# lakehq/sail

Hardware: NVIDIA H100
Metric: TPC-H Q1 rows/s (scan+filter+hash-aggregate), lineitem resident in HBM (higher is better)
Workload: dtype i128 (Decimal128) / i64

## Files before the change

sail_b200/csrc/capi.cu:

```cuda
#include <cstdio>

#include "h2d.hpp"
#include "runner.hpp"

using namespace sg;

struct sailgpu_ctx {
  Ctx ctx;
};
struct sailgpu_op {
  std::unique_ptr<Op> op;
  sailgpu_ctx* owner = nullptr;
  std::string last_error;
  std::vector<bool> input_finished;
};

namespace sg { std::atomic<bool> g_exiting{false}; }

namespace {
thread_local std::string g_ctx_error;
void mark_exiting() { sg::g_exiting.store(true); }

template <typename F>
int32_t guard(std::string* err, F&& f) {
  try {
    f();
    return SAILGPU_OK;
  } catch (const Error& e) {
    if (err) *err = e.what();
    return e.code;
  } catch (const std::exception& e) {
    if (err) *err = std::string("internal error: ") + e.what();
    return SAILGPU_ERR_CUDA;
  }
}
void set_device(const Ctx& c) { SG_CUDA(cudaSetDevice(c.device)); }
using CtxLock = std::lock_guard<std::recursive_mutex>;
}

namespace sg { void set_ctx_error(const std::string& m) { g_ctx_error = m; } }
namespace sg { void resolve_exchange_timing(Ctx* ctx);
void pipeline_static_check(const Json& spec, const std::vector<Schema>& inputs);
size_t pipeline_precompile(const Json& spec, const std::vector<Schema>& inputs, uint64_t validity_mask, bool cold, bool compile, std::string* source); }

namespace sg {
struct ParquetColumnDesc { const uint8_t* chunk; uint64_t chunk_len; int32_t physical_type, type_length, max_def_level, codec; int64_t num_values; };
DevColumn decode_parquet_column(Ctx* ctx, const Field& f, const ParquetColumnDesc& c, int64_t n_rows);
std::string parquet_plan_summary(const Field& f, const ParquetColumnDesc& c, int64_t n_rows);
}

extern "C" {

SAILGPU_API void sailgpu_borrowed_release(struct ArrowArray* a) { if (a) a->release = nullptr; }

SAILGPU_API uint32_t sailgpu_version(void) { return (0u << 16) | 1u; }

SAILGPU_API int32_t sailgpu_ctx_create(int32_t device, sailgpu_ctx** out) {
  return guard(&g_ctx_error, [&] {
    SG_CHECK(out != nullptr, SAILGPU_ERR_INVALID, "out is null");
    int n = 0;
    cudaError_t e = cudaGetDeviceCount(&n);
    if (e != cudaSuccess || n == 0)
      fail(SAILGPU_ERR_NO_DEVICE, std::string("no usable CUDA device (") + cudaGetErrorString(e) + "); libsailgpu has no CPU fallback");
    SG_CHECK(device >= 0 && device < n, SAILGPU_ERR_INVALID, "device ordinal out of range");
    static const int hooked = std::atexit(mark_exiting);
    (void)hooked;
    auto c = std::make_unique<sailgpu_ctx>();
    c->ctx.device = device;
    SG_CUDA(cudaSetDevice(device));
    cudaDeviceProp prop;
    SG_CUDA(cudaGetDeviceProperties(&prop, device));
    SG_CHECK(prop.major == 9 && prop.minor == 0, SAILGPU_ERR_NO_DEVICE, std::string("device '") + prop.name + "' is not sm_90 (Hopper); this library only carries sm_90a code");
    c->ctx.sm_count = prop.multiProcessorCount;
    c->ctx.max_smem = prop.sharedMemPerBlockOptin;
    SG_CUDA(cudaStreamCreateWithFlags(&c->ctx.stream, cudaStreamNonBlocking));
    cudaMemPool_t pool;
    SG_CUDA(cudaDeviceGetDefaultMemPool(&pool, device));
    uint64_t threshold = UINT64_MAX;
    SG_CUDA(cudaMemPoolSetAttribute(pool, cudaMemPoolAttrReleaseThreshold, &threshold));
    *out = c.release();
  });
}

SAILGPU_API void sailgpu_ctx_destroy(sailgpu_ctx* c) {
  if (!c) return;
  if (sg::g_exiting.load()) return;
  CtxLock lk(c->ctx.mu);
  cudaSetDevice(c->ctx.device);
  c->ctx.shared_objects.clear();
  c->ctx.dead.store(true);
  if (c->ctx.stream) { cudaStreamSynchronize(c->ctx.stream); cudaStreamDestroy(c->ctx.stream); c->ctx.stream = nullptr; }
  destroy_pack_pool(&c->ctx);
}

SAILGPU_API const char* sailgpu_ctx_last_error(const sailgpu_ctx*) { return g_ctx_error.c_str(); }

SAILGPU_API void* sailgpu_ctx_stream(sailgpu_ctx* c) { return c ? (void*)c->ctx.stream : nullptr; }
SAILGPU_API int32_t sailgpu_ctx_synchronize(sailgpu_ctx* c) {
  return guard(&g_ctx_error, [&] {
    SG_CHECK(c != nullptr, SAILGPU_ERR_INVALID, "null context");
    CtxLock lk(c->ctx.mu);
    set_device(c->ctx);
    SG_CUDA(cudaStreamSynchronize(c->ctx.stream));
  });
}

SAILGPU_API int32_t sailgpu_op_create(sailgpu_ctx* c, const char* spec_json, size_t spec_len, const struct ArrowSchema* const* input_schemas,
                          int32_t n_inputs, int32_t partition, sailgpu_op** out, struct ArrowSchema* out_schema) {
  return guard(&g_ctx_error, [&] {
    SG_CHECK(c && spec_json && out && out_schema, SAILGPU_ERR_INVALID, "null argument");
    CtxLock lk(c->ctx.mu);
    set_device(c->ctx);
    Json spec = JsonParser(spec_json, spec_len).parse();
    std::vector<Schema> ins;
    for (int i = 0; i < n_inputs; ++i) ins.push_back(schema_from_arrow(input_schemas[i]));
    auto h = std::make_unique<sailgpu_op>();
    h->owner = c;
    h->op = make_op(&c->ctx, spec, ins, partition);
    h->input_finished.assign((size_t)n_inputs, false);
    schema_to_arrow(h->op->out_schema, out_schema);
    *out = h.release();
  });
}

SAILGPU_API int32_t sailgpu_spec_validate(const char* spec_json, size_t spec_len, const struct ArrowSchema* const* input_schemas,
                                          int32_t n_inputs, struct ArrowSchema* out_schema, char* err_buf, size_t err_cap) {
  std::string err;
  const int32_t rc = guard(&err, [&] {
    SG_CHECK(spec_json && out_schema, SAILGPU_ERR_INVALID, "null argument");
    Json spec = JsonParser(spec_json, spec_len).parse();
    std::vector<Schema> ins;
    for (int i = 0; i < n_inputs; ++i) ins.push_back(schema_from_arrow(input_schemas[i]));
    std::unique_ptr<Op> op = make_op(nullptr, spec, ins, 0);
    pipeline_static_check(spec, ins);
    schema_to_arrow(op->out_schema, out_schema);
  });
  if (rc != 0 && err_buf && err_cap) { const size_t k = std::min(err.size(), err_cap - 1); memcpy(err_buf, err.data(), k); err_buf[k] = 0; }
  return rc;
}

SAILGPU_API int64_t sailgpu_jit_precompile(const char* spec_json, size_t spec_len, const struct ArrowSchema* const* input_schemas, int32_t n_inputs,
                                           uint64_t validity_mask, int32_t flags, char* buf, size_t cap) {
  std::string err, source;
  size_t cubin = 0;
  const int32_t rc = guard(&err, [&] {
    SG_CHECK(spec_json && n_inputs >= 1, SAILGPU_ERR_INVALID, "null argument");
    Json spec = JsonParser(spec_json, spec_len).parse();
    std::vector<Schema> ins;
    for (int i = 0; i < n_inputs; ++i) ins.push_back(schema_from_arrow(input_schemas[i]));
    cubin = pipeline_precompile(spec, ins, validity_mask, (flags & SAILGPU_JIT_COLD_VARIANT) != 0, (flags & SAILGPU_JIT_COMPILE) != 0, &source);
  });
// ... 9 lines not shown
  const int32_t rc = guard(&err, [&] {
    SG_CHECK(schema_c && cols && column >= 0 && column < n_cols, SAILGPU_ERR_INVALID, "bad argument");
    Schema schema = schema_from_arrow(schema_c);
    SG_CHECK((int)schema.size() == n_cols, SAILGPU_ERR_INVALID, "parquet: column count mismatch");
    ParquetColumnDesc d{cols[column].chunk, cols[column].chunk_len, cols[column].physical_type, cols[column].type_length, cols[column].max_def_level, cols[column].codec, cols[column].num_values};
    out = parquet_plan_summary(schema[(size_t)column], d, n_rows);
  });
  const std::string& text = rc != 0 ? err : out;
  if (buf && cap) { const size_t k = std::min(text.size(), cap - 1); memcpy(buf, text.data(), k); buf[k] = 0; }
  return rc;
}
SAILGPU_API int32_t sailgpu_parquet_decode(sailgpu_ctx* c, const struct ArrowSchema* schema_c, const sailgpu_parquet_column* cols, int32_t n_cols, int64_t n_rows,
                                           struct ArrowDeviceArray* out) {
  return guard(&g_ctx_error, [&] {
    SG_CHECK(c && schema_c && cols && out && n_rows >= 0, SAILGPU_ERR_INVALID, "null argument");
    CtxLock lk(c->ctx.mu);
    set_device(c->ctx);
    Schema schema = schema_from_arrow(schema_c);
    SG_CHECK((int)schema.size() == n_cols, SAILGPU_ERR_INVALID, "parquet: " + std::to_string(n_cols) + " column chunks for a schema of " + std::to_string(schema.size()) + " fields");
    auto b = std::make_shared<DevBatch>();
    b->rows = n_rows;
    for (int i = 0; i < n_cols; ++i) {
      ParquetColumnDesc d{cols[i].chunk, cols[i].chunk_len, cols[i].physical_type, cols[i].type_length, cols[i].max_def_level, cols[i].codec, cols[i].num_values};
      b->cols.push_back(decode_parquet_column(&c->ctx, schema[(size_t)i], d, n_rows));
    }
    export_device_batch(&c->ctx, schema, b, out);
  });
}

SAILGPU_API int32_t sailgpu_op_push(sailgpu_op* h, int32_t input_idx, struct ArrowArray* batch) {
  if (!h) return SAILGPU_ERR_INVALID;
  return guard(&h->last_error, [&] {
    CtxLock lk(h->owner->ctx.mu);
    set_device(h->owner->ctx);
    SG_CHECK(input_idx >= 0 && input_idx < (int)h->op->in_schemas.size(), SAILGPU_ERR_INVALID, "input index out of range");
    SG_CHECK(!h->input_finished[(size_t)input_idx], SAILGPU_ERR_STATE, "push after finish_input");
    BatchPtr b = import_host_batch(&h->owner->ctx, h->op->in_schemas[(size_t)input_idx], batch);
    h->op->push(input_idx, b);
  });
}

SAILGPU_API int32_t sailgpu_op_push_device(sailgpu_op* h, int32_t input_idx, struct ArrowDeviceArray* batch) {
  if (!h) return SAILGPU_ERR_INVALID;
  return guard(&h->last_error, [&] {
    CtxLock lk(h->owner->ctx.mu);
    set_device(h->owner->ctx);
    SG_CHECK(input_idx >= 0 && input_idx < (int)h->op->in_schemas.size(), SAILGPU_ERR_INVALID, "input index out of range");
    SG_CHECK(!h->input_finished[(size_t)input_idx], SAILGPU_ERR_STATE, "push after finish_input");
    SG_CHECK(batch && batch->array.release, SAILGPU_ERR_INVALID, "batch is null or released");
    BatchPtr b = take_internal_batch(batch, &h->owner->ctx);
    if (!b) { SG_CHECK(batch->array.n_children == (int64_t)h->op->in_schemas[(size_t)input_idx].size(), SAILGPU_ERR_INVALID, "device batch has no column arrays (a handle of another library instance?)"); }
    if (!b) { Trace t(&h->owner->ctx, "import_device_batch"); b = import_device_batch(&h->owner->ctx, h->op->in_schemas[(size_t)input_idx], batch); }
    Trace t2(&h->owner->ctx, "op.push");
    h->op->push(input_idx, b);
  });
}

SAILGPU_API int32_t sailgpu_op_finish_input(sailgpu_op* h, int32_t input_idx) {
  if (!h) return SAILGPU_ERR_INVALID;
  return guard(&h->last_error, [&] {
    CtxLock lk(h->owner->ctx.mu);
    set_device(h->owner->ctx);
    SG_CHECK(input_idx >= 0 && input_idx < (int)h->op->in_schemas.size(), SAILGPU_ERR_INVALID, "input index out of range");
    if (h->input_finished[(size_t)input_idx]) return;
    h->input_finished[(size_t)input_idx] = true;
    Trace t(&h->owner->ctx, "op.finish");
    h->op->finish(input_idx);
  });
}

static int32_t pull_common(sailgpu_op* h, int part, struct ArrowArray* host_out, struct ArrowDeviceArray* dev_out, int32_t* has_more, bool handle_only = false) {
  if (!h) return SAILGPU_ERR_INVALID;
  return guard(&h->last_error, [&] {
    CtxLock lk(h->owner->ctx.mu);
    set_device(h->owner->ctx);
    SG_CHECK(has_more && (host_out || dev_out), SAILGPU_ERR_INVALID, "null argument");
    BatchPtr b;
    bool more;
    { Trace t(&h->owner->ctx, "op.pull"); more = part >= 0 ? h->op->pull_partition(part, &b) : h->op->pull(&b); }
    Trace t2(&h->owner->ctx, "export");
    *has_more = more ? 1 : 0;
    if (!b) b = empty_batch(&h->owner->ctx, h->op->out_schema);
    if (host_out) export_host_batch(&h->owner->ctx, h->op->out_schema, b, host_out);
    else export_device_batch(&h->owner->ctx, h->op->out_schema, b, dev_out, handle_only);
  });
}

SAILGPU_API int32_t sailgpu_op_pull(sailgpu_op* h, struct ArrowArray* out, int32_t* has_more) { return pull_common(h, -1, out, nullptr, has_more); }
SAILGPU_API int32_t sailgpu_op_pull_device(sailgpu_op* h, struct ArrowDeviceArray* out, int32_t* has_more) { return pull_common(h, -1, nullptr, out, has_more); }
SAILGPU_API int32_t sailgpu_op_pull_device_handle(sailgpu_op* h, struct ArrowDeviceArray* out, int32_t* has_more) { return pull_common(h, -1, nullptr, out, has_more, true); }
SAILGPU_API int32_t sailgpu_op_pull_partition(sailgpu_op* h, int32_t part, struct ArrowDeviceArray* out, int32_t* has_more) {
  if (part < 0) return SAILGPU_ERR_INVALID;
  return pull_common(h, part, nullptr, out, has_more);
}

SAILGPU_API int32_t sailgpu_op_pull_ipc(sailgpu_op* h, uint8_t** data, size_t* len, int64_t* rows, int32_t* has_more) {
  if (!h || !data || !len || !has_more) return SAILGPU_ERR_INVALID;
  struct ArrowArray batch;
  memset(&batch, 0, sizeof(batch));
  int32_t rc = pull_common(h, -1, &batch, nullptr, has_more);
  if (rc != SAILGPU_OK) return rc;
  struct ArrowSchema schema;
  memset(&schema, 0, sizeof(schema));
  rc = guard(&h->last_error, [&] { schema_to_arrow(h->op->out_schema, &schema); });
  if (rc == SAILGPU_OK) {
    rc = sailgpu_ipc_stream(&schema, &batch, data, len);
    if (rc != SAILGPU_OK) h->last_error = sailgpu_ipc_last_error();
    else if (rows) *rows = batch.length;
  }
  if (schema.release) schema.release(&schema);
  if (batch.release) batch.release(&batch);
  return rc;
}

SAILGPU_API int64_t sailgpu_op_metrics(sailgpu_op* h, char* json_buf, size_t cap) {
  if (!h) return -1;
  CtxLock lk(h->owner->ctx.mu);
  cudaSetDevice(h->owner->ctx.device);
  const Metrics& m = h->op->m;
  char tmp[2048];
  sg::resolve_exchange_timing(&h->owner->ctx);
  int n = snprintf(tmp, sizeof(tmp),
                   "{\"output_rows\":%llu,\"output_batches\":%llu,\"input_rows\":%llu,\"input_batches\":%llu,"
                   "\"elapsed_compute\":%llu,\"build_input_rows\":%llu,\"build_input_batches\":%llu,\"build_time\":%llu,"
                   "\"join_time\":%llu,\"gpu.kernel_launches\":%llu,\"gpu.h2d_bytes\":%llu,\"gpu.d2h_bytes\":%llu,"
                   "\"gpu.pipeline_launches\":%llu,\"gpu.jit_launches\":%llu,\"gpu.pipeline_kernel_ns\":%llu,"
                   "\"gpu.exchange_sent_bytes\":%llu,\"gpu.exchange_recv_bytes\":%llu,\"gpu.exchange_ns\":%llu,\"gpu.exchange_calls\":%llu}",
                   (unsigned long long)m.output_rows, (unsigned long long)m.output_batches, (unsigned long long)m.input_rows,
                   (unsigned long long)m.input_batches, (unsigned long long)m.elapsed_compute_ns, (unsigned long long)m.build_input_rows,
                   (unsigned long long)m.build_input_batches, (unsigned long long)m.build_time_ns, (unsigned long long)m.join_time_ns,
                   (unsigned long long)m.kernel_launches, (unsigned long long)h->owner->ctx.h2d_bytes.load(),
                   (unsigned long long)h->owner->ctx.d2h_bytes.load(), (unsigned long long)h->op->m.pipeline_launches, (unsigned long long)h->op->m.jit_launches,
                   (unsigned long long)h->op->pipeline_kernel_ns(), (unsigned long long)h->owner->ctx.exch_sent_bytes.load(),
                   (unsigned long long)h->owner->ctx.exch_recv_bytes.load(), (unsigned long long)h->owner->ctx.exch_ns.load(),
                   (unsigned long long)h->owner->ctx.exch_calls.load());
  if (json_buf && cap) { size_t k = std::min<size_t>((size_t)n, cap - 1); memcpy(json_buf, tmp, k); json_buf[k] = 0; }
  return n + 1;
}

SAILGPU_API const char* sailgpu_last_error(const sailgpu_op* h) { return h ? h->last_error.c_str() : "null handle"; }

SAILGPU_API void sailgpu_op_destroy(sailgpu_op* h) {
  if (!h) return;
  if (sg::g_exiting.load()) return;
  CtxLock lk(h->owner->ctx.mu);
  cudaSetDevice(h->owner->ctx.device);
  cudaStreamSynchronize(h->owner->ctx.stream);
  delete h;
}

SAILGPU_API int32_t sailgpu_host_alloc(sailgpu_ctx* c, size_t bytes, void** out) {
  return guard(&g_ctx_error, [&] {
    SG_CHECK(c && out, SAILGPU_ERR_INVALID, "null argument");
    CtxLock lk(c->ctx.mu);
    set_device(c->ctx);
    SG_CUDA(cudaHostAlloc(out, bytes ? bytes : 1, cudaHostAllocDefault));
  });
}
SAILGPU_API void sailgpu_host_free(sailgpu_ctx* c, void* p) {
  if (!c || !p) return;
  CtxLock lk(c->ctx.mu);
  cudaSetDevice(c->ctx.device);
  cudaFreeHost(p);
}

}
```

sail_b200/csrc/device.cu:

```cuda
#include <cstdlib>
#include <cstring>

#include "device.hpp"
#include "h2d.hpp"
#include "kernels.hpp"
#include "relational.hpp"

namespace sg {

Schema schema_from_arrow(const ArrowSchema* s) {
  SG_CHECK(s && s->format && std::string(s->format) == "+s", SAILGPU_ERR_INVALID, "input schema must be a struct (+s)");
  Schema out;
  for (int64_t i = 0; i < s->n_children; ++i) {
    const ArrowSchema* c = s->children[i];
    Field f;
    f.name = c->name ? c->name : "";
    f.type = type_from_arrow_format(c->format);
    f.nullable = (c->flags & ARROW_FLAG_NULLABLE) != 0;
    out.push_back(f);
  }
  return out;
}

namespace {
struct SchemaPriv {
  std::string format, name;
  std::vector<ArrowSchema> children;
  std::vector<ArrowSchema*> child_ptrs;
};
void release_schema(ArrowSchema* s) {
  if (!s || !s->release) return;
  for (int64_t i = 0; i < s->n_children; ++i)
// ... 82 lines not shown
  c.type = f.type;
  c.length = a->length;
  c.null_count = a->null_count;
  auto borrow = [&](const void* p, size_t bytes) {
    auto b = std::make_shared<DevBuf>();
    b->ptr = const_cast<void*>(p); b->bytes = bytes;
    b->on_release = [token] {};
    return b;
  };
  const uint8_t* vbits = a->n_buffers > 0 ? static_cast<const uint8_t*>(a->buffers[0]) : nullptr;
  if (vbits && a->null_count != 0 && a->length > 0) {
    c.validity = import_bitmap(J, vbits, a->offset, a->length);
    if (on_device && c.validity->on_release) c.validity->on_release = [token] {};
    if (c.null_count < 0) c.null_count = -1;
  } else {
    c.null_count = 0;
  }
  const int w = f.type.arrow_width();
  switch (f.type.id) {
    case TypeId::Bool: {
      const uint8_t* bits = static_cast<const uint8_t*>(a->buffers[1]);
      c.data = a->length ? import_bitmap(J, bits, a->offset, a->length) : dev_alloc(ctx, 0);
      if (on_device && c.data->on_release) c.data->on_release = [token] {};
      break;
    }
    case TypeId::Utf8: {
      const int32_t* offs = static_cast<const int32_t*>(a->buffers[1]) + a->offset;
      const uint8_t* bytes = static_cast<const uint8_t*>(a->buffers[2]);
      BufPtr doffs, dbytes;
      if (on_device) {
        doffs = borrow(offs, (size_t)(a->length + 1) * 4);
        int32_t last = 0;
        if (a->length) SG_CUDA(cudaMemcpyAsync(&last, offs + a->length, 4, cudaMemcpyDeviceToHost, stream));
        SG_CUDA(cudaStreamSynchronize(stream));
        dbytes = borrow(bytes, (size_t)last);
      } else {
        doffs = J.upload(offs, a->length + 1, 4);
        const int32_t last = a->length ? offs[a->length] : 0;
        dbytes = J.upload(bytes, last, 1);
      }
      c.data = dev_alloc(ctx, (size_t)a->length * 16);
      {
        BufPtr views = c.data;
        const int64_t n = a->length;
        J.after([=] { SG_CUDA(launch_utf8_to_views(static_cast<const int32_t*>(doffs->ptr), static_cast<const uint8_t*>(dbytes->ptr), views->ptr, n, stream)); });
      }
      c.heaps = {dbytes, doffs};
      c.arrow_is_utf8 = true;
      break;
    }
    case TypeId::Utf8View: {
      const uint8_t* views = static_cast<const uint8_t*>(a->buffers[1]) + a->offset * 16;
      const int64_t n_data = a->n_buffers - 3;
      if (on_device && n_data <= 0) c.data = borrow(views, (size_t)a->length * 16);
      else c.data = J.upload(views, a->length, 16, n_data <= 0 ? HostCol::View16 : HostCol::Raw);
      if (n_data > 0) {
        std::vector<int64_t> sizes((size_t)n_data);
        const int64_t* size_buf = static_cast<const int64_t*>(a->buffers[a->n_buffers - 1]);
        if (on_device) { SG_CUDA(cudaMemcpyAsync(sizes.data(), size_buf, (size_t)n_data * 8, cudaMemcpyDeviceToHost, stream)); SG_CUDA(cudaStreamSynchronize(stream)); }
        else std::memcpy(sizes.data(), size_buf, (size_t)n_data * 8);
        auto bases = std::make_shared<std::vector<uint64_t>>((size_t)n_data);
        for (int64_t k = 0; k < n_data; ++k) {
          BufPtr h = on_device ? borrow(a->buffers[2 + k], (size_t)sizes[k]) : J.upload(a->buffers[2 + k], sizes[k], 1);
          (*bases)[(size_t)k] = reinterpret_cast<uint64_t>(h->ptr);
          c.heaps.push_back(h);
        }
        BufPtr dbases = dev_alloc(ctx, (size_t)n_data * 8);
        BufPtr vdata = c.data;
        const int64_t n = a->length;
        J.after([=] {
          SG_CUDA(cudaMemcpyAsync(dbases->ptr, bases->data(), (size_t)n_data * 8, cudaMemcpyHostToDevice, stream));
          SG_CUDA(launch_resolve_views(vdata->ptr, n, static_cast<const uint64_t*>(dbases->ptr), stream));
          SG_CUDA(cudaStreamSynchronize(stream));
        });
        c.heaps.push_back(dbases);
      }
      break;
    }
    default: {
      SG_CHECK(w > 0, SAILGPU_ERR_UNSUPPORTED, "unsupported column type " + f.type.str());
      const uint8_t* p = static_cast<const uint8_t*>(a->buffers[1]) + a->offset * w;
      if (on_device) c.data = borrow(p, (size_t)a->length * w);
      else {
        const TypeId id = f.type.id;
        const HostCol kind = id == TypeId::Decimal128 ? HostCol::Dec128
                           : (id == TypeId::Int64 || id == TypeId::UInt64) ? HostCol::Int64
                           : (id == TypeId::Int32 || id == TypeId::UInt32 || id == TypeId::Date32) ? HostCol::Int32 : HostCol::Raw;
        c.data = J.upload(p, a->length, w, kind);
      }
    }
  }
  return c;
}

BatchPtr import_batch(Ctx* ctx, const Schema& schema, ArrowArray* arr, bool on_device, cudaStream_t stream) {
  SG_CHECK(arr && arr->release, SAILGPU_ERR_INVALID, "batch is null or already released");
  SG_CHECK(arr->n_children == (int64_t)schema.size(), SAILGPU_ERR_INVALID,
           "batch has " + std::to_string(arr->n_children) + " columns, schema has " + std::to_string(schema.size()));
  SG_CHECK(arr->offset == 0, SAILGPU_ERR_UNSUPPORTED, "struct-level offset is not supported");
  auto token = std::make_shared<ReleaseToken>();
  token->arr = *arr;
  arr->release = nullptr;
  auto b = std::make_shared<DevBatch>();
  b->rows = token->arr.length;
  ImportJob J(ctx, on_device, stream);
  for (size_t i = 0; i < schema.size(); ++i) {
// ... 20 lines not shown
  if (arr->sync_event) SG_CUDA(cudaStreamWaitEvent(ctx->stream, *static_cast<cudaEvent_t*>(arr->sync_event), 0));
  return import_batch(ctx, schema, &arr->array, true, ctx->stream);
}

namespace {

struct ArrayPriv {
  std::vector<void*> host_allocs;
  std::vector<const void*> buffers;
  std::vector<ArrowArray> children;
  std::vector<ArrowArray*> child_ptrs;
  std::vector<BufPtr> keep;
  BatchPtr batch;
  Ctx* ctx = nullptr;
  bool opaque = false;
};
void release_array(ArrowArray* a) {
  if (!a || !a->release) return;
  for (int64_t i = 0; i < a->n_children; ++i)
    if (a->children[i]->release) a->children[i]->release(a->children[i]);
  auto* p = static_cast<ArrayPriv*>(a->private_data);
  for (void* h : p->host_allocs) free(h);
  delete p;
  a->release = nullptr;
}
void init_array(ArrowArray* a, int64_t length, int64_t null_count, ArrayPriv* p) {
  a->length = length; a->null_count = null_count; a->offset = 0;
  a->n_buffers = (int64_t)p->buffers.size(); a->buffers = p->buffers.data();
  a->n_children = 0; a->children = nullptr; a->dictionary = nullptr;
  a->release = release_array; a->private_data = p;
}

struct StringExport { BufPtr views_or_offsets, heap; int64_t heap_bytes = 0; };
StringExport export_strings(Ctx* ctx, const DevColumn& c, bool as_utf8) {
  StringExport out;
  const int64_t n = c.length;
  if (n == 0) {
    out.views_or_offsets = dev_alloc_zero(ctx, as_utf8 ? 4 : 0);
    out.heap = dev_alloc(ctx, 0);
    return out;
  }
  if (!as_utf8) {
    BufPtr mx = dev_alloc_zero(ctx, 8);
    unsigned int max_len = 0;
    SG_CUDA(launch_max_view_len(c.data->ptr, n, static_cast<unsigned int*>(mx->ptr), ctx->stream));
    SG_CUDA(cudaMemcpyAsync(&max_len, mx->ptr, 4, cudaMemcpyDeviceToHost, ctx->stream));
    SG_CUDA(cudaStreamSynchronize(ctx->stream));
    if (max_len <= 12) {
      out.views_or_offsets = c.data;
      out.heap = dev_alloc(ctx, 0);
      return out;
    }
  }
  BufPtr lens = dev_alloc(ctx, (size_t)n * 4);
  BufPtr offs = dev_alloc(ctx, (size_t)n * 8);
  BufPtr scratch = dev_alloc(ctx, 1026 * 8);
  SG_CUDA(launch_view_lengths(c.data->ptr, n, static_cast<uint32_t*>(lens->ptr), as_utf8 ? 1 : 0, ctx->stream));
  SG_CUDA(launch_exclusive_scan_u32(static_cast<uint32_t*>(lens->ptr), n, static_cast<uint64_t*>(offs->ptr), static_cast<uint64_t*>(scratch->ptr), ctx->stream));
  const int64_t nblocks = std::min<int64_t>(1024, (n + 4095) / 4096);
  uint64_t total = 0;
  SG_CUDA(cudaMemcpyAsync(&total, static_cast<uint64_t*>(scratch->ptr) + nblocks, 8, cudaMemcpyDeviceToHost, ctx->stream));
  SG_CUDA(cudaStreamSynchronize(ctx->stream));
  out.heap_bytes = (int64_t)total;
  out.heap = dev_alloc(ctx, (size_t)total);
  if (as_utf8) {
    SG_CHECK(total < (1ull << 31), SAILGPU_ERR_UNSUPPORTED, "Utf8 output exceeds 2 GiB of string data; use Utf8View");
    out.views_or_offsets = dev_alloc(ctx, (size_t)(n + 1) * 4);
    SG_CUDA(launch_views_to_utf8(c.data->ptr, n, static_cast<uint64_t*>(offs->ptr), static_cast<int32_t*>(out.views_or_offsets->ptr),
                                 static_cast<uint8_t*>(out.heap->ptr), ctx->stream));
  } else {
    SG_CHECK(total < (1ull << 31), SAILGPU_ERR_UNSUPPORTED, "string heap of one output batch exceeds 2 GiB");
    out.views_or_offsets = dev_alloc(ctx, (size_t)n * 16);
    SG_CUDA(cudaMemcpyAsync(out.views_or_offsets->ptr, c.data->ptr, (size_t)n * 16, cudaMemcpyDeviceToDevice, ctx->stream));
    SG_CUDA(launch_views_to_arrow(out.views_or_offsets->ptr, n, static_cast<uint64_t*>(offs->ptr), static_cast<uint8_t*>(out.heap->ptr), ctx->stream));
  }
  return out;
}

void* to_host(Ctx* ctx, const void* dptr, size_t bytes, ArrayPriv* p) {
  void* h = malloc(bytes ? bytes : 1);
  SG_CHECK(h != nullptr, SAILGPU_ERR_CUDA, "host allocation failed");
  p->host_allocs.push_back(h);
  ctx->d2h_bytes += bytes;
  if (!bytes) return h;
  if (bytes <= Ctx::D2H_SMALL) {
    if (!ctx->d2h_stage && cudaHostAlloc(&ctx->d2h_stage, Ctx::D2H_STAGE_BYTES, cudaHostAllocDefault) != cudaSuccess) { cudaGetLastError(); ctx->d2h_stage = nullptr; }
    const size_t off = (ctx->d2h_used + 15) & ~(size_t)15;
    if (ctx->d2h_stage && off + bytes <= Ctx::D2H_STAGE_BYTES) {
      SG_CUDA(cudaMemcpyAsync(static_cast<uint8_t*>(ctx->d2h_stage) + off, dptr, bytes, cudaMemcpyDeviceToHost, ctx->stream));
      ctx->d2h_pending.push_back({h, off, bytes});
      ctx->d2h_used = off + bytes;
      return h;
    }
  }
  SG_CUDA(cudaMemcpyAsync(h, dptr, bytes, cudaMemcpyDeviceToHost, ctx->stream));
  return h;
}

void finish_small_d2h(Ctx* ctx) {
  for (auto& it : ctx->d2h_pending) memcpy(it.host, static_cast<const uint8_t*>(ctx->d2h_stage) + it.off, it.bytes);
  ctx->d2h_pending.clear();
  ctx->d2h_used = 0;
}

void export_column(Ctx* ctx, const Field& f, const DevColumn& c, ArrowArray* out, bool to_device) {
  auto* p = new ArrayPriv();
  const int64_t n = c.length;
  auto emit = [&](const BufPtr& b, size_t bytes) -> const void* {
    if (!b) return nullptr;
    if (to_device) { p->keep.push_back(b); return b->ptr; }
    return to_host(ctx, b->ptr, bytes, p);
  };
  int64_t null_count = c.validity ? c.null_count : 0;
  p->buffers.push_back(c.validity ? emit(c.validity, (size_t)((n + 7) / 8)) : nullptr);
  if (f.type.is_string()) {
    const bool as_utf8 = f.type.id == TypeId::Utf8;
    StringExport s = export_strings(ctx, c, as_utf8);
    if (as_utf8) {
      p->buffers.push_back(emit(s.views_or_offsets, (size_t)(n + 1) * 4));
      p->buffers.push_back(emit(s.heap, (size_t)s.heap_bytes));
    } else {
      p->buffers.push_back(emit(s.views_or_offsets, (size_t)n * 16));
      const bool has_heap = s.heap_bytes > 0;
      if (has_heap) p->buffers.push_back(emit(s.heap, (size_t)s.heap_bytes));
      int64_t* sizes = static_cast<int64_t*>(malloc(8));
      sizes[0] = s.heap_bytes;
      p->host_allocs.push_back(sizes);
      if (to_device) {
        BufPtr dsz = dev_alloc(ctx, 8);
        SG_CUDA(cudaMemcpyAsync(dsz->ptr, sizes, 8, cudaMemcpyHostToDevice, ctx->stream));
        p->keep.push_back(dsz);
        p->buffers.push_back(dsz->ptr);
      } else {
        p->buffers.push_back(sizes);
      }
    }
  } else if (f.type.id == TypeId::Bool) {
    p->buffers.push_back(emit(c.data, (size_t)((n + 7) / 8)));
  } else {
    p->buffers.push_back(emit(c.data, (size_t)n * f.type.arrow_width()));
  }
  init_array(out, n, null_count, p);
}

}

void export_host_batch(Ctx* ctx, const Schema& schema, const BatchPtr& b, ArrowArray* out) {
  ctx->d2h_pending.clear(); ctx->d2h_used = 0;
  auto* p = new ArrayPriv();
  p->buffers.push_back(nullptr);
  p->children.resize(schema.size());
  p->child_ptrs.resize(schema.size());
  for (size_t i = 0; i < schema.size(); ++i) {
    p->children[i].release = nullptr;
    export_column(ctx, schema[i], b->cols[i], &p->children[i], false);
    p->child_ptrs[i] = &p->children[i];
  }
  SG_CUDA(cudaStreamSynchronize(ctx->stream));
  finish_small_d2h(ctx);
  init_array(out, b->rows, 0, p);
  out->n_children = (int64_t)schema.size();
  out->children = p->child_ptrs.data();
}

void export_device_batch(Ctx* ctx, const Schema& schema, const BatchPtr& b, ArrowDeviceArray* out, bool handle_only) {
  auto* p = new ArrayPriv();
  p->buffers.push_back(nullptr);
  p->batch = b;
  p->ctx = ctx;
  if (handle_only) {
    p->opaque = true;
    init_array(&out->array, b->rows, 0, p);
    out->array.n_children = 0;
    out->array.children = nullptr;
  } else {
    p->children.resize(schema.size());
    p->child_ptrs.resize(schema.size());
    for (size_t i = 0; i < schema.size(); ++i) {
      p->children[i].release = nullptr;
      export_column(ctx, schema[i], b->cols[i], &p->children[i], true);
      p->child_ptrs[i] = &p->children[i];
    }
    SG_CUDA(cudaStreamSynchronize(ctx->stream));
    init_array(&out->array, b->rows, 0, p);
    out->array.n_children = (int64_t)schema.size();
    out->array.children = p->child_ptrs.data();
  }
  out->device_id = ctx->device;
  out->device_type = ARROW_DEVICE_CUDA;
  out->sync_event = nullptr;
  out->reserved[0] = out->reserved[1] = out->reserved[2] = 0;
}

BatchPtr take_internal_batch(ArrowDeviceArray* arr, Ctx* consumer) {
  if (arr->array.release != release_array) return nullptr;
  auto* p = static_cast<ArrayPriv*>(arr->array.private_data);
  BatchPtr b = p->batch;
  if (b) {
    if (p->opaque && p->ctx && p->ctx != consumer) cudaStreamSynchronize(p->ctx->stream);
    arr->array.release(&arr->array);
  }
  return b;
}

BatchPtr empty_batch(Ctx* ctx, const Schema& schema) {
  auto b = std::make_shared<DevBatch>();
  for (auto& f : schema) {
    DevColumn c; c.type = f.type; c.length = 0; c.data = dev_alloc(ctx, 0);
    c.arrow_is_utf8 = f.type.id == TypeId::Utf8;
    b->cols.push_back(c);
  }
  return b;
}

BatchPtr concat_batches(Ctx* ctx, const Schema& schema, const std::vector<BatchPtr>& parts) {
  if (parts.empty()) return empty_batch(ctx, schema);
// ... 49 lines not shown
```

sail_b200/csrc/device.hpp:

```cpp
#pragma once
#include <cuda_runtime.h>

#include <atomic>
#include <functional>
#include <mutex>
#include <unordered_map>
#include <vector>

#include "common.hpp"

namespace sg {

#define SG_CUDA(call)                                                                                  \
  do {                                                                                                 \
    cudaError_t _e = (call);                                                                           \
    if (_e != cudaSuccess)                                                                             \
      ::sg::fail(SAILGPU_ERR_CUDA, std::string("CUDA error: ") + cudaGetErrorString(_e) + " at " #call); \
  } while (0)

struct PackPool;

struct Ctx {
  int device = 0;
  int sm_count = 132;
  size_t max_smem = 227 * 1024;
  cudaStream_t stream = nullptr;
  std::map<std::string, std::shared_ptr<void>> shared_objects;
  PackPool* pack_pool = nullptr;
  std::string last_error;
  std::recursive_mutex mu;
  void* nccl_comm = nullptr;
  int rank = 0, world = 1;
  std::atomic<bool> dead{false};
  std::atomic<uint64_t> h2d_bytes{0}, d2h_bytes{0};
  std::atomic<uint64_t> exch_sent_bytes{0}, exch_recv_bytes{0}, exch_ns{0}, exch_calls{0};
  std::vector<std::pair<cudaEvent_t, cudaEvent_t>> exch_events;
  struct D2HItem { void* host; size_t off, bytes; };
  void* d2h_stage = nullptr;
  size_t d2h_used = 0;
  std::vector<D2HItem> d2h_pending;
  static constexpr size_t D2H_STAGE_BYTES = 1 << 20, D2H_SMALL = 64 << 10;
  std::mutex cache_mu;
  std::unordered_map<size_t, std::vector<void*>> cache;
  size_t cached_bytes = 0;
  static constexpr size_t CACHE_LIMIT = 64ull << 30;
  static size_t size_class(size_t padded) { return padded <= (1u << 20) ? (padded + 511) & ~(size_t)511 : (padded + (1u << 20) - 1) & ~(size_t)((1u << 20) - 1); }
};

extern std::atomic<bool> g_exiting;

struct DevBuf {
  void* ptr = nullptr;
  size_t bytes = 0;
  size_t cls = 0;
  Ctx* ctx = nullptr;
  std::function<void()> on_release;
  ~DevBuf() {
    if (g_exiting.load()) return;
    if (on_release) { on_release(); return; }
    if (!ptr || !ctx) return;
    if (ctx->dead.load()) { cudaFree(ptr); return; }
    if (cls) {
      std::lock_guard<std::mutex> g(ctx->cache_mu);
      if (ctx->cached_bytes + cls <= Ctx::CACHE_LIMIT) { ctx->cache[cls].push_back(ptr); ctx->cached_bytes += cls; return; }
    }
    cudaFreeAsync(ptr, ctx->stream);
  }
};
using BufPtr = std::shared_ptr<DevBuf>;

inline BufPtr dev_alloc(Ctx* ctx, size_t bytes) {
  auto b = std::make_shared<DevBuf>();
  b->ctx = ctx;
  b->bytes = bytes;
  const size_t padded = ((bytes + 255) & ~(size_t)255) + 256;
  static const bool no_cache = getenv("SAILGPU_NO_ALLOC_CACHE") != nullptr;
  const size_t cls = no_cache ? 0 : Ctx::size_class(padded);
  if (cls) {
    std::lock_guard<std::mutex> g(ctx->cache_mu);
    auto it = ctx->cache.find(cls);
// ... 55 lines not shown
```

sail_b200/csrc/engine.cu:

```cuda
#include "runner.hpp"

namespace sg {


StageSpec parse_stage(const Json& j, const Schema& in, Schema* out) {
  StageSpec st;
  const std::string op = j.at("op").as_str();
  if (op == "filter") {
    st.kind = StageSpec::Filter;
    st.predicate = parse_expr(j.at("predicate"), in);
    SG_CHECK(st.predicate->type.id == TypeId::Bool, SAILGPU_ERR_INVALID, "filter predicate must be boolean");
    const Json* p = j.find("projection");
    if (p && !p->is_null()) {
      st.has_projection = true;
      for (auto& x : p->a) {
        int i = (int)x.as_int();
        SG_CHECK(i >= 0 && i < (int)in.size(), SAILGPU_ERR_INVALID, "filter projection index out of range");
        st.projection.push_back(i);
        out->push_back(in[(size_t)i]);
      }
    } else *out = in;
  } else if (op == "projection") {
    st.kind = StageSpec::Projection;
    for (auto& x : j.at("exprs").a) {
      ExprPtr e = parse_expr(x.at("expr"), in);
      st.exprs.push_back(e);
      st.names.push_back(x.at("name").as_str());
      out->push_back({st.names.back(), e->type, e->nullable});
    }
  } else if (op == "aggregate") {
    st.kind = StageSpec::Aggregate;
    const Json* md = j.find("mode");
    st.mode = md ? md->as_str() : "single";
    SG_CHECK(st.mode == "single" || st.mode == "partial" || st.mode == "final" || st.mode == "final_partitioned", SAILGPU_ERR_INVALID,
             "aggregate mode '" + st.mode + "'");
// ... 9 lines not shown
      StageSpec::Agg ag;
      ag.fn = a.at("fn").as_str();
      ag.name = a.at("name").as_str();
      const Json* it = a.find("input_type");
      if (it && !it->is_null()) ag.input_type = parse_type(it->as_str());
      const Json* args = a.find("args");
      if (!merging && args && args->kind == Json::Arr && !args->a.empty()) { ag.arg = parse_expr(args->a[0], in); ag.has_arg = true; ag.input_type = ag.arg->type; }
      SG_CHECK(ag.fn == "count" || ag.has_arg || merging, SAILGPU_ERR_INVALID, "aggregate '" + ag.fn + "' needs an argument");
      SG_CHECK(ag.fn == "count" || ag.input_type.id != TypeId::Null, SAILGPU_ERR_INVALID, "aggregate '" + ag.name + "' needs input_type in final mode");
      AggTypes at = agg_types(ag.fn, ag.fn == "count" ? T(TypeId::Int64) : ag.input_type);
      if (merging) {
        for (size_t k = 0; k < at.state.size(); ++k) {
          SG_CHECK(state_col + k < in.size(), SAILGPU_ERR_INVALID, "final aggregate: input has too few state columns");
          const DataType& have = in[state_col + k].type;
          SG_CHECK(have == at.state[k] || (have.id == TypeId::Int64 && at.state[k].id == TypeId::UInt64) || (have.id == TypeId::UInt64 && at.state[k].id == TypeId::Int64),
                   SAILGPU_ERR_INVALID, "final aggregate: state column " + std::to_string(state_col + k) + " is " + have.str() + ", expected " + at.state[k].str());
        }
      }
      state_col += at.state.size();
      if (st.mode == "partial") {
        if (ag.fn == "avg") { out->push_back({ag.name + "[count]", at.state[0], false}); out->push_back({ag.name + "[sum]", at.state[1], true}); }
        else out->push_back({ag.name + "[" + ag.fn + "]", at.state[0], ag.fn != "count"});
      } else {
        out->push_back({ag.name, at.final_type, ag.fn != "count"});
      }
      st.aggs.push_back(ag);
    }
  } else {
    fail(SAILGPU_ERR_UNSUPPORTED, "operator '" + op + "' cannot be part of a fused pipeline");
  }
  return st;
}

void check_device_error(Ctx* ctx, uint32_t* dev_flag) {
  uint32_t f = 0;
  SG_CUDA(cudaMemcpyAsync(&f, dev_flag, 4, cudaMemcpyDeviceToHost, ctx->stream));
  SG_CUDA(cudaStreamSynchronize(ctx->stream));
  if (!f) return;
  SG_CUDA(cudaMemsetAsync(dev_flag, 0, 4, ctx->stream));
  if (f & ERR_DIV_ZERO) fail(SAILGPU_ERR_ARITHMETIC, "Divide by zero");
  if (f & ERR_OVERFLOW) fail(SAILGPU_ERR_ARITHMETIC, "Arithmetic overflow");
  if (f & ERR_TABLE_FULL) fail(SAILGPU_ERR_CUDA, "hash table overflow");
  fail(SAILGPU_ERR_UNSUPPORTED, "unsupported value encountered on device");
}

struct AggTable {
  BufPtr table, state, occ;
  uint64_t capacity = 0;
  bool direct = false;
};

struct PipelineOp : Op {
  PipelineRunner run;
  bool has_agg = false;
  StageSpec* agg_stage = nullptr;
  AggTable tab;
  std::shared_ptr<CompiledPipeline> agg_cp;
  std::deque<BatchPtr> ready;
  std::vector<BufPtr> kept_heaps;
  bool input_done = false, emitted = false;

  void collect_heaps(const DevBatch& b) {
    for (auto& c : b.cols)
      if (c.type.is_string()) for (auto& h : c.heaps) kept_heaps.push_back(h);
  }

  void push(int input, const BatchPtr& b) override {
    SG_CHECK(input == 0, SAILGPU_ERR_INVALID, "operator has one input");
    SG_CHECK(!input_done, SAILGPU_ERR_STATE, "push after finish_input");
    const uint64_t t0 = now_ns();
    m.input_rows += (uint64_t)b->rows; m.input_batches++;
    if (has_agg) { collect_heaps(*b); push_agg(b); }
    else if (const std::vector<int>* cols = rename_only()) {
      auto out = std::make_shared<DevBatch>();
      out->rows = b->rows;
      for (int c : *cols) out->cols.push_back(b->cols[(size_t)c]);
// ... 59 lines not shown
    mask_run.stages.push_back(f);
    mask_run.custom_sink = [](PipelineCompiler& pc, CompiledPipeline& cp) { pc.finish_mask_store(cp); };
    Schema in2 = in;
    Field mf; mf.name = "__mask"; mf.type.id = TypeId::Bool; mf.nullable = false;
    in2.push_back(mf);
    sel_run.init(ctx, in2);
    if (!share_key.empty()) sel_run.share(share_key + "#select");
    sel_run.stages = run.stages;
    StageSpec& s0 = sel_run.stages[0];
    auto me = std::make_shared<Expr>(); me->kind = Expr::Col; me->col = (int)in.size(); me->type.id = TypeId::Bool; me->nullable = false;
    s0.predicate = me;
    if (!s0.has_projection) { s0.has_projection = true; s0.projection.clear(); for (size_t i = 0; i < in.size(); ++i) s0.projection.push_back((int)i); }
    two_pass_ready = true;
  }
  bool two_pass_applies(const BatchPtr& b) const {
    const char* mn = getenv("SAILGPU_TWO_PASS_MIN");
    if (mn && !strcmp(mn, "off")) return false;
    const int64_t min_rows = mn && *mn ? atoll(mn) : TWO_PASS_MIN_ROWS;
    return !has_agg && !run.stages.empty() && run.stages[0].kind == StageSpec::Filter && b->rows >= min_rows;
  }
  BatchPtr run_two_pass(const BatchPtr& b) {
    if (!two_pass_ready) setup_two_pass();
    BatchPtr mb = run_streaming(mask_run, ctx, b, m, nullptr, {});
    auto b2 = std::make_shared<DevBatch>(*b);
    b2->cols.push_back(mb->cols[0]);
    auto cp2 = sel_run.compiled_for(*b2);
    const int tile_rows = cp2->rpt * NT;
    const int64_t n = b->rows, n_tiles = (n + tile_rows - 1) / tile_rows;
    BufPtr counts = dev_alloc_zero(ctx, (size_t)(n_tiles + 1) * 4), offs = dev_alloc(ctx, (size_t)(n_tiles + 1) * 8), scratch = dev_alloc(ctx, 1026 * 8);
    SG_CUDA(launch_tile_popcount(static_cast<const uint32_t*>(mb->cols[0].data->ptr), n, tile_rows, n_tiles, static_cast<uint32_t*>(counts->ptr), ctx->stream));
    SG_CUDA(launch_exclusive_scan_u32(static_cast<const uint32_t*>(counts->ptr), n_tiles + 1, static_cast<uint64_t*>(offs->ptr), static_cast<uint64_t*>(scratch->ptr), ctx->stream));
    unsigned long long total = 0;
    SG_CUDA(cudaMemcpyAsync(&total, static_cast<const uint64_t*>(offs->ptr) + n_tiles, 8, cudaMemcpyDeviceToHost, ctx->stream));
    SG_CUDA(cudaStreamSynchronize(ctx->stream));
    m.kernel_launches += 4;
    return run_streaming(sel_run, ctx, b2, m, nullptr, {}, static_cast<const unsigned long long*>(offs->ptr), (int64_t)total);
  }

  BatchPtr run_stream(const BatchPtr& b) {
    if (two_pass_applies(b)) return run_two_pass(b);
    return run_streaming(run, ctx, b, m, nullptr, {});
  }

  static constexpr uint64_t MIN_CAPACITY = 1ull << 22, MAX_CAPACITY = 1ull << 28;
  static constexpr uint64_t CARD_MANY_GROUPS = 256, HOT_GROUP_LIMIT = 1 << 16;
  static uint64_t min_capacity() { const char* v = getenv("SAILGPU_AGG_MIN_CAPACITY"); return v && *v ? next_pow2((uint64_t)atoll(v)) : MIN_CAPACITY; }
  bool use_cold = false;
  int64_t rows_in_table = 0;
  int64_t known_groups = -1;
  struct Pending { BatchPtr batch; std::shared_ptr<CompiledPipeline> cp; BufPtr deferred; int64_t n_tiles = 0; bool active = false; } pend;

  unsigned long long* n_deferred_ptr() { return reinterpret_cast<unsigned long long*>(static_cast<uint8_t*>(run.scal.buf->ptr) + 40); }

  uint64_t read_n_groups() {
    run.ensure_scratch();
    unsigned long long g = 0;
    SG_CUDA(cudaMemcpyAsync(&g, run.scal.n_groups(), 8, cudaMemcpyDeviceToHost, ctx->stream));
    SG_CUDA(cudaStreamSynchronize(ctx->stream));
    return g;
  }

  void fill_table(AggParams& A) {
    A.table = static_cast<uint8_t*>(tab.table->ptr);
    A.state = static_cast<uint32_t*>(tab.state->ptr);
    A.occ = static_cast<uint32_t*>(tab.occ->ptr);
    A.capacity_mask = tab.capacity - 1;
    A.n_groups = run.scal.n_groups();
    A.direct_key = tab.direct ? 1 : 0;
  }
  static bool direct_eligible(const AggParams& A) {
    const char* e = getenv("SAILGPU_DIRECT_KEY");
    return A.n_keys == 1 && A.key_words == 1 && !A.has_null_word && e && *e && atoi(e) != 0;
  }
  void build_occ(const AggTable& t, const AggParams& layout) {
    if (!t.direct) return;
    AggParams A = layout;
    A.table = static_cast<uint8_t*>(t.table->ptr); A.occ = static_cast<uint32_t*>(t.occ->ptr); A.capacity_mask = t.capacity - 1;
    BufPtr counter = dev_alloc_zero(ctx, 8);
    SG_CUDA(launch_agg_build_occ(A, static_cast<unsigned long long*>(counter->ptr), ctx->stream));
    m.kernel_launches++;
  }

  void alloc_table(const AggParams& A0, uint64_t cap, uint64_t groups) {
    SG_CHECK(cap <= MAX_CAPACITY, SAILGPU_ERR_UNSUPPORTED, "aggregate needs more than 2^28 group slots");
    AggTable old = tab;
    tab.capacity = cap;
    tab.direct = direct_eligible(A0);
    tab.table = dev_alloc(ctx, (size_t)(cap + 1) * A0.entry_words * 8);
    tab.state = tab.direct ? dev_alloc(ctx, 4) : dev_alloc_zero(ctx, (size_t)cap * 4);
    tab.occ = dev_alloc(ctx, (size_t)(cap + 1) * 4);
    if (tab.direct) { run.ensure_scratch(); AggParams A = A0; fill_table(A); SG_CUDA(launch_agg_init_direct(A, ctx->stream)); m.kernel_launches++; }
    if (old.capacity && groups) {
      build_occ(old, A0);
      AggParams A = A0;
      fill_table(A);
      SG_CUDA(cudaMemsetAsync(run.scal.n_groups(), 0, 8, ctx->stream));
      SG_CUDA(launch_agg_rehash(A, static_cast<const uint8_t*>(old.table->ptr), static_cast<const uint32_t*>(old.occ->ptr), groups, run.scal.error(), ctx->stream));
      m.kernel_launches++;
    }
  }

  void launch_agg(const std::shared_ptr<CompiledPipeline>& cp, const DevBatch& b, const BufPtr& list, int64_t n_list, const BufPtr& deferred_out) {
    PipelineParams P;
    run.prepare(P, *cp, b, 0, b.rows);
    if (list) { P.tile_list = static_cast<const uint32_t*>(list->ptr); P.n_list = n_list; }
    PipelineAux aux;
    memset(&aux, 0, sizeof(aux));
    aux.agg = cp->agg;
    fill_table(aux.agg);
    if (deferred_out) {
      SG_CUDA(cudaMemsetAsync(n_deferred_ptr(), 0, 8, ctx->stream));
      aux.agg.deferred = static_cast<uint32_t*>(deferred_out->ptr);
      aux.agg.n_deferred = n_deferred_ptr();
      const char* fl = getenv("SAILGPU_AGG_FIRST_LIMIT");
      aux.agg.group_limit = (!list && fl && *fl) ? (unsigned long long)atoll(fl) : ~0ull;
      run.group_limit_cap = (cp->cold_variant || list) ? ~0ull : HOT_GROUP_LIMIT;
    }
    run.launch(P, cp, &aux, m);
  }

  std::vector<bool> sticky_sig;
  BufPtr ones; size_t ones_bytes = 0;

  BatchPtr with_union_signature(const BatchPtr& b, bool* widened) {
    *widened = false;
    if (sticky_sig.empty()) sticky_sig.assign(b->cols.size(), false);
    bool same = true;
    for (size_t i = 0; i < b->cols.size(); ++i) {
      const bool has = (bool)b->cols[i].validity;
      if (has && !sticky_sig[i]) { sticky_sig[i] = true; *widened = true; }
      same &= has == sticky_sig[i];
    }
    if (same) return b;
    const size_t need = (size_t)((b->rows + 31) / 32 * 4);
    if (!ones || ones_bytes < need) {
      ones_bytes = std::max<size_t>(need, 1 << 16);
      ones = dev_alloc(ctx, ones_bytes);
      SG_CUDA(cudaMemsetAsync(ones->ptr, 0xFF, ones_bytes, ctx->stream));
    }
    auto bb = std::make_shared<DevBatch>(*b);
    for (size_t i = 0; i < bb->cols.size(); ++i)
      if (sticky_sig[i] && !bb->cols[i].validity) { bb->cols[i].validity = ones; bb->cols[i].null_count = 0; }
    return bb;
  }

  static bool same_layout(const CompiledPipeline& a, const CompiledPipeline& b) {
    const AggParams &x = a.agg, &y = b.agg;
    if (x.entry_words != y.entry_words || x.key_words != y.key_words || x.has_null_word != y.has_null_word || x.n_accs != y.n_accs) return false;
    for (int j = 0; j < x.n_accs; ++j)
      if (x.accs[j].op != y.accs[j].op || x.accs[j].word != y.accs[j].word || x.accs[j].track_seen != y.accs[j].track_seen) return false;
    return a.acc_ident == b.acc_ident;
  }

  void migrate_layout(const std::shared_ptr<CompiledPipeline>& from, const std::shared_ptr<CompiledPipeline>& to) {
    Trace tr(ctx, "agg.migrate");
    const AggParams &O = from->agg, &N = to->agg;
    AggMigrateMap M;
    memset(&M, 0, sizeof(M));
    M.old_entry_words = (int32_t)O.entry_words; M.old_key_words = O.key_words;
    M.key_shift = (N.has_null_word && !O.has_null_word) ? 1 : 0;
    SG_CHECK(N.key_words == O.key_words + M.key_shift && N.has_null_word >= O.has_null_word, SAILGPU_ERR_UNSUPPORTED, "aggregate layouts of two batches cannot be reconciled (group keys)");
    std::vector<int> src((size_t)N.n_accs, -1);
    for (auto& kv : to->acc_ident) {
      auto it = from->acc_ident.find(kv.first);
      SG_CHECK(it != from->acc_ident.end(), SAILGPU_ERR_UNSUPPORTED, "aggregate layouts of two batches cannot be reconciled (" + kv.first + ")");
      src[(size_t)kv.second] = it->second;
    }
    for (int j = 0; j < N.n_accs; ++j) {
      SG_CHECK(src[(size_t)j] >= 0 && O.accs[src[(size_t)j]].op == N.accs[j].op, SAILGPU_ERR_UNSUPPORTED, "aggregate layouts of two batches cannot be reconciled (accumulator kinds)");
      M.acc_src_word[j] = (int16_t)O.accs[src[(size_t)j]].word;
      M.seen_src[j] = N.accs[j].track_seen ? (O.accs[src[(size_t)j]].track_seen ? (int8_t)src[(size_t)j] : (int8_t)-1) : (int8_t)-2;
    }
    check_device_error(ctx, run.scal.error());
    const uint64_t groups = read_n_groups();
    AggTable old = tab;
    build_occ(old, O);
    tab.direct = direct_eligible(N);
    tab.table = dev_alloc(ctx, (size_t)(tab.capacity + 1) * N.entry_words * 8);
    tab.state = tab.direct ? dev_alloc(ctx, 4) : dev_alloc_zero(ctx, (size_t)tab.capacity * 4);
    tab.occ = dev_alloc(ctx, (size_t)(tab.capacity + 1) * 4);
    run.ensure_scratch();
    AggParams A = N;
    fill_table(A);
    if (tab.direct) { SG_CUDA(launch_agg_init_direct(A, ctx->stream)); m.kernel_launches++; }
    SG_CUDA(cudaMemsetAsync(run.scal.n_groups(), 0, 8, ctx->stream));
    SG_CUDA(launch_agg_migrate(A, M, static_cast<const uint8_t*>(old.table->ptr), static_cast<const uint32_t*>(old.occ->ptr), groups, run.scal.error(), ctx->stream));
    m.kernel_launches++;
    known_groups = -1;
  }

  void push_agg(const BatchPtr& b0) {
    Trace tr(ctx, "agg.push");
    resolve_pending();
    if (b0->rows == 0) return;
    bool widened = false;
    const BatchPtr b = with_union_signature(b0, &widened);
    auto cp = run.compiled_for(*b, use_cold);
    if (agg_cp && tab.capacity && !same_layout(*agg_cp, *cp)) {
      SG_CHECK(widened, SAILGPU_ERR_STATE, "aggregate layout changed without a new validity buffer");
      migrate_layout(agg_cp, cp);
    }
    agg_cp = cp;
    const bool grouped = cp->agg.n_keys > 0;
    if (!tab.capacity) alloc_table(cp->agg, grouped ? std::min<uint64_t>(min_capacity(), next_pow2(8 * (uint64_t)b->rows + 2048)) : 1024, 0);
    const int64_t tile_rows = (int64_t)cp->rpt * NT;
    const int64_t n_tiles = (b->rows + tile_rows - 1) / tile_rows;
    BufPtr deferred = grouped ? dev_alloc(ctx, (size_t)n_tiles * 4) : nullptr;
    launch_agg(cp, *b, nullptr, 0, deferred);
    rows_in_table += b->rows;
    known_groups = -1;
    if (grouped) { pend.batch = b; pend.cp = cp; pend.deferred = deferred; pend.n_tiles = n_tiles; pend.active = true; }
  }

  void resolve_pending() {
    if (!pend.active) return;
    Trace tr(ctx, "agg.resolve");
    uint64_t prev_def = 0;
    for (;;) {
      unsigned long long gd[3] = {0, 0, 0};
      SG_CUDA(cudaMemcpyAsync(gd, run.scal.n_groups(), 24, cudaMemcpyDeviceToHost, ctx->stream));
      check_device_error(ctx, run.scal.error());
      const uint64_t groups = gd[0], n_def = gd[2];
      if (n_def == 0) { known_groups = (int64_t)groups; break; }
      const int64_t tile_rows = (int64_t)pend.cp->rpt * NT;
      const double rows_def = (double)std::min<int64_t>((int64_t)n_def * tile_rows, pend.batch->rows);
      const double rows_done = std::max(1.0, (double)rows_in_table - rows_def);
      const double ratio = groups ? std::min(1.0, (double)groups / rows_done) : 1.0;
      const double est = ratio * rows_def * 1.25 + 1024.0;
      uint64_t cap = next_pow2((uint64_t)(2.0 * ((double)groups + est)) + 2 * MIN_CAPACITY / 2);
      const bool stuck = prev_def != 0 && n_def >= prev_def;
      if (cap <= tab.capacity && stuck) cap = tab.capacity * 2;
      prev_def = n_def;
      if (cap > tab.capacity) alloc_table(pend.cp->agg, cap, groups);
      std::shared_ptr<CompiledPipeline> cp = pend.cp;
      if (!use_cold && groups > CARD_MANY_GROUPS && getenv("SAILGPU_NO_COLD") == nullptr) {
        auto cold = run.compiled_for(*pend.batch, true);
        if (cold->agg.entry_words == cp->agg.entry_words) {
          use_cold = true;
          if (cold->rpt == cp->rpt) cp = cold;
        }
      }
      BufPtr next_deferred = dev_alloc(ctx, (size_t)n_def * 4);
      launch_agg(cp, *pend.batch, pend.deferred, (int64_t)n_def, next_deferred);
      pend.cp = cp; pend.deferred = next_deferred;
    }
    pend = Pending();
  }

  BatchPtr extract_agg() {
    resolve_pending();
    Trace tr(ctx, "agg.extract");
    std::shared_ptr<CompiledPipeline> cp = agg_cp;
    if (!cp) {
      DevBatch dummy;
      for (auto& f : run.in_schema) { DevColumn c; c.type = f.type; dummy.cols.push_back(c); }
      cp = run.compiled_for(dummy);
    }
    const AggParams& A0 = cp->agg;
    run.ensure_scratch();
    uint64_t groups = 0;
    if (tab.capacity) {
      if (known_groups >= 0) groups = (uint64_t)known_groups;
      else { check_device_error(ctx, run.scal.error()); groups = read_n_groups(); }
    }
    const bool synth = A0.n_keys == 0 && groups == 0;
    const int64_t rows = synth ? 1 : (int64_t)groups;
    auto out = std::make_shared<DevBatch>();
    out->rows = rows;
    AggExtractParams X;
    memset(&X, 0, sizeof(X));
    X.n_cols = (int)cp->agg_outs.size();
    std::vector<BufPtr> vbytes((size_t)X.n_cols);
    for (int i = 0; i < X.n_cols; ++i) {
      const AggOutSpec& s = cp->agg_outs[(size_t)i];
      AggOutCol& o = X.cols[i];
      o.kind = s.kind; o.a = s.a; o.b = s.b; o.nullable = s.nullable ? 1 : 0;
      o.width = s.type.is_string() ? 16 : s.type.arrow_width();
      SG_CHECK(s.type.id != TypeId::Bool, SAILGPU_ERR_UNSUPPORTED, "boolean group keys are not supported yet");
      if (s.kind == 0) { o.key_word = s.b; o.src_words = A0.keys[s.a].width == 16 ? 2 : 1; }
      else if (s.kind == 1) { const int op = A0.accs[s.a].op; o.src_words = (op == ACC_SUM_I128 || op == ACC_MIN_I128 || op == ACC_MAX_I128) ? 2 : 1; }
      else {
        o.is_float = s.type.is_float() ? 1 : 0;
        if (!o.is_float) { i128 mul = pow10_i128(s.type.scale - s.in_type.scale); o.scale_mul_lo = (uint64_t)(u128)mul; o.scale_mul_hi = (uint64_t)((u128)mul >> 64); }
      }
      DevColumn c; c.type = s.type; c.length = rows; c.arrow_is_utf8 = s.type.id == TypeId::Utf8;
      c.data = dev_alloc_zero(ctx, (size_t)rows * o.width);
      o.data = static_cast<uint8_t*>(c.data->ptr);
      if (s.nullable) { vbytes[(size_t)i] = dev_alloc_zero(ctx, (size_t)rows + 4); o.valid_bytes = static_cast<uint8_t*>(vbytes[(size_t)i]->ptr); }
      if (c.type.is_string()) c.heaps = kept_heaps;
      out->cols.push_back(c);
    }
    if (!synth && rows > 0) {
      build_occ(tab, A0);
      AggParams A = A0;
      fill_table(A);
      SG_CUDA(launch_agg_extract(A, X, groups, run.scal.error(), ctx->stream));
      m.kernel_launches++;
    } else if (synth) {
      for (int i = 0; i < X.n_cols; ++i) {
        const AggOutSpec& s = cp->agg_outs[(size_t)i];
        const bool is_count = s.kind == 1 && (A0.accs[s.a].op == ACC_COUNT || (A0.accs[s.a].op == ACC_SUM_I64 && !A0.accs[s.a].track_seen));
        if (vbytes[(size_t)i] && is_count) SG_CUDA(cudaMemsetAsync(vbytes[(size_t)i]->ptr, 1, 1, ctx->stream));
      }
    }
    SG_CUDA(cudaMemsetAsync(run.scal.nulls(0), 0, 8 * 20, ctx->stream));
    std::vector<unsigned long long> nulls((size_t)X.n_cols, 0);
    BufPtr nullctr = dev_alloc_zero(ctx, (size_t)X.n_cols * 8 + 8);
    for (int i = 0; i < X.n_cols; ++i) {
      if (!vbytes[(size_t)i] || rows == 0) continue;
      DevColumn& c = out->cols[(size_t)i];
      c.validity = dev_alloc_zero(ctx, (size_t)((rows + 31) / 32 * 4));
      SG_CUDA(launch_pack_bytes(static_cast<const uint8_t*>(vbytes[(size_t)i]->ptr), static_cast<uint32_t*>(c.validity->ptr), rows,
                                static_cast<unsigned long long*>(nullctr->ptr) + i, ctx->stream));
    }
    SG_CUDA(cudaMemcpyAsync(nulls.data(), nullctr->ptr, (size_t)X.n_cols * 8, cudaMemcpyDeviceToHost, ctx->stream));
    SG_CUDA(cudaStreamSynchronize(ctx->stream));
    for (int i = 0; i < X.n_cols; ++i) {
      DevColumn& c = out->cols[(size_t)i];
      if (c.validity) { c.null_count = (int64_t)nulls[(size_t)i]; if (c.null_count == 0) c.validity = nullptr; }
    }
    return out;
  }
};

size_t pipeline_precompile(const Json& spec, const std::vector<Schema>& inputs, uint64_t validity_mask, bool cold, bool compile, std::string* source) {
  static Ctx plan_ctx;
  std::unique_ptr<Op> op = make_op(&plan_ctx, spec, inputs, 0);
  PipelineOp* p = dynamic_cast<PipelineOp*>(op.get());
  SG_CHECK(p != nullptr, SAILGPU_ERR_UNSUPPORTED, "only filter / projection / aggregate pipelines are specialised");
  DevBatch shape;
  for (size_t i = 0; i < inputs[0].size(); ++i) {
    DevColumn c; c.type = inputs[0][i].type;
    if (i < 64 && ((validity_mask >> i) & 1)) c.validity = std::make_shared<DevBuf>();
    shape.cols.push_back(c);
  }
  auto cp = p->run.compiled_for(shape, cold);
  std::string why;
  SG_CHECK(jit_supported(*cp, &why), SAILGPU_ERR_UNSUPPORTED, "kernel specialiser: " + why);
  JitPlan plan;
  SG_CHECK(jit_plan(*cp, plan_ctx.max_smem, &plan), SAILGPU_ERR_UNSUPPORTED, "kernel specialiser: pipeline does not fit in shared memory");
  const std::string src = jit_generate(*cp, plan);
  if (source) *source = src;
  return compile ? jit_precompile_to_cache(src) : 0;
}

static thread_local bool g_in_static_check = false;
std::unique_ptr<Op> make_wide_agg_op(Ctx* ctx, const Json& spec, const std::vector<Schema>& inputs, const Schema& out_schema);
void pipeline_static_check(const Json& spec, const std::vector<Schema>& inputs) {
  static Ctx plan_ctx;
// ... 19 lines not shown
  if (kind == "hash_join") return make_join_op(ctx, spec, inputs);
  if (kind == "nested_loop_join") return make_nlj_op(ctx, spec, inputs);
  if (kind == "sort") return make_sort_op(ctx, spec, inputs);
  if (kind == "sort_preserving_merge") return make_merge_op(ctx, spec, inputs);
  if (kind == "repartition") return make_repartition_op(ctx, spec, inputs);
  if (kind == "chain") return make_chain_op(ctx, spec, inputs);
  if (kind == "exchange") return make_exchange_op(ctx, spec, inputs);
  SG_CHECK(inputs.size() == 1, SAILGPU_ERR_INVALID, "operator '" + kind + "' takes exactly one input");
  auto op = std::make_unique<PipelineOp>();
  op->ctx = ctx; op->kind = kind; op->in_schemas = inputs;
  op->run.init(ctx, inputs[0]);
  std::vector<const Json*> stage_specs;
  if (kind == "pipeline") for (auto& s : spec.at("stages").a) stage_specs.push_back(&s);
  else stage_specs.push_back(&spec);
  SG_CHECK(!stage_specs.empty(), SAILGPU_ERR_INVALID, "empty pipeline");
  Schema cur = inputs[0];
  for (const Json* s : stage_specs) {
    Schema next;
    op->run.stages.push_back(parse_stage(*s, cur, &next));
    cur = next;
  }
  {
    std::string key = "pipeline|";
    json_dump(spec, &key);
    for (auto& f : inputs[0]) { key += '|'; key += f.type.str(); key += f.nullable ? '?' : '!'; }
    op->share_key = key;
    op->run.share(key);
  }
  op->has_agg = op->run.stages.back().kind == StageSpec::Aggregate;
  for (size_t i = 0; i + 1 < op->run.stages.size(); ++i)
    SG_CHECK(op->run.stages[i].kind != StageSpec::Aggregate, SAILGPU_ERR_INVALID, "aggregate must be the last stage of a pipeline");
  op->out_schema = cur;
  if (kind == "aggregate" && !g_in_static_check) {
    bool wide = false;
    g_in_static_check = true;
    try { pipeline_static_check(spec, inputs); }
    catch (const Error& e) { wide = e.code == SAILGPU_ERR_UNSUPPORTED && std::string(e.what()).find("group key") != std::string::npos; }
    g_in_static_check = false;
    if (wide) return make_wide_agg_op(ctx, spec, inputs, cur);
  }
  return op;
}

}
```

sail_b200/csrc/engine.hpp:

```cpp
#pragma once
#include <chrono>
#include <deque>

#include "compiler.hpp"
#include "device.hpp"
#include "kernels.hpp"

namespace sg {

BatchPtr take_internal_batch(ArrowDeviceArray* arr, Ctx* consumer);

struct Metrics {
  uint64_t input_rows = 0, input_batches = 0, output_rows = 0, output_batches = 0;
  uint64_t elapsed_compute_ns = 0, kernel_launches = 0;
  uint64_t build_input_rows = 0, build_input_batches = 0, build_time_ns = 0, join_time_ns = 0;
  uint64_t pipeline_launches = 0, pipeline_kernel_ns = 0, jit_launches = 0;
  std::vector<std::pair<cudaEvent_t, cudaEvent_t>> pending;
};

struct Op {
  Ctx* ctx = nullptr;
  std::vector<Schema> in_schemas;
  Schema out_schema;
  std::string last_error;
  std::string kind;
  Metrics m;
  virtual ~Op() { if (!g_exiting.load()) for (auto& p : m.pending) { cudaEventDestroy(p.first); cudaEventDestroy(p.second); } }
  uint64_t pipeline_kernel_ns() {
    for (auto& p : m.pending) {
      float ms = 0.f;
      if (cudaEventSynchronize(p.second) == cudaSuccess && cudaEventElapsedTime(&ms, p.first, p.second) == cudaSuccess)
        m.pipeline_kernel_ns += (uint64_t)((double)ms * 1e6);
      cudaEventDestroy(p.first); cudaEventDestroy(p.second);
    }
    m.pending.clear();
    return m.pipeline_kernel_ns;
  }
  virtual void push(int input, const BatchPtr& b) = 0;
  virtual void finish(int input) = 0;
  virtual bool pull(BatchPtr* out) = 0;
  virtual bool pull_partition(int, BatchPtr*) { fail(SAILGPU_ERR_STATE, "operator has no partitioned output"); }
};

std::unique_ptr<Op> make_op(Ctx* ctx, const Json& spec, const std::vector<Schema>& inputs, int partition);

StageSpec parse_stage(const Json& j, const Schema& in, Schema* out);
void check_device_error(Ctx* ctx, uint32_t* dev_flag);

struct DevScalars {
// ... 11 lines not shown
```

sail_b200/csrc/ops_more.cu:

```cuda
#include <dlfcn.h>

#include "relational.hpp"
#include "runner.hpp"

namespace sg {

struct JoinOp : Op {
  std::string jt;
  std::vector<int> lkeys, rkeys;
  Json filter_json; bool has_filter = false;
  std::vector<int> projection; bool has_proj = false;
  Schema bs, ps, joined;
  std::vector<BatchPtr> bparts;
  BatchPtr build;
  bool build_done = false, probe_done = false, tail_done = false;
  BufPtr table, dupflag, visited, next;
  uint64_t capacity = 0;
  bool dup = false;
  std::vector<BufPtr> build_valid_bytes, build_bool_bytes;
  std::vector<BufPtr> build_heaps;
  PipelineRunner brun, prun, frun, trun;
  ProbeParams pp{};
  std::map<const CompiledPipeline*, ProbeParams> pps;
  std::deque<BatchPtr> pending, ready;
// ... 313 lines not shown
    }
    return c;
  }

  void mark_all_matches(const BatchPtr& b) {
    JoinMultiParams J; memset(&J, 0, sizeof(J));
    J.n_probe = b->rows; J.n_keys = (int)lkeys.size();
    fill_raw(J.build_keys, *build, lkeys, bs);
    fill_raw(J.probe_keys, *b, rkeys, ps);
    J.table = static_cast<const uint8_t*>(table->ptr); J.capacity_mask = capacity - 1;
    J.visited = static_cast<uint8_t*>(visited->ptr);
    J.next = static_cast<const int64_t*>(next->ptr);
    J.pass = 2;
    SG_CUDA(launch_join_multi(J, ctx->stream));
    m.kernel_launches++;
  }

  void probe_general(const BatchPtr& b) {
    const int64_t n = b->rows;
    JoinMultiParams J; memset(&J, 0, sizeof(J));
    J.n_probe = n; J.n_keys = (int)lkeys.size();
    fill_raw(J.build_keys, *build, lkeys, bs);
    fill_raw(J.probe_keys, *b, rkeys, ps);
    J.table = static_cast<const uint8_t*>(table->ptr); J.capacity_mask = capacity - 1;
    J.emit_unmatched_probe = jt == "right" ? 1 : 0;
    J.next = static_cast<const int64_t*>(next->ptr);
    BufPtr counts = dev_alloc(ctx, (size_t)n * 4), offs = dev_alloc(ctx, (size_t)n * 8), scratch = dev_alloc(ctx, 1026 * 8);
    J.counts = static_cast<uint32_t*>(counts->ptr); J.pass = 0;
    SG_CUDA(launch_join_multi(J, ctx->stream));
    SG_CUDA(launch_exclusive_scan_u32(J.counts, n, static_cast<uint64_t*>(offs->ptr), static_cast<uint64_t*>(scratch->ptr), ctx->stream));
    const int64_t nblocks = std::min<int64_t>(1024, (n + 4095) / 4096);
    uint64_t total = 0;
    SG_CUDA(cudaMemcpyAsync(&total, static_cast<uint64_t*>(scratch->ptr) + nblocks, 8, cudaMemcpyDeviceToHost, ctx->stream));
    SG_CUDA(cudaStreamSynchronize(ctx->stream));
    if (total == 0) return;
    BufPtr ob = dev_alloc(ctx, (size_t)total * 8), op = dev_alloc(ctx, (size_t)total * 8);
    J.offsets = static_cast<const uint64_t*>(offs->ptr); J.out_build = static_cast<int64_t*>(ob->ptr); J.out_probe = static_cast<int64_t*>(op->ptr);
    J.visited = visited ? static_cast<uint8_t*>(visited->ptr) : nullptr;
    J.pass = 1;
    SG_CUDA(launch_join_multi(J, ctx->stream));
    m.kernel_launches += 2;
    auto out = std::make_shared<DevBatch>();
    out->rows = (int64_t)total;
    for (size_t i = 0; i < bs.size(); ++i) out->cols.push_back(gather_column(build->cols[i], bs[i], J.out_build, (int64_t)total, jt == "right"));
    for (size_t i = 0; i < ps.size(); ++i) out->cols.push_back(gather_column(b->cols[i], ps[i], J.out_probe, (int64_t)total, false));
    SG_CUDA(cudaStreamSynchronize(ctx->stream));
    ready.push_back(post_filter(out));
  }

  BatchPtr post_filter(const BatchPtr& joined_batch) {
    if (!has_filter && !has_proj) return joined_batch;
    if (frun.stages.empty()) {
      if (has_filter) {
        StageSpec st; st.kind = StageSpec::Filter; st.predicate = parse_expr(filter_json, joined); st.has_projection = has_proj; st.projection = projection;
        frun.stages.push_back(st);
      } else {
        return project_plain(joined_batch, 0);
      }
    }
    return run_streaming(frun, ctx, joined_batch, m, nullptr, {});
  }

  void emit_tail() {
    if (tail_done) return;
    tail_done = true;
    if (!needs_visited() || build->rows == 0) return;
    const int64_t n = build->rows;
    auto ext = std::make_shared<DevBatch>(*build);
    DevColumn vis; vis.type = T(TypeId::Bool); vis.length = n;
    vis.data = dev_alloc_zero(ctx, (size_t)((n + 31) / 32 * 4));
    SG_CUDA(launch_pack_bytes(static_cast<const uint8_t*>(visited->ptr), static_cast<uint32_t*>(vis.data->ptr), n, nullptr, ctx->stream));
    ext->cols.push_back(vis);
    Schema es = bs; es.push_back({"__visited", T(TypeId::Bool), false});
    trun.init(ctx, es);
    auto vcol = std::make_shared<Expr>(); vcol->kind = Expr::Col; vcol->col = (int)bs.size(); vcol->type = T(TypeId::Bool);
    ExprPtr pred = vcol;
    if (jt != "left_semi") { auto nt = std::make_shared<Expr>(); nt->kind = Expr::Not; nt->args = {vcol}; nt->type = T(TypeId::Bool); pred = nt; }
    StageSpec f; f.kind = StageSpec::Filter; f.predicate = pred; f.has_projection = true;
    for (size_t i = 0; i < bs.size(); ++i) f.projection.push_back((int)i);
// ... 219 lines not shown
  Json a; a.kind = Json::Obj;
  a.o = {{"op", FilteredSemiJoinOp::jstr("hash_join")}, {"join_type", FilteredSemiJoinOp::jstr("inner")}, {"on", spec.at("on")}, {"filter", fmap},
         {"projection", FilteredSemiJoinOp::jarr({FilteredSemiJoinOp::jnum(nb)})}};
  op->pairs = make_plain_join_op(ctx, a, {bs_id, inputs[1]});
  std::vector<Json> proj;
  const Json* pj = spec.find("projection");
  if (pj && !pj->is_null()) for (auto& x : pj->a) proj.push_back(x);
  else for (int i = 0; i < nb; ++i) proj.push_back(FilteredSemiJoinOp::jnum(i));
  Json b; b.kind = Json::Obj;
  b.o = {{"op", FilteredSemiJoinOp::jstr("hash_join")}, {"join_type", FilteredSemiJoinOp::jstr(jt)},
         {"on", FilteredSemiJoinOp::jarr({FilteredSemiJoinOp::jarr({FilteredSemiJoinOp::jnum(nb), FilteredSemiJoinOp::jnum(0)})})},
         {"projection", FilteredSemiJoinOp::jarr(proj)}};
  Schema ids = {{"__row", T(TypeId::Int64), true}};
  op->pick = make_plain_join_op(ctx, b, {bs_id, ids});
  return op;
}

struct NestedLoopJoinOp : Op {
  static constexpr int64_t MAX_BUILD_ROWS = 64;
  Schema ls, rs, joined;
  ExprPtr filter;
  std::vector<int> projection;
  std::vector<BatchPtr> lparts;
  std::vector<std::unique_ptr<PipelineRunner>> runs;
  std::deque<BatchPtr> pending, ready;
  bool left_done = false, right_done = false;

  static ExprPtr literal_of(Ctx* ctx, const DevColumn& c, const DataType& t, int64_t row) {
    auto e = std::make_shared<Expr>();
    e->kind = Expr::Lit; e->type = t;
    if (c.validity) {
      uint8_t byte = 0;
      SG_CUDA(cudaMemcpyAsync(&byte, static_cast<const uint8_t*>(c.validity->ptr) + (row >> 3), 1, cudaMemcpyDeviceToHost, ctx->stream));
      SG_CUDA(cudaStreamSynchronize(ctx->stream));
      if (!((byte >> (row & 7)) & 1)) { e->lit_null = true; e->nullable = true; return e; }
    }
    if (t.id == TypeId::Bool) {
      uint8_t byte = 0;
      SG_CUDA(cudaMemcpyAsync(&byte, static_cast<const uint8_t*>(c.data->ptr) + (row >> 3), 1, cudaMemcpyDeviceToHost, ctx->stream));
      SG_CUDA(cudaStreamSynchronize(ctx->stream));
      e->lit_i = (byte >> (row & 7)) & 1;
      return e;
    }
    const int w = t.is_string() ? 16 : t.arrow_width();
    uint8_t raw[16] = {0};
    SG_CUDA(cudaMemcpyAsync(raw, static_cast<const uint8_t*>(c.data->ptr) + row * w, (size_t)w, cudaMemcpyDeviceToHost, ctx->stream));
    SG_CUDA(cudaStreamSynchronize(ctx->stream));
    if (t.is_string()) {
      uint32_t len; memcpy(&len, raw, 4);
      e->lit_s.resize(len);
      if (len <= 12) memcpy(&e->lit_s[0], raw + 4, len);
      else {
        uint64_t ptr; memcpy(&ptr, raw + 8, 8);
        SG_CUDA(cudaMemcpyAsync(&e->lit_s[0], reinterpret_cast<const void*>(ptr), len, cudaMemcpyDeviceToHost, ctx->stream));
        SG_CUDA(cudaStreamSynchronize(ctx->stream));
      }
    } else if (t.id == TypeId::Float64) { memcpy(&e->lit_f, raw, 8); }
    else if (t.id == TypeId::Float32) { float f; memcpy(&f, raw, 4); e->lit_f = f; }
    else if (w == 16) { u128 v; memcpy(&v, raw, 16); e->lit_i = (i128)v; }
    else if (w == 8) { int64_t v; memcpy(&v, raw, 8); e->lit_i = t.is_unsigned_int() ? (i128)(uint64_t)v : (i128)v; }
    else if (w == 4) { int32_t v; memcpy(&v, raw, 4); e->lit_i = t.is_unsigned_int() ? (i128)(uint32_t)v : (i128)v; }
    else if (w == 2) { int16_t v; memcpy(&v, raw, 2); e->lit_i = t.is_unsigned_int() ? (i128)(uint16_t)v : (i128)v; }
    else { int8_t v; memcpy(&v, raw, 1); e->lit_i = t.is_unsigned_int() ? (i128)(uint8_t)v : (i128)v; }
    return e;
  }
  ExprPtr bind_row(const ExprPtr& e, const std::vector<ExprPtr>& lits) const {
    if (e->kind == Expr::Col) {
      if (e->col < (int)ls.size()) return lits[(size_t)e->col];
      auto c = std::make_shared<Expr>(*e);
      c->col = e->col - (int)ls.size();
      return c;
    }
    if (e->kind == Expr::Lit) return e;
    auto c = std::make_shared<Expr>(*e);
    for (auto& a : c->args) a = bind_row(a, lits);
    return c;
  }

  void build_runners() {
    BatchPtr left = lparts.empty() ? empty_batch(ctx, ls) : concat_batches(ctx, ls, lparts);
    lparts.clear();
    SG_CHECK(left->rows <= MAX_BUILD_ROWS, SAILGPU_ERR_UNSUPPORTED,
             "nested loop join with " + std::to_string(left->rows) + " build rows (the GPU path covers the scalar-subquery shapes: at most " + std::to_string(MAX_BUILD_ROWS) + ")");
    for (int64_t r = 0; r < left->rows; ++r) {
      std::vector<ExprPtr> lits;
      for (size_t c = 0; c < ls.size(); ++c) lits.push_back(literal_of(ctx, left->cols[c], ls[c].type, r));
      auto run = std::make_unique<PipelineRunner>();
      run->init(ctx, rs);
// ... 61 lines not shown
  for (int i : op->projection) op->out_schema.push_back(op->joined[(size_t)i]);
  SG_CHECK((int)op->out_schema.size() <= MAX_OUTPUTS, SAILGPU_ERR_UNSUPPORTED, "nested_loop_join: more than " + std::to_string(MAX_OUTPUTS) + " output columns");
  return op;
}

struct SortOp : Op {
  struct Key { ExprPtr e; bool asc, nulls_first; };
  std::vector<Key> keys;
  int64_t fetch = -1;
  std::vector<BatchPtr> parts;
  bool input_done = false, emitted = false;
  PipelineRunner krun;

  void push(int input, const BatchPtr& b) override {
    SG_CHECK(input == 0, SAILGPU_ERR_INVALID, "sort has one input");
    m.input_rows += (uint64_t)b->rows; m.input_batches++;
    parts.push_back(b);
  }
  void finish(int) override { input_done = true; }
  bool pull(BatchPtr* out) override {
    *out = nullptr;
    if (!input_done) return true;
    if (emitted) return false;
    const uint64_t t0 = now_ns();
    *out = run();
    emitted = true;
    m.elapsed_compute_ns += now_ns() - t0;
    m.output_rows += (uint64_t)(*out)->rows; m.output_batches++;
    return false;
  }

  struct Encoded { BufPtr keys, bits; int key_bytes = 0; };

  Encoded encode_keys(const BatchPtr& all, const Schema& sch, const std::vector<Key>& ks) {
    const int64_t n = all->rows;
    SortEncodeParams E; memset(&E, 0, sizeof(E));
    E.n = n; E.n_keys = (int)ks.size();
    int off = 0;
    BufPtr maxlen = dev_alloc_zero(ctx, 8 * 8);
    std::vector<int> str_keys;
    for (size_t k = 0; k < ks.size(); ++k) {
      SG_CHECK(ks[k].e->kind == Expr::Col, SAILGPU_ERR_UNSUPPORTED, "sort keys must be column references");
      const DevColumn& c = all->cols[(size_t)ks[k].e->col];
      const DataType& t = sch[(size_t)ks[k].e->col].type;
      SortKeyCol& s = E.cols[k];
      s.data = static_cast<const uint8_t*>(c.data->ptr);
      s.validity_bits = c.validity ? static_cast<const uint8_t*>(c.validity->ptr) : nullptr;
      s.asc = ks[k].asc; s.nulls_first = ks[k].nulls_first;
      if (t.is_string()) { s.kind = SORT_VIEW; s.width = 16; SG_CUDA(launch_max_view_len(c.data->ptr, n, static_cast<unsigned int*>(maxlen->ptr) + k, ctx->stream)); str_keys.push_back((int)k); }
      else if (t.id == TypeId::Bool) { s.kind = SORT_BOOL; s.width = 1; s.enc_bytes = 1; }
      else if (t.is_float()) { SG_CHECK(t.id == TypeId::Float64, SAILGPU_ERR_UNSUPPORTED, "Float32 sort keys"); s.kind = SORT_F64; s.width = 8; s.enc_bytes = 8; }
      else if (t.is_unsigned_int()) { s.kind = SORT_UINT; s.width = t.arrow_width(); s.enc_bytes = s.width; }
      else { s.kind = SORT_INT; s.width = t.arrow_width(); s.enc_bytes = s.width; }
    }
    if (!str_keys.empty()) {
      unsigned int lens[8] = {0};
      SG_CUDA(cudaMemcpyAsync(lens, maxlen->ptr, sizeof(lens), cudaMemcpyDeviceToHost, ctx->stream));
      SG_CUDA(cudaStreamSynchronize(ctx->stream));
      for (int k : str_keys) {
        SG_CHECK(lens[k] <= 256, SAILGPU_ERR_UNSUPPORTED, "sort key strings longer than 256 bytes are not supported yet");
        E.cols[k].str_len = (int)lens[k]; E.cols[k].enc_bytes = (int)lens[k] + 4;
      }
    }
    for (size_t k = 0; k < ks.size(); ++k) { E.cols[k].out_off = off; off += 1 + E.cols[k].enc_bytes; }
    E.key_bytes = off;
    Encoded out;
    out.key_bytes = off;
    out.keys = dev_alloc(ctx, (size_t)n * off);
    out.bits = dev_alloc_zero(ctx, (size_t)off * 8);
    E.keys = static_cast<uint8_t*>(out.keys->ptr);
    E.bits = static_cast<uint32_t*>(out.bits->ptr);
    SG_CUDA(launch_sort_encode(E, ctx->stream));
    m.kernel_launches += 1;
    return out;
  }

  BatchPtr take_rows(const BatchPtr& all, const Schema& sch, const int64_t* idx, int64_t take) {
    auto out = std::make_shared<DevBatch>();
    out->rows = take;
    JoinOp helper; helper.ctx = ctx;
    for (size_t i = 0; i < sch.size(); ++i) out->cols.push_back(helper.gather_column(all->cols[i], sch[i], idx, take, false));
    m.kernel_launches += sch.size();
    return out;
  }

  BatchPtr sort_rows(const BatchPtr& all, const Schema& sch, const std::vector<Key>& ks, int64_t limit) {
    const int64_t n = all->rows;
    if (n == 0) return all;
    SG_CHECK(n < (1ll << 32), SAILGPU_ERR_UNSUPPORTED, "sort of more than 2^32 rows in one partition");
    Encoded enc = encode_keys(all, sch, ks);
    const int64_t n_chunks = (n + 2047) / 2048;
    BufPtr ia = dev_alloc(ctx, (size_t)n * 4), ib = dev_alloc(ctx, (size_t)n * 4), ka = dev_alloc(ctx, (size_t)n * 8), kbuf = dev_alloc(ctx, (size_t)n * 8),
           hist = dev_alloc(ctx, (size_t)n_chunks * 256 * 4), offs = dev_alloc(ctx, (size_t)n_chunks * 256 * 8), scr = dev_alloc(ctx, 1026 * 8);
    RadixScratch S;
    S.idx_a = static_cast<uint32_t*>(ia->ptr); S.idx_b = static_cast<uint32_t*>(ib->ptr);
    S.kw_a = static_cast<uint64_t*>(ka->ptr); S.kw_b = static_cast<uint64_t*>(kbuf->ptr);
    S.hist = static_cast<uint32_t*>(hist->ptr); S.offs = static_cast<uint64_t*>(offs->ptr); S.scan_scratch = static_cast<uint64_t*>(scr->ptr);
    int sort_launches = 0;
    SG_CUDA(radix_sort_indices(static_cast<const uint8_t*>(enc.keys->ptr), enc.key_bytes, n, S, static_cast<const uint32_t*>(enc.bits->ptr), ctx->stream, &sort_launches));
    m.kernel_launches += (uint64_t)(sort_launches + 1);
    const int64_t take = limit >= 0 ? std::min<int64_t>(limit, n) : n;
    BufPtr idx = dev_alloc(ctx, (size_t)take * 8);
    SG_CUDA(launch_widen_u32(static_cast<const uint32_t*>(ia->ptr), static_cast<int64_t*>(idx->ptr), take, ctx->stream));
    BatchPtr out = take_rows(all, sch, static_cast<const int64_t*>(idx->ptr), take);
    SG_CUDA(cudaStreamSynchronize(ctx->stream));
    return out;
  }

  static constexpr int64_t TOPK_MIN_ROWS = 1 << 18, TOPK_MAX_K = 1 << 16;
  BatchPtr topk_rows(const BatchPtr& all, const Schema& sch, const std::vector<Key>& ks, int64_t k) {
    const int64_t n = all->rows;
    Encoded enc = encode_keys(all, sch, ks);
    const uint8_t* kp = static_cast<const uint8_t*>(enc.keys->ptr);
    const int total_bits = std::min(64, enc.key_bytes * 8);
    const int64_t want_at_most = std::max<int64_t>(4 * k, 1 << 16);
    BufPtr hist = dev_alloc(ctx, 2048 * 4);
    std::vector<uint32_t> h(2048);
    int used = 0;
    uint64_t prefix = 0;
    int64_t below = 0, cand = n;
    while (used < total_bits && below + cand > want_at_most) {
      const int db = std::min(11, total_bits - used);
      SG_CUDA(cudaMemsetAsync(hist->ptr, 0, 2048 * 4, ctx->stream));
      SG_CUDA(launch_topk_hist(kp, enc.key_bytes, n, used, prefix, db, static_cast<uint32_t*>(hist->ptr), ctx->stream));
      SG_CUDA(cudaMemcpyAsync(h.data(), hist->ptr, 2048 * 4, cudaMemcpyDeviceToHost, ctx->stream));
      SG_CUDA(cudaStreamSynchronize(ctx->stream));
      m.kernel_launches += 1;
      int64_t run = below;
      int bin = 0;
      for (; bin < (1 << db); ++bin) { if (run + h[(size_t)bin] >= k) break; run += h[(size_t)bin]; }
      if (bin == (1 << db)) bin = (1 << db) - 1;
      below = run; cand = h[(size_t)bin];
      prefix = (prefix << db) | (uint64_t)bin;
      used += db;
    }
    if (below + cand > std::max<int64_t>(want_at_most, n / 4)) return nullptr;
    BufPtr idx = dev_alloc(ctx, (size_t)(below + cand) * 8), ctr = dev_alloc_zero(ctx, 8);
    SG_CUDA(launch_topk_compact(kp, enc.key_bytes, n, used, prefix, static_cast<int64_t*>(idx->ptr), static_cast<unsigned long long*>(ctr->ptr), ctx->stream));
    m.kernel_launches += 1;
    const int64_t nc = below + cand;
    BatchPtr sub = take_rows(all, sch, static_cast<const int64_t*>(idx->ptr), nc);
    DevColumn rowno; rowno.type = T(TypeId::Int64); rowno.length = nc; rowno.data = idx;
    sub->cols.push_back(rowno);
    Schema sch2 = sch;
    sch2.push_back({"__row", T(TypeId::Int64), false});
    std::vector<Key> ks2 = ks;
    auto re = std::make_shared<Expr>(); re->kind = Expr::Col; re->col = (int)sch.size(); re->type = T(TypeId::Int64); re->nullable = false;
    ks2.push_back({re, true, true});
    BatchPtr sorted = sort_rows(sub, sch2, ks2, k);
    sorted->cols.pop_back();
    return sorted;
  }

  BatchPtr run() {
    const Schema& sch = in_schemas[0];
    BatchPtr all = concat_batches(ctx, sch, parts);
    parts.clear();
    const int64_t n = all->rows;
    if (n == 0) return all;
// ... 22 lines not shown
    SG_CHECK(input >= 0 && input < (int)done_in.size(), SAILGPU_ERR_INVALID, "merge input index out of range");
    done_in[(size_t)input] = true;
    input_done = true;
    for (bool d : done_in) input_done = input_done && d;
  }
  bool pull(BatchPtr* out) override {
    *out = nullptr;
    if (!input_done) return true;
    if (emitted) return false;
    const uint64_t t0 = now_ns();
    *out = merge();
    emitted = true;
    m.elapsed_compute_ns += now_ns() - t0;
    m.output_rows += (uint64_t)(*out)->rows; m.output_batches++;
    return false;
  }

  BatchPtr merge() {
    const Schema& sch = in_schemas[0];
    std::vector<BatchPtr> runs;
    for (auto& in : per_input) {
      if (in.empty()) continue;
      if (runs_are_batches) for (auto& b : in) runs.push_back(b);
      else runs.push_back(in.size() == 1 ? in[0] : concat_batches(ctx, sch, in));
    }
    per_input.clear();
    if (runs.empty()) return empty_batch(ctx, sch);
    if (fetch >= 0)
      for (auto& r : runs)
        if (r->rows > fetch) {
          BufPtr idx = dev_alloc(ctx, (size_t)fetch * 8);
          SG_CUDA(launch_iota(static_cast<int64_t*>(idx->ptr), fetch, ctx->stream));
          r = take_rows(r, sch, static_cast<const int64_t*>(idx->ptr), fetch);
          SG_CUDA(cudaStreamSynchronize(ctx->stream));
        }
    if (runs.size() == 1) return runs[0];
    std::vector<int64_t> off(runs.size() + 1, 0);
    for (size_t i = 0; i < runs.size(); ++i) off[i + 1] = off[i] + runs[i]->rows;
    BatchPtr all = concat_batches(ctx, sch, runs);
    const int64_t n = all->rows;
    Encoded enc = encode_keys(all, sch, keys);
    BufPtr doff = dev_alloc(ctx, off.size() * 8), perm = dev_alloc(ctx, (size_t)n * 8);
    SG_CUDA(cudaMemcpyAsync(doff->ptr, off.data(), off.size() * 8, cudaMemcpyHostToDevice, ctx->stream));
    SG_CUDA(launch_merge_rank(static_cast<const uint8_t*>(enc.keys->ptr), enc.key_bytes, static_cast<const int64_t*>(doff->ptr), (int)runs.size(), n,
                              static_cast<int64_t*>(perm->ptr), ctx->stream));
    m.kernel_launches += 1;
    const int64_t take = fetch >= 0 ? std::min<int64_t>(fetch, n) : n;
    BatchPtr out = take_rows(all, sch, static_cast<const int64_t*>(perm->ptr), take);
    SG_CUDA(cudaStreamSynchronize(ctx->stream));
    return out;
  }
};

static void parse_sort_keys(SortOp* op, const Json& spec, const Schema& in) {
  for (auto& k : spec.at("keys").a) {
    SortOp::Key key;
    key.e = parse_expr(k.at("expr"), in);
    const Json* asc = k.find("asc"); key.asc = !asc || asc->kind != Json::Bool || asc->b;
    const Json* nf = k.find("nulls_first"); key.nulls_first = nf && nf->kind == Json::Bool ? nf->b : key.asc;
    op->keys.push_back(key);
  }
  SG_CHECK(!op->keys.empty() && op->keys.size() <= 7, SAILGPU_ERR_INVALID, "sort needs 1..7 keys");
  for (auto& k : op->keys) {
    SG_CHECK(k.e->kind == Expr::Col, SAILGPU_ERR_UNSUPPORTED, "sort keys must be column references");
    SG_CHECK(k.e->type.id != TypeId::Float32, SAILGPU_ERR_UNSUPPORTED, "Float32 sort keys");
  }
  const Json* f = spec.find("fetch");
  if (f && !f->is_null()) op->fetch = f->as_int();
}

std::unique_ptr<Op> make_merge_op(Ctx* ctx, const Json& spec, const std::vector<Schema>& inputs) {
  SG_CHECK(!inputs.empty(), SAILGPU_ERR_INVALID, "sort_preserving_merge takes one input per sorted partition");
  for (auto& s : inputs) {
    SG_CHECK(s.size() == inputs[0].size(), SAILGPU_ERR_INVALID, "sort_preserving_merge inputs differ in schema");
    for (size_t i = 0; i < s.size(); ++i) SG_CHECK(s[i].type == inputs[0][i].type, SAILGPU_ERR_INVALID, "sort_preserving_merge inputs differ in schema");
  }
  auto op = std::make_unique<MergeOp>();
  op->ctx = ctx; op->kind = "sort_preserving_merge"; op->in_schemas = inputs; op->out_schema = inputs[0];
  parse_sort_keys(op.get(), spec, inputs[0]);
  const Json* r = spec.find("runs");
  op->runs_are_batches = r && !r->is_null() && r->as_str() == "batches";
  op->per_input.resize(inputs.size());
// ... 56 lines not shown
  BatchPtr run() {
    const Schema& in = in_schemas[0];
    if (parts.empty()) return empty_batch(ctx, out_schema);
    BatchPtr all = parts.size() == 1 ? parts[0] : concat_batches(ctx, in, parts);
    parts.clear();
    const int64_t n = all->rows;
    SG_CHECK(n < (1ll << 32), SAILGPU_ERR_UNSUPPORTED, "sort-based grouping of more than 2^32 rows in one partition");
    const Json& gb = spec.at("group_by");
    std::vector<Json> kex;
    for (size_t i = 0; i < gb.a.size(); ++i) kex.push_back(jobj({{"expr", gb.a[i].at("expr")}, {"name", jstr("__k" + std::to_string(i))}}));
    Schema ks;
    BatchPtr kb = through(jobj({{"op", jstr("projection")}, {"exprs", jarr(kex)}}), in, all, &ks);
    SortOp so; so.ctx = ctx;
    std::vector<SortOp::Key> keys;
    for (int i = 0; i < n_keys; ++i) keys.push_back({parse_expr(jcol(i), ks), true, true});
    SortOp::Encoded enc = so.encode_keys(kb, ks, keys);
    const int64_t n_chunks = (n + 2047) / 2048;
    BufPtr ia = dev_alloc(ctx, (size_t)n * 4), ib = dev_alloc(ctx, (size_t)n * 4), ka = dev_alloc(ctx, (size_t)n * 8), kbuf = dev_alloc(ctx, (size_t)n * 8),
           hist = dev_alloc(ctx, (size_t)n_chunks * 256 * 4), offs = dev_alloc(ctx, (size_t)n_chunks * 256 * 8), scr = dev_alloc(ctx, 1026 * 8);
    RadixScratch S;
    S.idx_a = static_cast<uint32_t*>(ia->ptr); S.idx_b = static_cast<uint32_t*>(ib->ptr);
    S.kw_a = static_cast<uint64_t*>(ka->ptr); S.kw_b = static_cast<uint64_t*>(kbuf->ptr);
    S.hist = static_cast<uint32_t*>(hist->ptr); S.offs = static_cast<uint64_t*>(offs->ptr); S.scan_scratch = static_cast<uint64_t*>(scr->ptr);
    int sort_launches = 0;
    BufPtr hk = dev_alloc(ctx, (size_t)n * 8), all_bits = dev_alloc(ctx, 16 * 4), coll = dev_alloc_zero(ctx, 8);
    SG_CUDA(cudaMemsetAsync(all_bits->ptr, 0xFF, 16 * 4, ctx->stream));
    SG_CUDA(launch_key_hash(static_cast<const uint8_t*>(enc.keys->ptr), enc.key_bytes, n, static_cast<uint8_t*>(hk->ptr), ctx->stream));
    SG_CUDA(radix_sort_indices(static_cast<const uint8_t*>(hk->ptr), 8, n, S, static_cast<const uint32_t*>(all_bits->ptr), ctx->stream, &sort_launches));
    BufPtr heads = dev_alloc(ctx, (size_t)n * 4), before = dev_alloc(ctx, (size_t)n * 8), scr2 = dev_alloc(ctx, 1026 * 8);
    SG_CUDA(launch_group_heads(static_cast<const uint8_t*>(enc.keys->ptr), enc.key_bytes, S.idx_a, n, static_cast<uint32_t*>(heads->ptr),
                               static_cast<const uint8_t*>(hk->ptr), static_cast<unsigned long long*>(coll->ptr), ctx->stream));
    unsigned long long n_coll = 0;
    SG_CUDA(cudaMemcpyAsync(&n_coll, coll->ptr, 8, cudaMemcpyDeviceToHost, ctx->stream));
    SG_CUDA(cudaStreamSynchronize(ctx->stream));
    if (n_coll != 0 || getenv("SAILGPU_WIDEAGG_FULL_SORT") != nullptr) {
      int more = 0;
      SG_CUDA(radix_sort_indices(static_cast<const uint8_t*>(enc.keys->ptr), enc.key_bytes, n, S, static_cast<const uint32_t*>(enc.bits->ptr), ctx->stream, &more));
      SG_CUDA(launch_group_heads(static_cast<const uint8_t*>(enc.keys->ptr), enc.key_bytes, S.idx_a, n, static_cast<uint32_t*>(heads->ptr), nullptr, nullptr, ctx->stream));
      sort_launches += more + 1;
    }
    SG_CUDA(launch_exclusive_scan_u32(static_cast<const uint32_t*>(heads->ptr), n, static_cast<uint64_t*>(before->ptr), static_cast<uint64_t*>(scr2->ptr), ctx->stream));
    uint64_t n_groups = 0;
    SG_CUDA(cudaMemcpyAsync(&n_groups, static_cast<uint64_t*>(scr2->ptr) + std::min<int64_t>(1024, (n + 4095) / 4096), 8, cudaMemcpyDeviceToHost, ctx->stream));
    SG_CUDA(cudaStreamSynchronize(ctx->stream));
    DevColumn gid; gid.type = T(TypeId::Int64); gid.length = n; gid.data = dev_alloc(ctx, (size_t)n * 8);
    BufPtr rep = dev_alloc(ctx, (size_t)n_groups * 8);
    SG_CUDA(launch_assign_groups(S.idx_a, static_cast<const uint32_t*>(heads->ptr), static_cast<const uint64_t*>(before->ptr), n,
                                 static_cast<int64_t*>(gid.data->ptr), static_cast<int64_t*>(rep->ptr), ctx->stream));
    m.kernel_launches += (uint64_t)sort_launches + 4;
    auto agg_in = std::make_shared<DevBatch>();
    agg_in->rows = n;
    Schema ain;
    Field gf; gf.name = "__gid"; gf.type = T(TypeId::Int64); gf.nullable = false;
    int gid_col = 0;
    if (merging) {
      ain.push_back(gf); agg_in->cols.push_back(gid);
      for (size_t i = (size_t)n_keys; i < in.size(); ++i) { ain.push_back(in[i]); agg_in->cols.push_back(all->cols[i]); }
    } else {
      ain = in; agg_in->cols = all->cols;
      gid_col = (int)in.size();
      ain.push_back(gf); agg_in->cols.push_back(gid);
    }
    std::vector<std::pair<std::string, Json>> so2;
    for (auto& kv : spec.o) {
      if (kv.first == "group_by") so2.push_back({"group_by", jarr({jobj({{"expr", jcol(gid_col)}, {"name", jstr("__gid")}})})});
      else so2.push_back(kv);
    }
    Schema aos;
    BatchPtr agg = through(jobj(so2), ain, agg_in, &aos);
    SG_CHECK((uint64_t)agg->rows == n_groups, SAILGPU_ERR_STATE, "sort-based grouping: group count mismatch");
    JoinOp helper; helper.ctx = ctx;
    DevColumn repc; repc.type = T(TypeId::Int64); repc.length = (int64_t)n_groups; repc.data = rep;
    DevColumn pick = helper.gather_column(repc, gf, static_cast<const int64_t*>(agg->cols[0].data->ptr), agg->rows, false);
    auto out = std::make_shared<DevBatch>();
    out->rows = agg->rows;
    for (int i = 0; i < n_keys; ++i) {
      DevColumn c = helper.gather_column(kb->cols[(size_t)i], ks[(size_t)i], static_cast<const int64_t*>(pick.data->ptr), agg->rows, false);
      out->cols.push_back(c);
    }
    for (size_t i = 1; i < agg->cols.size(); ++i) out->cols.push_back(agg->cols[i]);
    m.kernel_launches += (uint64_t)n_keys + 1;
    SG_CUDA(cudaStreamSynchronize(ctx->stream));
    return out;
  }
};

std::unique_ptr<Op> make_wide_agg_op(Ctx* ctx, const Json& spec, const std::vector<Schema>& inputs, const Schema& out_schema) {
  auto op = std::make_unique<WideAggOp>();
  op->ctx = ctx; op->kind = "aggregate"; op->in_schemas = inputs; op->out_schema = out_schema; op->spec = spec;
  op->n_keys = (int)spec.at("group_by").a.size();
  const std::string mode = spec.at("mode").as_str();
  op->merging = mode == "final" || mode == "final_partitioned";
  SG_CHECK(op->n_keys >= 1 && op->n_keys <= 7, SAILGPU_ERR_UNSUPPORTED, "sort-based grouping takes 1 to 7 group keys");
  for (int i = 0; i < op->n_keys; ++i) {
    const DataType& t = out_schema[(size_t)i].type;
    SG_CHECK(t.id != TypeId::Float32, SAILGPU_ERR_UNSUPPORTED, "Float32 group keys");
  }
  return op;
}

struct RepartitionOp : Op {
  int n_parts = 1;
  std::vector<ExprPtr> exprs;
  PipelineRunner run;
  std::vector<std::deque<BatchPtr>> ready;
  bool input_done = false;
  int rr = 0;
  bool row_round_robin = false;
  int64_t next_idx = 0;

  void partition_round_robin(const BatchPtr& b) {
    const int64_t n = b->rows;
    JoinOp helper; helper.ctx = ctx;
    for (int p = 0; p < n_parts; ++p) {
      const int64_t first = ((int64_t)p - next_idx % n_parts + n_parts) % n_parts;
      if (first >= n) continue;
      const int64_t k = (n - first + n_parts - 1) / n_parts;
      BufPtr idx = dev_alloc(ctx, (size_t)k * 8);
      SG_CUDA(launch_iota_stride(static_cast<int64_t*>(idx->ptr), first, n_parts, k, ctx->stream));
      auto pb = std::make_shared<DevBatch>();
      pb->rows = k;
      for (size_t c = 0; c < b->cols.size(); ++c) pb->cols.push_back(helper.gather_column(b->cols[c], in_schemas[0][c], static_cast<const int64_t*>(idx->ptr), k, false));
      m.kernel_launches += 1 + b->cols.size();
      ready[(size_t)p].push_back(pb);
    }
    next_idx = (next_idx + n) % n_parts;
    SG_CUDA(cudaStreamSynchronize(ctx->stream));
  }

  void push(int input, const BatchPtr& b) override {
    SG_CHECK(input == 0, SAILGPU_ERR_INVALID, "repartition has one input");
    const uint64_t t0 = now_ns();
    m.input_rows += (uint64_t)b->rows; m.input_batches++;
    if (b->rows && row_round_robin) partition_round_robin(b);
    else if (b->rows) partition(b);
    m.elapsed_compute_ns += now_ns() - t0;
  }
  void finish(int) override { input_done = true; }
  bool pull(BatchPtr* out) override {
    *out = nullptr;
    for (int t = 0; t < n_parts; ++t) {
      const int p = (rr + t) % n_parts;
      if (!ready[(size_t)p].empty()) { *out = ready[(size_t)p].front(); ready[(size_t)p].pop_front(); rr = p + 1; break; }
    }
    bool any = false; for (auto& q : ready) any |= !q.empty();
    if (*out) { m.output_rows += (uint64_t)(*out)->rows; m.output_batches++; }
    return any || !input_done;
  }
  bool pull_partition(int p, BatchPtr* out) override {
    SG_CHECK(p >= 0 && p < n_parts, SAILGPU_ERR_INVALID, "partition index out of range");
    *out = nullptr;
    if (!ready[(size_t)p].empty()) { *out = ready[(size_t)p].front(); ready[(size_t)p].pop_front(); m.output_rows += (uint64_t)(*out)->rows; m.output_batches++; }
    return !ready[(size_t)p].empty() || !input_done;
  }

  void partition(const BatchPtr& b) {
    auto cp = run.compiled_for(*b);
    const int64_t n = b->rows;
    BufPtr counts = dev_alloc_zero(ctx, (size_t)n_parts * 8), offsets = dev_alloc(ctx, (size_t)n_parts * 8);
    PipelineAux aux; memset(&aux, 0, sizeof(aux));
    aux.part.n_parts = n_parts;
    aux.part.n_keys = (int)cp->keys.size();
    for (size_t i = 0; i < cp->keys.size(); ++i) aux.part.keys[i] = cp->keys[i];
    aux.part.part_counts = static_cast<unsigned long long*>(counts->ptr);
    aux.part.part_offsets = static_cast<const int64_t*>(offsets->ptr);
    aux.part.pid_slot = NO_SLOT;
    aux.part.smem_off = cp->scratch_off;
    PipelineParams P;
    run.prepare(P, *cp, *b, 0, n);
    P.n_out = 0;
    aux.part.pass = 0;
    run.launch(P, cp, &aux, m);
    std::vector<int64_t> cnt((size_t)n_parts), off((size_t)n_parts);
    SG_CUDA(cudaMemcpyAsync(cnt.data(), counts->ptr, (size_t)n_parts * 8, cudaMemcpyDeviceToHost, ctx->stream));
    SG_CUDA(cudaStreamSynchronize(ctx->stream));
    int64_t run_off = 0;
    for (int p = 0; p < n_parts; ++p) { off[(size_t)p] = run_off; run_off += cnt[(size_t)p]; }
    SG_CUDA(cudaMemcpyAsync(offsets->ptr, off.data(), (size_t)n_parts * 8, cudaMemcpyHostToDevice, ctx->stream));
    SG_CUDA(cudaMemsetAsync(counts->ptr, 0, (size_t)n_parts * 8, ctx->stream));
    run.prepare(P, *cp, *b, 0, n);
    P.n_out = (int)cp->outs.size();
    std::vector<DevColumn> cols;
    std::vector<BufPtr> vbytes((size_t)P.n_out), bbytes((size_t)P.n_out);
    std::vector<BufPtr> heaps;
    for (auto& c : b->cols) if (c.type.is_string()) for (auto& h : c.heaps) heaps.push_back(h);
    for (int j = 0; j < P.n_out; ++j) {
      OutputCol o = cp->outs[(size_t)j];
      DevColumn c; c.type = cp->out_types[(size_t)j]; c.arrow_is_utf8 = c.type.id == TypeId::Utf8;
      if (o.width) { c.data = dev_alloc(ctx, (size_t)n * o.width); o.data = static_cast<uint8_t*>(c.data->ptr); }
      else { bbytes[(size_t)j] = dev_alloc(ctx, (size_t)n + 4); o.data = static_cast<uint8_t*>(bbytes[(size_t)j]->ptr); }
      if (o.valid_slot != NO_SLOT) { vbytes[(size_t)j] = dev_alloc(ctx, (size_t)n + 4); o.valid_bytes = static_cast<uint8_t*>(vbytes[(size_t)j]->ptr); }
      if (c.type.is_string()) c.heaps = heaps;
      P.out[j] = o;
      cols.push_back(c);
    }
    aux.part.pass = 1;
    run.launch(P, cp, &aux, m);
    check_device_error(ctx, run.scal.error());
    for (int p = 0; p < n_parts; ++p) {
      const int64_t o = off[(size_t)p], k = cnt[(size_t)p];
      if (k == 0) continue;
      auto pb = std::make_shared<DevBatch>();
      pb->rows = k;
      for (int j = 0; j < P.n_out; ++j) {
        DevColumn c = cols[(size_t)j];
        c.length = k;
        if (bbytes[(size_t)j]) {
          c.data = dev_alloc_zero(ctx, (size_t)((k + 31) / 32 * 4));
          SG_CUDA(launch_pack_bytes(static_cast<const uint8_t*>(bbytes[(size_t)j]->ptr) + o, static_cast<uint32_t*>(c.data->ptr), k, nullptr, ctx->stream));
        } else {
          auto view = std::make_shared<DevBuf>();
          const int w = c.type.is_string() ? 16 : c.type.arrow_width();
          view->ptr = static_cast<uint8_t*>(cols[(size_t)j].data->ptr) + o * w; view->bytes = (size_t)k * w;
          BufPtr keep = cols[(size_t)j].data;
          view->on_release = [keep] {};
          c.data = view;
        }
        if (vbytes[(size_t)j]) {
          c.validity = dev_alloc_zero(ctx, (size_t)((k + 31) / 32 * 4));
          SG_CUDA(launch_pack_bytes(static_cast<const uint8_t*>(vbytes[(size_t)j]->ptr) + o, static_cast<uint32_t*>(c.validity->ptr), k, nullptr, ctx->stream));
          c.null_count = -1;
        }
        pb->cols.push_back(c);
      }
      ready[(size_t)p].push_back(pb);
    }
    SG_CUDA(cudaStreamSynchronize(ctx->stream));
  }
};

std::unique_ptr<Op> make_repartition_op(Ctx* ctx, const Json& spec, const std::vector<Schema>& inputs) {
  SG_CHECK(inputs.size() == 1, SAILGPU_ERR_INVALID, "repartition takes one input");
  auto op = std::make_unique<RepartitionOp>();
  op->ctx = ctx; op->kind = "repartition"; op->in_schemas = inputs; op->out_schema = inputs[0];
  const Json* sch = spec.find("scheme");
  const std::string scheme = sch ? sch->as_str() : "hash";
  SG_CHECK(scheme == "hash" || scheme == "round_robin_row", SAILGPU_ERR_UNSUPPORTED,
           "repartition scheme '" + scheme + "': Partitioning::Hash and the row round-robin of ExplicitRepartitionExec run on the GPU; "
           "RoundRobinBatch only re-labels whole batches and stays with the reference's stream plumbing (SURVEY.md 8b)");
  op->n_parts = (int)spec.at("n").as_int();
  SG_CHECK(op->n_parts >= 1 && op->n_parts <= 4096, SAILGPU_ERR_INVALID, "partition count out of range");
  if (scheme == "round_robin_row") {
    const Json* ip = spec.find("input_partition"); const Json* np = spec.find("num_input_partitions");
    const int64_t in_part = ip && !ip->is_null() ? ip->as_int() : 0, n_in = np && !np->is_null() ? np->as_int() : 1;
    SG_CHECK(n_in >= 1 && in_part >= 0 && in_part < n_in, SAILGPU_ERR_INVALID, "input_partition / num_input_partitions out of range");
    op->row_round_robin = true;
    op->next_idx = (in_part * op->n_parts) / n_in;
    op->ready.resize((size_t)op->n_parts);
    return op;
  }
  for (auto& e : spec.at("exprs").a) op->exprs.push_back(parse_expr(e, inputs[0]));
  SG_CHECK(!op->exprs.empty() && (int)op->exprs.size() <= MAX_KEYS, SAILGPU_ERR_INVALID, "hash repartition needs 1.." + std::to_string(MAX_KEYS) + " key expressions");
  op->ready.resize((size_t)op->n_parts);
  op->run.init(ctx, inputs[0]);
  auto* raw = op.get();
  op->run.custom_sink = [raw](PipelineCompiler& pc, CompiledPipeline& cp) {
    pc.finish_partition(cp, raw->exprs);
    cp.extra_scratch = (uint32_t)(raw->n_parts * 16 + 16);
  };
  return op;
}


BatchPtr exchange_batches(Ctx* ctx, const Schema& schema, const std::vector<BatchPtr>& parts, std::vector<int64_t>* source_offsets = nullptr, int64_t abort_above_rows = -1);
std::unique_ptr<Op> make_repartition_op(Ctx* ctx, const Json& spec, const std::vector<Schema>& inputs);

struct ExchangeOp : Op {
  std::string mode = "gather";
  int root = 0;
  int64_t small_rows = 1 << 14;
  Json exprs_json;
  std::vector<BatchPtr> parts_in;
  BatchPtr result;
  bool done = false, pulled = false;
  bool* on_root_hint = nullptr;
  bool keep_runs = false;
  std::deque<BatchPtr> run_batches;

  void split_runs(const std::vector<int64_t>& off) {
    JoinOp helper; helper.ctx = ctx;
    const Schema& sch = in_schemas[0];
    for (size_t s = 0; s + 1 < off.size(); ++s) {
      const int64_t k = off[s + 1] - off[s];
      if (k == 0) continue;
      if (k == result->rows) { run_batches.push_back(result); continue; }
      BufPtr idx = dev_alloc(ctx, (size_t)k * 8);
      SG_CUDA(launch_iota_stride(static_cast<int64_t*>(idx->ptr), off[s], 1, k, ctx->stream));
      auto b = std::make_shared<DevBatch>();
      b->rows = k;
      for (size_t c = 0; c < sch.size(); ++c) b->cols.push_back(helper.gather_column(result->cols[c], sch[c], static_cast<const int64_t*>(idx->ptr), k, false));
      SG_CUDA(cudaStreamSynchronize(ctx->stream));
      run_batches.push_back(b);
    }
    if (run_batches.empty()) run_batches.push_back(result);
  }

  void push(int input, const BatchPtr& b) override {
    SG_CHECK(input == 0, SAILGPU_ERR_INVALID, "exchange has one input");
    m.input_rows += (uint64_t)b->rows; m.input_batches++;
    if (b->rows) parts_in.push_back(b);
  }
  void finish(int) override {
    const uint64_t t0 = now_ns();
    const Schema& sch = in_schemas[0];
    BatchPtr all = parts_in.empty() ? empty_batch(ctx, sch) : concat_batches(ctx, sch, parts_in);
    parts_in.clear();
    const int W = ctx->world;
    if (W == 1) { result = all; done = true; if (keep_runs) run_batches.push_back(result); return; }
    std::vector<int64_t> src_off;
    if (mode == "gather" && on_root_hint && *on_root_hint) {
      result = all; done = true; if (keep_runs) run_batches.push_back(result); return;
    }
    std::vector<BatchPtr> parts((size_t)W);
    bool sent = false;
    if (mode == "gather" || mode == "auto") {
      for (int p = 0; p < W; ++p) parts[(size_t)p] = p == root ? all : empty_batch(ctx, sch);
      result = exchange_batches(ctx, sch, parts, keep_runs ? &src_off : nullptr, mode == "auto" ? small_rows : -1);
      sent = result != nullptr;
      if (on_root_hint) *on_root_hint = sent && mode == "auto";
    }
    if (!sent) {
      if (on_root_hint) *on_root_hint = false;
      Json spec; spec.kind = Json::Obj;
      Json opk; opk.kind = Json::Str; opk.s = "repartition";
// ... 153 lines not shown
BatchPtr exchange_batches(Ctx* ctx, const Schema& schema, const std::vector<BatchPtr>& parts, std::vector<int64_t>* source_offsets, int64_t abort_above_rows) {
  const int n = (int)parts.size();
  SG_CHECK(n == ctx->world, SAILGPU_ERR_INVALID, "exchange needs one batch per rank");
  if (n == 1) { if (source_offsets) *source_offsets = {0, parts[0]->rows}; return parts[0]; }
  SG_CHECK(ctx->nccl_comm != nullptr, SAILGPU_ERR_STATE, "sailgpu_ctx_comm_init has not been called");
  const int W = n, me = ctx->rank;
  const size_t ncols = schema.size();
  const size_t rec = 1 + 2 * ncols;
  std::vector<int64_t> mine((size_t)W * rec, 0);
  struct Pending { int p; size_t ci; BufPtr offs, scratch; int64_t nblocks; };
  std::vector<Pending> pend;
  for (int p = 0; p < W; ++p) {
    mine[(size_t)p * rec] = parts[(size_t)p]->rows;
    for (size_t ci = 0; ci < ncols; ++ci) {
      const DevColumn& col = parts[(size_t)p]->cols[ci];
      const int64_t k = col.length;
      mine[(size_t)p * rec + 1 + ncols + ci] = (k > 0 && col.validity) ? 1 : 0;
      if (schema[ci].type.is_string() && k > 0) {
        BufPtr lens = dev_alloc(ctx, (size_t)k * 4), offs = dev_alloc(ctx, (size_t)k * 8), scratch = dev_alloc(ctx, 1026 * 8);
        SG_CUDA(launch_view_lengths(col.data->ptr, k, static_cast<uint32_t*>(lens->ptr), 0, ctx->stream));
        SG_CUDA(launch_exclusive_scan_u32(static_cast<uint32_t*>(lens->ptr), k, static_cast<uint64_t*>(offs->ptr), static_cast<uint64_t*>(scratch->ptr), ctx->stream));
        pend.push_back({p, ci, offs, scratch, std::min<int64_t>(1024, (k + 4095) / 4096)});
      }
    }
  }
  BufPtr dmine = dev_alloc(ctx, mine.size() * 8), dall = dev_alloc(ctx, mine.size() * 8 * (size_t)W);
  SG_CUDA(cudaMemcpyAsync(dmine->ptr, mine.data(), mine.size() * 8, cudaMemcpyHostToDevice, ctx->stream));
  for (auto& q : pend)
    SG_CUDA(cudaMemcpyAsync(static_cast<int64_t*>(dmine->ptr) + (size_t)q.p * rec + 1 + q.ci, static_cast<uint64_t*>(q.scratch->ptr) + q.nblocks, 8,
                            cudaMemcpyDeviceToDevice, ctx->stream));
  NCCL_CALL(g_nccl.AllGather(dmine->ptr, dall->ptr, mine.size(), NCCL_INT64, ctx->nccl_comm, ctx->stream));
  std::vector<int64_t> all(mine.size() * (size_t)W);
  SG_CUDA(cudaMemcpyAsync(all.data(), dall->ptr, all.size() * 8, cudaMemcpyDeviceToHost, ctx->stream));
  SG_CUDA(cudaStreamSynchronize(ctx->stream));
  auto cnt = [&](int src, int dst, size_t field) { return all[((size_t)src * W + dst) * rec + field]; };
  if (abort_above_rows >= 0) {
    int64_t mx = 0;
    for (int s = 0; s < W; ++s) { int64_t r = 0; for (int d = 0; d < W; ++d) r += cnt(s, d, 0); mx = std::max(mx, r); }
    if (mx > abort_above_rows) return nullptr;
  }
  auto vneed = [&](int dst, size_t ci) { for (int s = 0; s < W; ++s) if (cnt(s, dst, 1 + ncols + ci)) return true; return false; };
  struct SendCol { BufPtr data, validity_bytes, heap; int64_t heap_bytes = 0; };
  std::vector<std::vector<SendCol>> sc((size_t)W, std::vector<SendCol>(ncols));
  for (int p = 0; p < W; ++p)
    for (size_t ci = 0; ci < ncols; ++ci) {
      const DevColumn& col = parts[(size_t)p]->cols[ci];
      SendCol& sd = sc[(size_t)p][ci];
      const int64_t k = col.length;
      if (k == 0) continue;
      if (schema[ci].type.id == TypeId::Bool) {
        sd.data = dev_alloc(ctx, (size_t)k);
        SG_CUDA(launch_unpack_bits(static_cast<const uint8_t*>(col.data->ptr), static_cast<uint8_t*>(sd.data->ptr), k, 0, ctx->stream));
      } else if (!schema[ci].type.is_string()) sd.data = col.data;
      if (vneed(p, ci)) {
        sd.validity_bytes = dev_alloc(ctx, (size_t)k);
        if (col.validity) SG_CUDA(launch_unpack_bits(static_cast<const uint8_t*>(col.validity->ptr), static_cast<uint8_t*>(sd.validity_bytes->ptr), k, 0, ctx->stream));
        else SG_CUDA(cudaMemsetAsync(sd.validity_bytes->ptr, 1, (size_t)k, ctx->stream));
      }
    }
  for (auto& q : pend) {
    const DevColumn& col = parts[(size_t)q.p]->cols[q.ci];
    SendCol& sd = sc[(size_t)q.p][q.ci];
    const int64_t k = col.length;
    sd.heap_bytes = cnt(me, q.p, 1 + q.ci);
    sd.heap = dev_alloc(ctx, (size_t)sd.heap_bytes);
    sd.data = dev_alloc(ctx, (size_t)k * 16);
    SG_CUDA(cudaMemcpyAsync(sd.data->ptr, col.data->ptr, (size_t)k * 16, cudaMemcpyDeviceToDevice, ctx->stream));
// ... 183 lines not shown
```

sail_b200/csrc/parquet.cu:

```cuda
#include <cstring>

#include "device.hpp"
#include "h2d.hpp"
#include "kernels.hpp"

namespace sg {

namespace {

struct TReader {
  const uint8_t* p; const uint8_t* end;
  int16_t last = 0;
  uint64_t varint() {
    uint64_t v = 0; int sh = 0;
    for (;;) {
      SG_CHECK(p < end && sh < 64, SAILGPU_ERR_INVALID, "parquet: truncated page header");
      const uint8_t b = *p++;
      v |= (uint64_t)(b & 0x7F) << sh;
      if (!(b & 0x80)) return v;
      sh += 7;
    }
  }
  int64_t zigzag() { const uint64_t v = varint(); return (int64_t)(v >> 1) ^ -(int64_t)(v & 1); }
  bool field(int* id, int* type) {
// ... 320 lines not shown
  return P;
}

DevColumn decode_parquet_column(Ctx* ctx, const Field& f, const ParquetColumnDesc& c, int64_t n_rows) {
  ColumnPlan P = plan_parquet_column(f, c, n_rows);
  const uint8_t* base = c.chunk;
  const int pt = c.physical_type;
  const bool is_str = P.is_str;
  const int out_width = P.out_width;
  std::vector<Run>& level_runs = P.level_runs; std::vector<Run>& index_runs = P.index_runs;
  std::vector<Segment>& segs = P.segs;
  std::vector<uint64_t>& str_off = P.str_off;
  const int64_t dense_done = P.dense, dict_count = P.dict_count, dict_len = P.dict_len;
  const uint8_t* dict_bytes = P.dict_bytes;
  const bool any_dict_page = P.any_dict_page, any_plain_page = P.any_plain_page;
  DevColumn col; col.type = f.type; col.length = n_rows;
  BufPtr dchunk = dev_alloc(ctx, (size_t)c.chunk_len + 64);
  {
    HostStager st(ctx);
    st.add_raw(dchunk->ptr, c.chunk, (size_t)c.chunk_len);
    st.flush();
  }
  const uint8_t* dbase = static_cast<const uint8_t*>(dchunk->ptr);
  BufPtr err = dev_alloc_zero(ctx, 8);
  auto expand = [&](const std::vector<Run>& runs, int64_t n) -> BufPtr {
    BufPtr out = dev_alloc(ctx, (size_t)n * 4 + 16);
    if (n == 0) return out;
    std::vector<int64_t> starts(runs.size());
    for (size_t i = 0; i < runs.size(); ++i) starts[i] = runs[i].out_start;
    BufPtr druns = upload_vec(ctx, runs.data(), runs.size() * sizeof(Run)), dstarts = upload_vec(ctx, starts.data(), starts.size() * 8);
    expand_runs_kernel<<<(int)std::min<int64_t>((n + 255) / 256, grid_cap(8)), 256, 0, ctx->stream>>>(dbase, static_cast<const Run*>(druns->ptr), static_cast<const int64_t*>(dstarts->ptr),
                                                                                                (int)runs.size(), n, static_cast<uint32_t*>(out->ptr));
    SG_CUDA(cudaGetLastError());
    SG_CUDA(cudaStreamSynchronize(ctx->stream));
    return out;
  };
  DecodeParams D; memset(&D, 0, sizeof(D));
  D.chunk = dbase; D.n_rows = n_rows; D.physical = pt; D.type_length = c.type_length; D.out_width = out_width; D.is_view = is_str ? 1 : 0;
  D.error = static_cast<uint32_t*>(err->ptr);
  BufPtr valid, vpos, scratch, didx, ddict, dsegs, dstr;
  if (c.max_def_level > 0) {
    valid = expand(level_runs, n_rows);
    vpos = dev_alloc(ctx, (size_t)(n_rows + 1) * 8);
    scratch = dev_alloc(ctx, 1026 * 8);
    SG_CUDA(launch_exclusive_scan_u32(static_cast<const uint32_t*>(valid->ptr), n_rows, static_cast<uint64_t*>(vpos->ptr), static_cast<uint64_t*>(scratch->ptr), ctx->stream));
    D.valid = static_cast<const uint32_t*>(valid->ptr); D.vpos = static_cast<const uint64_t*>(vpos->ptr);
  }
  if (any_dict_page) {
    DecodeParams Q; memset(&Q, 0, sizeof(Q));
    Q.chunk = dbase; Q.n_rows = dict_count; Q.physical = pt; Q.type_length = c.type_length; Q.out_width = out_width; Q.is_view = D.is_view; Q.error = D.error;
    std::vector<Segment> ds{Segment{0, (int64_t)(dict_bytes - base), 0}};
    std::vector<uint64_t> doff;
    BufPtr qsegs, qoff;
    if (is_str) {
      const uint8_t* q = dict_bytes;
      for (int64_t i = 0; i < dict_count; ++i) {
        SG_CHECK(q + 4 <= dict_bytes + dict_len, SAILGPU_ERR_INVALID, "parquet: dictionary value overruns its page");
        uint32_t len; memcpy(&len, q, 4);
        doff.push_back((uint64_t)(q - base));
        q += 4 + (size_t)len;
      }
      qoff = upload_vec(ctx, doff.data(), doff.size() * 8);
      Q.str_off = static_cast<const uint64_t*>(qoff->ptr);
    }
    qsegs = upload_vec(ctx, ds.data(), sizeof(Segment));
    Q.segs = static_cast<const Segment*>(qsegs->ptr); Q.n_segs = 1;
    ddict = dev_alloc(ctx, (size_t)std::max<int64_t>(dict_count, 1) * out_width);
    if (dict_count) decode_values_kernel<<<(int)std::min<int64_t>((dict_count + 255) / 256, grid_cap(4)), 256, 0, ctx->stream>>>(Q, static_cast<uint8_t*>(ddict->ptr));
    SG_CUDA(cudaGetLastError());
    SG_CUDA(cudaStreamSynchronize(ctx->stream));
    didx = expand(index_runs, dense_done);
    D.dict_idx = static_cast<const uint32_t*>(didx->ptr); D.dict_vals = static_cast<const uint8_t*>(ddict->ptr); D.dict_size = (uint32_t)dict_count;
  }
  if (is_str && any_plain_page) {
    str_off.resize((size_t)dense_done, 0);
    dstr = upload_vec(ctx, str_off.data(), str_off.size() * 8);
    D.str_off = static_cast<const uint64_t*>(dstr->ptr);
  }
  if (segs.empty()) segs.push_back(Segment{0, 0, 0});
  dsegs = upload_vec(ctx, segs.data(), segs.size() * sizeof(Segment));
  D.segs = static_cast<const Segment*>(dsegs->ptr); D.n_segs = (int)segs.size();
  col.data = dev_alloc(ctx, (size_t)n_rows * out_width);
  if (n_rows) decode_values_kernel<<<(int)std::min<int64_t>((n_rows + 255) / 256, grid_cap(8)), 256, 0, ctx->stream>>>(D, static_cast<uint8_t*>(col.data->ptr));
  SG_CUDA(cudaGetLastError());
  if (is_str) col.heaps = {dchunk};
  col.null_count = 0;
  if (c.max_def_level > 0 && dense_done < n_rows) {
    BufPtr bytes = dev_alloc(ctx, (size_t)n_rows + 4);
    SG_CUDA(launch_u32_to_bytes(static_cast<const uint32_t*>(valid->ptr), static_cast<uint8_t*>(bytes->ptr), n_rows, ctx->stream));
    col.validity = dev_alloc_zero(ctx, (size_t)((n_rows + 31) / 32 * 4));
    SG_CUDA(launch_pack_bytes(static_cast<const uint8_t*>(bytes->ptr), static_cast<uint32_t*>(col.validity->ptr), n_rows, nullptr, ctx->stream));
    col.null_count = n_rows - dense_done;
  }
  uint32_t e = 0;
  SG_CUDA(cudaMemcpyAsync(&e, err->ptr, 4, cudaMemcpyDeviceToHost, ctx->stream));
  SG_CUDA(cudaStreamSynchronize(ctx->stream));
  SG_CHECK(e == 0, SAILGPU_ERR_INVALID, "parquet: dictionary index out of range in column '" + f.name + "'");
  return col;
}

std::string parquet_plan_summary(const Field& f, const ParquetColumnDesc& c, int64_t n_rows) {
  ColumnPlan P = plan_parquet_column(f, c, n_rows);
  int64_t level_vals = 0, index_vals = 0;
  for (auto& r : P.level_runs) level_vals += r.count;
  for (auto& r : P.index_runs) index_vals += r.count;
  char b[512];
  snprintf(b, sizeof b, "{\"pages\":%lld,\"dense\":%lld,\"dict_count\":%lld,\"level_values\":%lld,\"index_values\":%lld,\"level_runs\":%zu,\"index_runs\":%zu,"
                        "\"plain_strings\":%zu,\"dict_pages\":%d,\"plain_pages\":%d}",
           (long long)P.n_pages, (long long)P.dense, (long long)P.dict_count, (long long)level_vals, (long long)index_vals, P.level_runs.size(), P.index_runs.size(),
           P.str_off.size(), P.any_dict_page ? 1 : 0, P.any_plain_page ? 1 : 0);
  return b;
}

}
```

sail_b200/csrc/relational.cu:

```cuda
#include <cuda_runtime.h>
#include <stdint.h>

#include <algorithm>
#include <vector>

#include "dev_util.cuh"
#include "kernels.hpp"
#include "relational.hpp"

namespace sg {

__device__ __forceinline__ bool col_is_null(const RawKeyCol& k, int64_t row) {
  return k.validity_bits && !((k.validity_bits[row >> 3] >> (row & 7)) & 1);
}
__device__ __forceinline__ uint64_t raw_key_hash(const RawKeyCol* keys, int n_keys, int64_t row, bool* has_null) {
  uint64_t h = 0x243F6A8885A308D3ull;
  *has_null = false;
  for (int i = 0; i < n_keys; ++i) {
    const RawKeyCol& k = keys[i];
    if (col_is_null(k, row)) { *has_null = true; return 0; }
    const uint8_t* p = k.data + row * k.stride;
    if (k.width == 16) {
      ulonglong2 v = *reinterpret_cast<const ulonglong2*>(p);
      h = mix64(h ^ (k.is_view ? view_hash(v) : mix64(v.x ^ mix64(v.y))));
// ... 210 lines not shown
    const bool in = i < b1;
    const uint64_t w = in ? kw_in[i] : 0;
    const uint32_t row = in ? (idx_in ? idx_in[i] : (uint32_t)i) : 0;
    const uint32_t d = in ? (uint32_t)((w >> shift) & 255u) : 0x100u + lane;
    const unsigned peers = __match_any_sync(0xFFFFFFFFu, d);
    const int rank = __popc(peers & ((1u << lane) - 1));
    uint64_t pos = 0;
    if (in) pos = base[d] + rank;
    __syncwarp();
    if (in && rank == __popc(peers) - 1) base[d] += __popc(peers);
    __syncwarp();
    if (in) { kw_out[pos] = w; idx_out[pos] = row; }
  }
}

__global__ void iota_u32_kernel(uint32_t* out, int64_t n) {
  for (int64_t i = blockIdx.x * (int64_t)blockDim.x + threadIdx.x; i < n; i += (int64_t)gridDim.x * blockDim.x) out[i] = (uint32_t)i;
}

__global__ void small_sort_kernel(const uint8_t* __restrict__ keys, int key_bytes, int n, uint32_t* __restrict__ idx_out) {
  const int i = threadIdx.x;
  if (i >= n) return;
  const uint8_t* ki = keys + (int64_t)i * key_bytes;
  int rank = 0;
  for (int j = 0; j < n; ++j) {
    const uint8_t* kj = keys + (int64_t)j * key_bytes;
    int c = 0;
    for (int b = 0; b < key_bytes && c == 0; ++b) c = (int)kj[b] - (int)ki[b];
    rank += (c < 0 || (c == 0 && j < i)) ? 1 : 0;
  }
  idx_out[rank] = (uint32_t)i;
}

cudaError_t radix_sort_indices(const uint8_t* keys, int key_bytes, int64_t n, const RadixScratch& S, const uint32_t* bits, cudaStream_t s, int* launches) {
  int nl = 0;
  if (launches) *launches = 0;
  if (n == 0) return cudaSuccess;
  if (n <= 1024) { small_sort_kernel<<<1, 1024, 0, s>>>(keys, key_bytes, (int)n, S.idx_a); if (launches) *launches = 1; return cudaGetLastError(); }
  std::vector<uint32_t> hb((size_t)key_bytes * 2);
  cudaError_t e = cudaMemcpyAsync(hb.data(), bits, hb.size() * 4, cudaMemcpyDeviceToHost, s);
  if (e != cudaSuccess) return e;
  e = cudaStreamSynchronize(s);
  if (e != cudaSuccess) return e;
  auto trivial = [&](int d) { return (hb[(size_t)d] & hb[(size_t)key_bytes + d] & 0xFFu) == 0; };
  const int64_t n_chunks = (n + RADIX_CHUNK - 1) / RADIX_CHUNK;
  const int blocks = (int)((n_chunks + 7) / 8);
  const int flat = (int)std::min<int64_t>((n + 255) / 256, grid_cap(8));
  const uint32_t* in_idx = nullptr;
  uint32_t* out_idx = S.idx_a;
  uint64_t* kw_in = S.kw_a; uint64_t* kw_out = S.kw_b;
  for (int hi = key_bytes; hi > 0;) {
    const int lo = std::max(0, hi - 8);
    bool any = false;
    for (int d = lo; d < hi; ++d) any |= !trivial(d);
    if (any) {
      radix_gather_word_kernel<<<flat, 256, 0, s>>>(keys, key_bytes, lo, hi - lo, in_idx, n, kw_in); ++nl;
      for (int d = hi - 1; d >= lo; --d) {
        if (trivial(d)) continue;
        const int shift = 8 * (hi - 1 - d);
        radix_hist_kernel<<<blocks, 256, 0, s>>>(kw_in, shift, n, S.hist, n_chunks);
        e = launch_exclusive_scan_u32(S.hist, 256 * n_chunks, S.offs, S.scan_scratch, s);
        if (e != cudaSuccess) return e;
        radix_scatter_kernel<<<blocks, 256, 0, s>>>(kw_in, in_idx, kw_out, out_idx, shift, n, S.offs, n_chunks);
        nl += 5;
        std::swap(kw_in, kw_out);
        in_idx = out_idx;
// ... 172 lines not shown
```

sail_b200/csrc/relational.hpp:

```cpp
#pragma once
#include <cuda_runtime.h>
#include <stdint.h>

#include "vm.h"

namespace sg {

struct RawKeyCol {
  const uint8_t* data;
  const uint8_t* validity_bits;
  int32_t width;
  int32_t is_view;
  int32_t stride;
  int32_t pad;
};

struct JoinMultiParams {
  int64_t n_probe;
  int32_t n_keys;
  int32_t pass;
  int32_t emit_unmatched_probe;
  int32_t pad;
  RawKeyCol probe_keys[MAX_KEYS];
  RawKeyCol build_keys[MAX_KEYS];
// ... 7 lines not shown
  const int64_t* next;
};

enum SortKind : int32_t { SORT_INT = 0, SORT_UINT = 1, SORT_F64 = 2, SORT_BOOL = 3, SORT_VIEW = 4 };
struct SortKeyCol {
  const uint8_t* data;
  const uint8_t* validity_bits;
  int32_t kind, width;
  int32_t asc, nulls_first;
  int32_t out_off;
  int32_t enc_bytes;
  int32_t str_len;
  int32_t pad;
};
struct SortEncodeParams {
  int64_t n;
  int32_t n_keys, key_bytes;
  uint8_t* keys;
  uint32_t* bits;
  SortKeyCol cols[8];
};
struct RadixScratch {
  uint32_t *idx_a, *idx_b;
  uint64_t *kw_a, *kw_b;
  uint32_t* hist;
  uint64_t* offs;
  uint64_t* scan_scratch;
};

cudaError_t launch_join_multi(const JoinMultiParams& P, cudaStream_t s);
cudaError_t launch_gather_bits(const uint8_t* bits, uint8_t* out, const int64_t* idx, int64_t n, int dflt, cudaStream_t s);
cudaError_t launch_max_view_len(const void* views, int64_t n, unsigned int* out, cudaStream_t s);
cudaError_t launch_sort_encode(const SortEncodeParams& P, cudaStream_t s);
cudaError_t radix_sort_indices(const uint8_t* keys, int key_bytes, int64_t n, const RadixScratch& S, const uint32_t* bits, cudaStream_t s, int* launches);
cudaError_t launch_topk_hist(const uint8_t* keys, int key_bytes, int64_t n, int used, uint64_t prefix, int digit_bits, uint32_t* hist , cudaStream_t s);
cudaError_t launch_topk_compact(const uint8_t* keys, int key_bytes, int64_t n, int used, uint64_t threshold, int64_t* out, unsigned long long* counter, cudaStream_t s);
cudaError_t launch_merge_rank(const uint8_t* keys, int key_bytes, const int64_t* run_off, int n_runs, int64_t n, int64_t* perm, cudaStream_t s);
cudaError_t launch_key_hash(const uint8_t* keys, int key_bytes, int64_t n, uint8_t* out8, cudaStream_t s);
cudaError_t launch_group_heads(const uint8_t* keys, int key_bytes, const uint32_t* idx, int64_t n, uint32_t* heads, const uint8_t* hashes,
                               unsigned long long* collisions, cudaStream_t s);
cudaError_t launch_assign_groups(const uint32_t* idx, const uint32_t* heads, const uint64_t* before, int64_t n, int64_t* gid_of_row, int64_t* rep, cudaStream_t s);
cudaError_t launch_iota(int64_t* out, int64_t n, cudaStream_t s);
cudaError_t launch_iota_stride(int64_t* out, int64_t first, int64_t stride, int64_t n, cudaStream_t s);
cudaError_t launch_widen_u32(const uint32_t* in, int64_t* out, int64_t n, cudaStream_t s);
struct CopySeg { const uint8_t* src; uint8_t* dst; unsigned long long bytes; };
cudaError_t launch_multi_copy_raw(const CopySeg* dev_segs, int n, cudaStream_t s);
cudaError_t launch_rebase_views(void* views, int64_t n, uint64_t heap_base, cudaStream_t s);

}
```

sail_b200/csrc/runner.hpp:

```cpp
#pragma once
#include <algorithm>

#include "engine.hpp"
#include "jit.hpp"

namespace sg {

inline uint64_t now_ns() {
  return (uint64_t)std::chrono::duration_cast<std::chrono::nanoseconds>(std::chrono::steady_clock::now().time_since_epoch()).count();
}
struct Trace {
  Ctx* ctx; const char* what; uint64_t t0; bool on;
  Trace(Ctx* c, const char* w) : ctx(c), what(w), on(getenv("SAILGPU_TRACE") != nullptr) { if (on) { cudaStreamSynchronize(ctx->stream); t0 = now_ns(); } }
  ~Trace() { if (on) { cudaStreamSynchronize(ctx->stream); fprintf(stderr, "[sailgpu trace] %-28s %8.3f ms\n", what, (now_ns() - t0) / 1e6); } }
};

inline uint64_t next_pow2(uint64_t v) { uint64_t p = 1; while (p < v) p <<= 1; return p; }

struct DevProgram {
  BufPtr literals;
  std::vector<uint64_t> literal_ptrs;
};

inline bool timing_enabled() { static const bool on = getenv("SAILGPU_TIMING") != nullptr; return on; }
// ... 64 lines not shown
      } else if (st.kind == StageSpec::Projection) {
        pc.set_exprs(st.exprs);
      } else {
        pc.finish_aggregate(*cp, st);
        agg = true;
      }
    }
    if (!agg) { if (custom_sink) custom_sink(pc, *cp); else pc.finish_store_or_compact(*cp); }
    int hot = 0;
    if (agg) hot = cp->agg.n_keys == 0 ? 1 : hot_wanted;
    pc.finalize(*cp, ctx, hot);
    cache[cache_key] = cp;
    if (getenv("SAILGPU_DUMP")) dump_pipeline(*cp);
    return cp;
  }

  DevProgram& program_for(const std::shared_ptr<CompiledPipeline>& cp) {
    auto& programs = shared_state->programs;
    auto it = programs.find(cp.get());
    if (it == programs.end()) {
      DevProgram dp;
      size_t lit_bytes = 0;
      for (auto& s : cp->literals) lit_bytes += (s.size() + 15) & ~(size_t)15;
      dp.literals = dev_alloc(ctx, lit_bytes + 16);
      std::vector<uint8_t> blob(lit_bytes + 16, 0);
      size_t off = 0;
      for (auto& s : cp->literals) {
        memcpy(blob.data() + off, s.data(), s.size());
        dp.literal_ptrs.push_back(reinterpret_cast<uint64_t>(dp.literals->ptr) + off);
        off += (s.size() + 15) & ~(size_t)15;
      }
      if (!cp->literals.empty()) {
        SG_CUDA(cudaMemcpyAsync(dp.literals->ptr, blob.data(), blob.size(), cudaMemcpyHostToDevice, ctx->stream));
        SG_CUDA(cudaStreamSynchronize(ctx->stream));
      }
      for (auto& fx : cp->literal_fixups) cp->prog[(size_t)fx.first].imm1 = dp.literal_ptrs[(size_t)fx.second];
      it = programs.emplace(cp.get(), std::move(dp)).first;
    }
    return it->second;
  }

  void prepare(PipelineParams& P, const CompiledPipeline& cp, const DevBatch& b, int64_t row0, int64_t nrows) {
    ensure_scratch();
    memset(&P, 0, sizeof(P));
    P.n_rows = nrows;
    P.tile_rows = cp.rpt * NT;
    P.n_inputs = (int)cp.inputs.size();
    P.n_inst = (int)cp.prog.size();
    P.sink = cp.sink;
    P.arena_bytes = cp.arena_bytes;
    P.mask_slot = cp.mask_slot;
    P.error_flag = scal.error();
    P.n_probes = cp.n_probes;
    bool tma = getenv("SAILGPU_NO_TMA") == nullptr;
    SG_CHECK(row0 % 1024 == 0, SAILGPU_ERR_INVALID, "chunk offset must be a multiple of 1024 rows");
    for (size_t i = 0; i < cp.inputs.size(); ++i) {
      const InputReg& r = cp.inputs[i];
      const DevColumn& c = b.cols[(size_t)r.col];
      const uint8_t* base = static_cast<const uint8_t*>(r.validity ? c.validity->ptr : c.data->ptr);
      base += r.width ? row0 * r.width : row0 / 8;
      P.in[i].data = base;
      P.in[i].slot = (uint32_t)r.slot;
      P.in[i].width = r.width;
      P.in[i].tma_ok = (reinterpret_cast<uint64_t>(base) & 15) == 0 ? 1 : 0;
      tma &= P.in[i].tma_ok != 0;
    }
    P.use_tma = tma ? 1 : 0;
// ... 111 lines not shown
    P.out[j] = o;
    out->cols.push_back(c);
  }
  BufPtr status;
  if (compact && tile_offsets) {
    P.tile_offsets = tile_offsets;
  } else if (compact) {
    const int64_t n_tiles = (n + P.tile_rows - 1) / P.tile_rows;
    status = dev_alloc_zero(ctx, (size_t)(n_tiles + 1) * 8);
    P.tile_status = static_cast<unsigned long long*>(status->ptr);
    P.ticket = run.scal.ticket();
    P.out_count = run.scal.out_count();
    SG_CUDA(cudaMemsetAsync(static_cast<uint8_t*>(run.scal.buf->ptr) + 8, 0, 16, ctx->stream));
  }
  run.launch(P, cp, aux_host, m);
  int64_t out_rows = n;
  if (compact) {
    unsigned long long cnt = (unsigned long long)known_out_rows;
    if (!tile_offsets) SG_CUDA(cudaMemcpyAsync(&cnt, run.scal.out_count(), 8, cudaMemcpyDeviceToHost, ctx->stream));
    check_device_error(ctx, run.scal.error());
    out_rows = (int64_t)cnt;
    for (int j = 0; j < P.n_out; ++j) {
      DevColumn& c = out->cols[(size_t)j];
      if (bool_tmp[(size_t)j]) {
        c.data = dev_alloc_zero(ctx, (size_t)((out_rows + 31) / 32 * 4));
        SG_CUDA(launch_pack_bytes(static_cast<const uint8_t*>(bool_tmp[(size_t)j]->ptr), static_cast<uint32_t*>(c.data->ptr), out_rows, nullptr, ctx->stream));
      }
      if (valid_tmp[(size_t)j]) {
        c.validity = dev_alloc_zero(ctx, (size_t)((out_rows + 31) / 32 * 4));
        SG_CUDA(launch_pack_bytes(static_cast<const uint8_t*>(valid_tmp[(size_t)j]->ptr), static_cast<uint32_t*>(c.validity->ptr), out_rows, nullptr, ctx->stream));
        c.null_count = -1;
      }
    }
    if (!bool_tmp.empty() || !valid_tmp.empty()) SG_CUDA(cudaStreamSynchronize(ctx->stream));
  } else {
    check_device_error(ctx, run.scal.error());
  }
  out->rows = out_rows;
  for (auto& c : out->cols) c.length = out_rows;
  return out;
}


}
```

Before: 25.02 billion.

## Cut host syncs in aggregation with pinned counters, batched view export, small sort

Replaces the per-batch host read of the aggregation group and deferred-row counters with an asynchronous copy into mapped pinned memory, using double-buffered slots, events and an in-flight queue. Host-to-device stalls between batches should shrink. The change also batches the string-view max-length checks during export, adds a single-block small multi-column sort kernel, and counts host syncs as a new metric. The added complexity risks ordering bugs between the counter slots and the deferred reset.

```diff
diff --git a/sail_b200/csrc/capi.cu b/sail_b200/csrc/capi.cu
--- a/sail_b200/csrc/capi.cu
+++ b/sail_b200/csrc/capi.cu
@@ -35,6 +35,11 @@
   }
 }
 void set_device(const Ctx& c) { SG_CUDA(cudaSetDevice(c.device)); }
+struct SyncCharge {
+  sailgpu_op* h; uint64_t s0;
+  explicit SyncCharge(sailgpu_op* op) : h(op), s0(op->owner->ctx.host_syncs.load()) {}
+  ~SyncCharge() { if (h->op) h->op->m.host_syncs += h->owner->ctx.host_syncs.load() - s0; }
+};
 using CtxLock = std::lock_guard<std::recursive_mutex>;
 }
 
@@ -90,6 +95,7 @@
   c->ctx.shared_objects.clear();
   c->ctx.dead.store(true);
   if (c->ctx.stream) { cudaStreamSynchronize(c->ctx.stream); cudaStreamDestroy(c->ctx.stream); c->ctx.stream = nullptr; }
+  if (c->ctx.pinned_block) { cudaFreeHost(c->ctx.pinned_block); c->ctx.pinned_block = nullptr; }
   destroy_pack_pool(&c->ctx);
 }
 
@@ -116,7 +122,9 @@
     for (int i = 0; i < n_inputs; ++i) ins.push_back(schema_from_arrow(input_schemas[i]));
     auto h = std::make_unique<sailgpu_op>();
     h->owner = c;
+    const uint64_t s0 = c->ctx.host_syncs.load();
     h->op = make_op(&c->ctx, spec, ins, partition);
+    h->op->m.host_syncs += c->ctx.host_syncs.load() - s0;
     h->input_finished.assign((size_t)n_inputs, false);
     schema_to_arrow(h->op->out_schema, out_schema);
     *out = h.release();
@@ -192,6 +200,7 @@
   if (!h) return SAILGPU_ERR_INVALID;
   return guard(&h->last_error, [&] {
     CtxLock lk(h->owner->ctx.mu);
+    SyncCharge charge(h);
     set_device(h->owner->ctx);
     SG_CHECK(input_idx >= 0 && input_idx < (int)h->op->in_schemas.size(), SAILGPU_ERR_INVALID, "input index out of range");
     SG_CHECK(!h->input_finished[(size_t)input_idx], SAILGPU_ERR_STATE, "push after finish_input");
@@ -204,6 +213,7 @@
   if (!h) return SAILGPU_ERR_INVALID;
   return guard(&h->last_error, [&] {
     CtxLock lk(h->owner->ctx.mu);
+    SyncCharge charge(h);
     set_device(h->owner->ctx);
     SG_CHECK(input_idx >= 0 && input_idx < (int)h->op->in_schemas.size(), SAILGPU_ERR_INVALID, "input index out of range");
     SG_CHECK(!h->input_finished[(size_t)input_idx], SAILGPU_ERR_STATE, "push after finish_input");
@@ -220,6 +230,7 @@
   if (!h) return SAILGPU_ERR_INVALID;
   return guard(&h->last_error, [&] {
     CtxLock lk(h->owner->ctx.mu);
+    SyncCharge charge(h);
     set_device(h->owner->ctx);
     SG_CHECK(input_idx >= 0 && input_idx < (int)h->op->in_schemas.size(), SAILGPU_ERR_INVALID, "input index out of range");
     if (h->input_finished[(size_t)input_idx]) return;
@@ -233,6 +244,7 @@
   if (!h) return SAILGPU_ERR_INVALID;
   return guard(&h->last_error, [&] {
     CtxLock lk(h->owner->ctx.mu);
+    SyncCharge charge(h);
     set_device(h->owner->ctx);
     SG_CHECK(has_more && (host_out || dev_out), SAILGPU_ERR_INVALID, "null argument");
     BatchPtr b;
@@ -285,7 +297,8 @@
                    "\"elapsed_compute\":%llu,\"build_input_rows\":%llu,\"build_input_batches\":%llu,\"build_time\":%llu,"
                    "\"join_time\":%llu,\"gpu.kernel_launches\":%llu,\"gpu.h2d_bytes\":%llu,\"gpu.d2h_bytes\":%llu,"
                    "\"gpu.pipeline_launches\":%llu,\"gpu.jit_launches\":%llu,\"gpu.pipeline_kernel_ns\":%llu,"
-                   "\"gpu.exchange_sent_bytes\":%llu,\"gpu.exchange_recv_bytes\":%llu,\"gpu.exchange_ns\":%llu,\"gpu.exchange_calls\":%llu}",
+                   "\"gpu.exchange_sent_bytes\":%llu,\"gpu.exchange_recv_bytes\":%llu,\"gpu.exchange_ns\":%llu,\"gpu.exchange_calls\":%llu,"
+                   "\"gpu.host_syncs\":%llu}",
                    (unsigned long long)m.output_rows, (unsigned long long)m.output_batches, (unsigned long long)m.input_rows,
                    (unsigned long long)m.input_batches, (unsigned long long)m.elapsed_compute_ns, (unsigned long long)m.build_input_rows,
                    (unsigned long long)m.build_input_batches, (unsigned long long)m.build_time_ns, (unsigned long long)m.join_time_ns,
@@ -293,7 +306,7 @@
                    (unsigned long long)h->owner->ctx.d2h_bytes.load(), (unsigned long long)h->op->m.pipeline_launches, (unsigned long long)h->op->m.jit_launches,
                    (unsigned long long)h->op->pipeline_kernel_ns(), (unsigned long long)h->owner->ctx.exch_sent_bytes.load(),
                    (unsigned long long)h->owner->ctx.exch_recv_bytes.load(), (unsigned long long)h->owner->ctx.exch_ns.load(),
-                   (unsigned long long)h->owner->ctx.exch_calls.load());
+                   (unsigned long long)h->owner->ctx.exch_calls.load(), (unsigned long long)m.host_syncs);
   if (json_buf && cap) { size_t k = std::min<size_t>((size_t)n, cap - 1); memcpy(json_buf, tmp, k); json_buf[k] = 0; }
   return n + 1;
 }
diff --git a/sail_b200/csrc/device.cu b/sail_b200/csrc/device.cu
--- a/sail_b200/csrc/device.cu
+++ b/sail_b200/csrc/device.cu
@@ -1,3 +1,4 @@
+#include <algorithm>
 #include <cstdlib>
 #include <cstring>
 
@@ -146,7 +147,7 @@
         doffs = borrow(offs, (size_t)(a->length + 1) * 4);
         int32_t last = 0;
         if (a->length) SG_CUDA(cudaMemcpyAsync(&last, offs + a->length, 4, cudaMemcpyDeviceToHost, stream));
-        SG_CUDA(cudaStreamSynchronize(stream));
+        stream_sync(ctx);
         dbytes = borrow(bytes, (size_t)last);
       } else {
         doffs = J.upload(offs, a->length + 1, 4);
@@ -171,7 +172,7 @@
       if (n_data > 0) {
         std::vector<int64_t> sizes((size_t)n_data);
         const int64_t* size_buf = static_cast<const int64_t*>(a->buffers[a->n_buffers - 1]);
-        if (on_device) { SG_CUDA(cudaMemcpyAsync(sizes.data(), size_buf, (size_t)n_data * 8, cudaMemcpyDeviceToHost, stream)); SG_CUDA(cudaStreamSynchronize(stream)); }
+        if (on_device) { SG_CUDA(cudaMemcpyAsync(sizes.data(), size_buf, (size_t)n_data * 8, cudaMemcpyDeviceToHost, stream)); stream_sync(ctx); }
         else std::memcpy(sizes.data(), size_buf, (size_t)n_data * 8);
         auto bases = std::make_shared<std::vector<uint64_t>>((size_t)n_data);
         for (int64_t k = 0; k < n_data; ++k) {
@@ -185,7 +186,7 @@
         J.after([=] {
           SG_CUDA(cudaMemcpyAsync(dbases->ptr, bases->data(), (size_t)n_data * 8, cudaMemcpyHostToDevice, stream));
           SG_CUDA(launch_resolve_views(vdata->ptr, n, static_cast<const uint64_t*>(dbases->ptr), stream));
-          SG_CUDA(cudaStreamSynchronize(stream));
+          stream_sync(ctx);
         });
         c.heaps.push_back(dbases);
       }
@@ -272,7 +273,7 @@
 }
 
 struct StringExport { BufPtr views_or_offsets, heap; int64_t heap_bytes = 0; };
-StringExport export_strings(Ctx* ctx, const DevColumn& c, bool as_utf8) {
+StringExport export_strings(Ctx* ctx, const DevColumn& c, bool as_utf8, bool inline_known) {
   StringExport out;
   const int64_t n = c.length;
   if (n == 0) {
@@ -280,12 +281,17 @@
     out.heap = dev_alloc(ctx, 0);
     return out;
   }
+  if (inline_known) {
+    out.views_or_offsets = c.data;
+    out.heap = dev_alloc(ctx, 0);
+    return out;
+  }
   if (!as_utf8) {
     BufPtr mx = dev_alloc_zero(ctx, 8);
     unsigned int max_len = 0;
     SG_CUDA(launch_max_view_len(c.data->ptr, n, static_cast<unsigned int*>(mx->ptr), ctx->stream));
     SG_CUDA(cudaMemcpyAsync(&max_len, mx->ptr, 4, cudaMemcpyDeviceToHost, ctx->stream));
-    SG_CUDA(cudaStreamSynchronize(ctx->stream));
+    stream_sync(ctx);
     if (max_len <= 12) {
       out.views_or_offsets = c.data;
       out.heap = dev_alloc(ctx, 0);
@@ -300,7 +306,7 @@
   const int64_t nblocks = std::min<int64_t>(1024, (n + 4095) / 4096);
   uint64_t total = 0;
   SG_CUDA(cudaMemcpyAsync(&total, static_cast<uint64_t*>(scratch->ptr) + nblocks, 8, cudaMemcpyDeviceToHost, ctx->stream));
-  SG_CUDA(cudaStreamSynchronize(ctx->stream));
+  stream_sync(ctx);
   out.heap_bytes = (int64_t)total;
   out.heap = dev_alloc(ctx, (size_t)total);
   if (as_utf8) {
@@ -343,7 +349,7 @@
   ctx->d2h_used = 0;
 }
 
-void export_column(Ctx* ctx, const Field& f, const DevColumn& c, ArrowArray* out, bool to_device) {
+void export_column(Ctx* ctx, const Field& f, const DevColumn& c, ArrowArray* out, bool to_device, bool inline_known = false) {
   auto* p = new ArrayPriv();
   const int64_t n = c.length;
   auto emit = [&](const BufPtr& b, size_t bytes) -> const void* {
@@ -355,7 +361,7 @@
   p->buffers.push_back(c.validity ? emit(c.validity, (size_t)((n + 7) / 8)) : nullptr);
   if (f.type.is_string()) {
     const bool as_utf8 = f.type.id == TypeId::Utf8;
-    StringExport s = export_strings(ctx, c, as_utf8);
+    StringExport s = export_strings(ctx, c, as_utf8, inline_known);
     if (as_utf8) {
       p->buffers.push_back(emit(s.views_or_offsets, (size_t)(n + 1) * 4));
       p->buffers.push_back(emit(s.heap, (size_t)s.heap_bytes));
@@ -391,13 +397,36 @@
   p->buffers.push_back(nullptr);
   p->children.resize(schema.size());
   p->child_ptrs.resize(schema.size());
+  std::vector<size_t> view_cols;
+  for (size_t i = 0; i < schema.size(); ++i)
+    if (schema[i].type.id == TypeId::Utf8View && b->cols[i].length > 0) view_cols.push_back(i);
+  const unsigned int* max_len = nullptr;
+  if (!view_cols.empty()) {
+    BufPtr mx = dev_alloc_zero(ctx, view_cols.size() * 4);
+    for (size_t k = 0; k < view_cols.size(); ++k)
+      SG_CUDA(launch_max_view_len(b->cols[view_cols[k]].data->ptr, b->cols[view_cols[k]].length, static_cast<unsigned int*>(mx->ptr) + k, ctx->stream));
+    max_len = static_cast<const unsigned int*>(to_host(ctx, mx->ptr, view_cols.size() * 4, p));
+  }
+  auto is_view = [&](size_t i) { return std::find(view_cols.begin(), view_cols.end(), i) != view_cols.end(); };
   for (size_t i = 0; i < schema.size(); ++i) {
     p->children[i].release = nullptr;
-    export_column(ctx, schema[i], b->cols[i], &p->children[i], false);
+    export_column(ctx, schema[i], b->cols[i], &p->children[i], false, is_view(i));
     p->child_ptrs[i] = &p->children[i];
   }
-  SG_CUDA(cudaStreamSynchronize(ctx->stream));
+  stream_sync(ctx);
   finish_small_d2h(ctx);
+  bool again = false;
+  for (size_t k = 0; k < view_cols.size(); ++k) {
+    if (max_len[k] <= 12) continue;
+    const size_t i = view_cols[k];
+    p->children[i].release(&p->children[i]);
+    export_column(ctx, schema[i], b->cols[i], &p->children[i], false, false);
+    again = true;
+  }
+  if (again) {
+    stream_sync(ctx);
+    finish_small_d2h(ctx);
+  }
   init_array(out, b->rows, 0, p);
   out->n_children = (int64_t)schema.size();
   out->children = p->child_ptrs.data();
@@ -421,7 +450,7 @@
       export_column(ctx, schema[i], b->cols[i], &p->children[i], true);
       p->child_ptrs[i] = &p->children[i];
     }
-    SG_CUDA(cudaStreamSynchronize(ctx->stream));
+    stream_sync(ctx);
     init_array(&out->array, b->rows, 0, p);
     out->array.n_children = (int64_t)schema.size();
     out->array.children = p->child_ptrs.data();
diff --git a/sail_b200/csrc/device.hpp b/sail_b200/csrc/device.hpp
--- a/sail_b200/csrc/device.hpp
+++ b/sail_b200/csrc/device.hpp
@@ -45,7 +45,32 @@
   size_t cached_bytes = 0;
   static constexpr size_t CACHE_LIMIT = 64ull << 30;
   static size_t size_class(size_t padded) { return padded <= (1u << 20) ? (padded + 511) & ~(size_t)511 : (padded + (1u << 20) - 1) & ~(size_t)((1u << 20) - 1); }
+  std::atomic<uint64_t> host_syncs{0};
+  static constexpr size_t PINNED_SLOT = 128, PINNED_SLOTS = 512;
+  void* pinned_block = nullptr;
+  std::vector<uint32_t> pinned_free;
+  uint32_t pinned_next = 0;
 };
+
+inline void stream_sync(Ctx* ctx) {
+  ctx->host_syncs++;
+  SG_CUDA(cudaStreamSynchronize(ctx->stream));
+}
+
+inline void* pinned_slot_acquire(Ctx* ctx) {
+  if (!ctx->pinned_block) {
+    if (cudaHostAlloc(&ctx->pinned_block, Ctx::PINNED_SLOT * Ctx::PINNED_SLOTS, cudaHostAllocMapped) != cudaSuccess) { cudaGetLastError(); ctx->pinned_block = nullptr; return nullptr; }
+  }
+  uint32_t i;
+  if (!ctx->pinned_free.empty()) { i = ctx->pinned_free.back(); ctx->pinned_free.pop_back(); }
+  else if (ctx->pinned_next < Ctx::PINNED_SLOTS) i = ctx->pinned_next++;
+  else return nullptr;
+  return static_cast<uint8_t*>(ctx->pinned_block) + (size_t)i * Ctx::PINNED_SLOT;
+}
+inline void pinned_slot_release(Ctx* ctx, void* p) {
+  if (!p || !ctx->pinned_block) return;
+  ctx->pinned_free.push_back((uint32_t)((static_cast<uint8_t*>(p) - static_cast<uint8_t*>(ctx->pinned_block)) / Ctx::PINNED_SLOT));
+}
 
 extern std::atomic<bool> g_exiting;
 
diff --git a/sail_b200/csrc/engine.cu b/sail_b200/csrc/engine.cu
--- a/sail_b200/csrc/engine.cu
+++ b/sail_b200/csrc/engine.cu
@@ -1,6 +1,13 @@
 #include "runner.hpp"
 
 namespace sg {
+
+__global__ void agg_counters_kernel(const unsigned long long* __restrict__ scal, unsigned long long* host, int words, unsigned long long* zero) {
+  if (threadIdx.x < words) host[threadIdx.x] = scal[threadIdx.x];
+  __threadfence_system();
+  __syncthreads();
+  if (threadIdx.x == 0 && zero) *zero = 0;
+}
 
 
 StageSpec parse_stage(const Json& j, const Schema& in, Schema* out) {
@@ -76,16 +83,20 @@
   return st;
 }
 
-void check_device_error(Ctx* ctx, uint32_t* dev_flag) {
-  uint32_t f = 0;
-  SG_CUDA(cudaMemcpyAsync(&f, dev_flag, 4, cudaMemcpyDeviceToHost, ctx->stream));
-  SG_CUDA(cudaStreamSynchronize(ctx->stream));
+void raise_device_error(Ctx* ctx, uint32_t* dev_flag, uint32_t f) {
   if (!f) return;
   SG_CUDA(cudaMemsetAsync(dev_flag, 0, 4, ctx->stream));
   if (f & ERR_DIV_ZERO) fail(SAILGPU_ERR_ARITHMETIC, "Divide by zero");
   if (f & ERR_OVERFLOW) fail(SAILGPU_ERR_ARITHMETIC, "Arithmetic overflow");
   if (f & ERR_TABLE_FULL) fail(SAILGPU_ERR_CUDA, "hash table overflow");
   fail(SAILGPU_ERR_UNSUPPORTED, "unsupported value encountered on device");
+}
+
+void check_device_error(Ctx* ctx, uint32_t* dev_flag) {
+  uint32_t f = 0;
+  SG_CUDA(cudaMemcpyAsync(&f, dev_flag, 4, cudaMemcpyDeviceToHost, ctx->stream));
+  stream_sync(ctx);
+  raise_device_error(ctx, dev_flag, f);
 }
 
 struct AggTable {
@@ -211,7 +222,7 @@
     SG_CUDA(launch_exclusive_scan_u32(static_cast<const uint32_t*>(counts->ptr), n_tiles + 1, static_cast<uint64_t*>(offs->ptr), static_cast<uint64_t*>(scratch->ptr), ctx->stream));
     unsigned long long total = 0;
     SG_CUDA(cudaMemcpyAsync(&total, static_cast<const uint64_t*>(offs->ptr) + n_tiles, 8, cudaMemcpyDeviceToHost, ctx->stream));
-    SG_CUDA(cudaStreamSynchronize(ctx->stream));
+    stream_sync(ctx);
     m.kernel_launches += 4;
     return run_streaming(sel_run, ctx, b2, m, nullptr, {}, static_cast<const unsigned long long*>(offs->ptr), (int64_t)total);
   }
@@ -227,16 +238,43 @@
   bool use_cold = false;
   int64_t rows_in_table = 0;
   int64_t known_groups = -1;
-  struct Pending { BatchPtr batch; std::shared_ptr<CompiledPipeline> cp; BufPtr deferred; int64_t n_tiles = 0; bool active = false; } pend;
-
-  unsigned long long* n_deferred_ptr() { return reinterpret_cast<unsigned long long*>(static_cast<uint8_t*>(run.scal.buf->ptr) + 40); }
-
-  uint64_t read_n_groups() {
-    run.ensure_scratch();
-    unsigned long long g = 0;
-    SG_CUDA(cudaMemcpyAsync(&g, run.scal.n_groups(), 8, cudaMemcpyDeviceToHost, ctx->stream));
-    SG_CUDA(cudaStreamSynchronize(ctx->stream));
-    return g;
+  struct InFlight { BatchPtr batch; std::shared_ptr<CompiledPipeline> cp; BufPtr deferred; int slot = 0; };
+  std::deque<InFlight> inflight;
+  int next_slot = 0;
+  struct Counters { uint32_t error; uint32_t pad_[5]; unsigned long long n_groups, cursor, n_def[2]; };
+  static_assert(sizeof(Counters) == 56, "counter copy layout");
+  Counters* counters = nullptr;
+  Counters* counters_dev = nullptr;
+  bool counters_pinned = false, next_zeroed = false;
+  cudaEvent_t copied[2] = {nullptr, nullptr};
+
+  ~PipelineOp() override {
+    if (g_exiting.load()) return;
+    for (cudaEvent_t e : copied) if (e) cudaEventDestroy(e);
+    if (counters_pinned) pinned_slot_release(ctx, counters); else delete[] counters;
+  }
+
+  unsigned long long* n_deferred_ptr(int slot) { return reinterpret_cast<unsigned long long*>(static_cast<uint8_t*>(run.scal.buf->ptr) + 40 + 8 * slot); }
+
+  void copy_counters(int slot, bool zero_next) {
+    if (!counters) {
+      static_assert(2 * sizeof(Counters) <= Ctx::PINNED_SLOT, "pinned slot too small");
+      counters = static_cast<Counters*>(pinned_slot_acquire(ctx));
+      counters_pinned = counters != nullptr;
+      if (counters_pinned) SG_CUDA(cudaHostGetDevicePointer(reinterpret_cast<void**>(&counters_dev), counters, 0));
+      else counters = new Counters[2];
+      for (auto& e : copied) SG_CUDA(cudaEventCreateWithFlags(&e, cudaEventDisableTiming));
+    }
+    if (counters_pinned) {
+      agg_counters_kernel<<<1, 32, 0, ctx->stream>>>(static_cast<const unsigned long long*>(run.scal.buf->ptr), reinterpret_cast<unsigned long long*>(&counters_dev[slot]),
+                                                     (int)(sizeof(Counters) / 8), zero_next ? n_deferred_ptr(slot ^ 1) : nullptr);
+      SG_CUDA(cudaGetLastError());
+      m.kernel_launches++;
+      next_zeroed = zero_next;
+    } else {
+      SG_CUDA(cudaMemcpyAsync(&counters[slot], run.scal.buf->ptr, sizeof(Counters), cudaMemcpyDeviceToHost, ctx->stream));
+    }
+    SG_CUDA(cudaEventRecord(copied[slot], ctx->stream));
   }
 
   void fill_table(AggParams& A) {
@@ -279,7 +317,7 @@
     }
   }
 
-  void launch_agg(const std::shared_ptr<CompiledPipeline>& cp, const DevBatch& b, const BufPtr& list, int64_t n_list, const BufPtr& deferred_out) {
+  void launch_agg(const std::shared_ptr<CompiledPipeline>& cp, const DevBatch& b, const BufPtr& list, int64_t n_list, const BufPtr& deferred_out, int slot) {
     PipelineParams P;
     run.prepare(P, *cp, b, 0, b.rows);
     if (list) { P.tile_list = static_cast<const uint32_t*>(list->ptr); P.n_list = n_list; }
@@ -288,9 +326,10 @@
     aux.agg = cp->agg;
     fill_table(aux.agg);
     if (deferred_out) {
-      SG_CUDA(cudaMemsetAsync(n_deferred_ptr(), 0, 8, ctx->stream));
+      if (!(next_zeroed && !list)) SG_CUDA(cudaMemsetAsync(n_deferred_ptr(slot), 0, 8, ctx->stream));
+      next_zeroed = false;
       aux.agg.deferred = static_cast<uint32_t*>(deferred_out->ptr);
-      aux.agg.n_deferred = n_deferred_ptr();
+      aux.agg.n_deferred = n_deferred_ptr(slot);
       const char* fl = getenv("SAILGPU_AGG_FIRST_LIMIT");
       aux.agg.group_limit = (!list && fl && *fl) ? (unsigned long long)atoll(fl) : ~0ull;
       run.group_limit_cap = (cp->cold_variant || list) ? ~0ull : HOT_GROUP_LIMIT;
@@ -350,8 +389,7 @@
       M.acc_src_word[j] = (int16_t)O.accs[src[(size_t)j]].word;
       M.seen_src[j] = N.accs[j].track_seen ? (O.accs[src[(size_t)j]].track_seen ? (int8_t)src[(size_t)j] : (int8_t)-1) : (int8_t)-2;
     }
-    check_device_error(ctx, run.scal.error());
-    const uint64_t groups = read_n_groups();
+    const uint64_t groups = current_groups();
     AggTable old = tab;
     build_occ(old, O);
     tab.direct = direct_eligible(N);
@@ -370,7 +408,6 @@
 
   void push_agg(const BatchPtr& b0) {
     Trace tr(ctx, "agg.push");
-    resolve_pending();
     if (b0->rows == 0) return;
     bool widened = false;
     const BatchPtr b = with_union_signature(b0, &widened);
@@ -385,49 +422,92 @@
     const int64_t tile_rows = (int64_t)cp->rpt * NT;
     const int64_t n_tiles = (b->rows + tile_rows - 1) / tile_rows;
     BufPtr deferred = grouped ? dev_alloc(ctx, (size_t)n_tiles * 4) : nullptr;
-    launch_agg(cp, *b, nullptr, 0, deferred);
+    const int slot = next_slot;
+    launch_agg(cp, *b, nullptr, 0, deferred, slot);
     rows_in_table += b->rows;
     known_groups = -1;
-    if (grouped) { pend.batch = b; pend.cp = cp; pend.deferred = deferred; pend.n_tiles = n_tiles; pend.active = true; }
-  }
-
-  void resolve_pending() {
-    if (!pend.active) return;
+    if (!grouped) return;
+    next_slot ^= 1;
+    copy_counters(slot, true);
+    inflight.push_back({b, cp, deferred, slot});
+    settle(1);
+  }
+
+  void settle(size_t keep) {
+    while (inflight.size() > keep) {
+      const InFlight& f = inflight.front();
+      const bool last = inflight.size() == 1;
+      if (last) stream_sync(ctx);
+      else SG_CUDA(cudaEventSynchronize(copied[f.slot]));
+      const Counters& c = counters[f.slot];
+      if (c.error || c.n_def[f.slot]) { resolve_all(); return; }
+      if (last) known_groups = (int64_t)c.n_groups;
+      inflight.pop_front();
+    }
+  }
+
+  void resolve_all() {
     Trace tr(ctx, "agg.resolve");
+    stream_sync(ctx);
+    const Counters* latest = &counters[inflight.back().slot];
     uint64_t prev_def = 0;
     for (;;) {
-      unsigned long long gd[3] = {0, 0, 0};
-      SG_CUDA(cudaMemcpyAsync(gd, run.scal.n_groups(), 24, cudaMemcpyDeviceToHost, ctx->stream));
-      check_device_error(ctx, run.scal.error());
-      const uint64_t groups = gd[0], n_def = gd[2];
-      if (n_def == 0) { known_groups = (int64_t)groups; break; }
-      const int64_t tile_rows = (int64_t)pend.cp->rpt * NT;
-      const double rows_def = (double)std::min<int64_t>((int64_t)n_def * tile_rows, pend.batch->rows);
+      raise_device_error(ctx, run.scal.error(), latest->error);
+      const uint64_t groups = latest->n_groups;
+      double rows_def = 0.0;
+      uint64_t n_def_total = 0;
+      for (auto& f : inflight) {
+        const uint64_t n_def = latest->n_def[f.slot];
+        n_def_total += n_def;
+        rows_def += (double)std::min<int64_t>((int64_t)n_def * f.cp->rpt * NT, f.batch->rows);
+      }
+      if (n_def_total == 0) { known_groups = (int64_t)groups; break; }
       const double rows_done = std::max(1.0, (double)rows_in_table - rows_def);
       const double ratio = groups ? std::min(1.0, (double)groups / rows_done) : 1.0;
       const double est = ratio * rows_def * 1.25 + 1024.0;
       uint64_t cap = next_pow2((uint64_t)(2.0 * ((double)groups + est)) + 2 * MIN_CAPACITY / 2);
-      const bool stuck = prev_def != 0 && n_def >= prev_def;
+      const bool stuck = prev_def != 0 && n_def_total >= prev_def;
       if (cap <= tab.capacity && stuck) cap = tab.capacity * 2;
-      prev_def = n_def;
-      if (cap > tab.capacity) alloc_table(pend.cp->agg, cap, groups);
-      std::shared_ptr<CompiledPipeline> cp = pend.cp;
+      prev_def = n_def_total;
+      if (cap > tab.capacity) alloc_table(inflight.front().cp->agg, cap, groups);
       if (!use_cold && groups > CARD_MANY_GROUPS && getenv("SAILGPU_NO_COLD") == nullptr) {
-        auto cold = run.compiled_for(*pend.batch, true);
-        if (cold->agg.entry_words == cp->agg.entry_words) {
-          use_cold = true;
-          if (cold->rpt == cp->rpt) cp = cold;
+        auto cold = run.compiled_for(*inflight.front().batch, true);
+        if (cold->agg.entry_words == inflight.front().cp->agg.entry_words) use_cold = true;
+      }
+      for (auto it = inflight.begin(); it != inflight.end();) {
+        const uint64_t n_def = latest->n_def[it->slot];
+        if (n_def == 0) { it = inflight.erase(it); continue; }
+        if (use_cold && !it->cp->cold_variant) {
+          auto cold = run.compiled_for(*it->batch, true);
+          if (cold->rpt == it->cp->rpt && cold->agg.entry_words == it->cp->agg.entry_words) it->cp = cold;
         }
-      }
-      BufPtr next_deferred = dev_alloc(ctx, (size_t)n_def * 4);
-      launch_agg(cp, *pend.batch, pend.deferred, (int64_t)n_def, next_deferred);
-      pend.cp = cp; pend.deferred = next_deferred;
-    }
-    pend = Pending();
+        BufPtr next_deferred = dev_alloc(ctx, (size_t)n_def * 4);
+        launch_agg(it->cp, *it->batch, it->deferred, (int64_t)n_def, next_deferred, it->slot);
+        it->deferred = next_deferred;
+        ++it;
+      }
+      const int slot = inflight.back().slot;
+      copy_counters(slot, false);
+      stream_sync(ctx);
+      latest = &counters[slot];
+    }
+    inflight.clear();
+  }
+
+  uint64_t current_groups() {
+    settle(0);
+    if (known_groups < 0) {
+      run.ensure_scratch();
+      unsigned long long gd[4] = {0, 0, 0, 0};
+      SG_CUDA(cudaMemcpyAsync(gd, run.scal.buf->ptr, 32, cudaMemcpyDeviceToHost, ctx->stream));
+      stream_sync(ctx);
+      raise_device_error(ctx, run.scal.error(), (uint32_t)gd[0]);
+      known_groups = (int64_t)gd[3];
+    }
+    return (uint64_t)known_groups;
   }
 
   BatchPtr extract_agg() {
-    resolve_pending();
     Trace tr(ctx, "agg.extract");
     std::shared_ptr<CompiledPipeline> cp = agg_cp;
     if (!cp) {
@@ -437,11 +517,7 @@
     }
     const AggParams& A0 = cp->agg;
     run.ensure_scratch();
-    uint64_t groups = 0;
-    if (tab.capacity) {
-      if (known_groups >= 0) groups = (uint64_t)known_groups;
-      else { check_device_error(ctx, run.scal.error()); groups = read_n_groups(); }
-    }
+    const uint64_t groups = tab.capacity ? current_groups() : 0;
     const bool synth = A0.n_keys == 0 && groups == 0;
     const int64_t rows = synth ? 1 : (int64_t)groups;
     auto out = std::make_shared<DevBatch>();
@@ -482,7 +558,9 @@
         if (vbytes[(size_t)i] && is_count) SG_CUDA(cudaMemsetAsync(vbytes[(size_t)i]->ptr, 1, 1, ctx->stream));
       }
     }
-    SG_CUDA(cudaMemsetAsync(run.scal.nulls(0), 0, 8 * 20, ctx->stream));
+    bool any_nullable = false;
+    for (int i = 0; i < X.n_cols; ++i) any_nullable |= vbytes[(size_t)i] && rows > 0;
+    if (!any_nullable) return out;
     std::vector<unsigned long long> nulls((size_t)X.n_cols, 0);
     BufPtr nullctr = dev_alloc_zero(ctx, (size_t)X.n_cols * 8 + 8);
     for (int i = 0; i < X.n_cols; ++i) {
@@ -493,7 +571,7 @@
                                 static_cast<unsigned long long*>(nullctr->ptr) + i, ctx->stream));
     }
     SG_CUDA(cudaMemcpyAsync(nulls.data(), nullctr->ptr, (size_t)X.n_cols * 8, cudaMemcpyDeviceToHost, ctx->stream));
-    SG_CUDA(cudaStreamSynchronize(ctx->stream));
+    stream_sync(ctx);
     for (int i = 0; i < X.n_cols; ++i) {
       DevColumn& c = out->cols[(size_t)i];
       if (c.validity) { c.null_count = (int64_t)nulls[(size_t)i]; if (c.null_count == 0) c.validity = nullptr; }
@@ -579,12 +657,23 @@
     SG_CHECK(op->run.stages[i].kind != StageSpec::Aggregate, SAILGPU_ERR_INVALID, "aggregate must be the last stage of a pipeline");
   op->out_schema = cur;
   if (kind == "aggregate" && !g_in_static_check) {
-    bool wide = false;
-    g_in_static_check = true;
-    try { pipeline_static_check(spec, inputs); }
-    catch (const Error& e) { wide = e.code == SAILGPU_ERR_UNSUPPORTED && std::string(e.what()).find("group key") != std::string::npos; }
-    g_in_static_check = false;
-    if (wide) return make_wide_agg_op(ctx, spec, inputs, cur);
+    std::shared_ptr<bool> verdict;
+    const std::string vkey = "wide_agg|" + op->share_key;
+    const bool cacheable = ctx && ctx->stream != nullptr;
+    if (cacheable) {
+      auto it = ctx->shared_objects.find(vkey);
+      if (it != ctx->shared_objects.end()) verdict = std::static_pointer_cast<bool>(it->second);
+    }
+    if (!verdict) {
+      bool wide = false;
+      g_in_static_check = true;
+      try { pipeline_static_check(spec, inputs); }
+      catch (const Error& e) { wide = e.code == SAILGPU_ERR_UNSUPPORTED && std::string(e.what()).find("group key") != std::string::npos; }
+      g_in_static_check = false;
+      verdict = std::make_shared<bool>(wide);
+      if (cacheable) ctx->shared_objects.emplace(vkey, std::static_pointer_cast<void>(verdict));
+    }
+    if (*verdict) return make_wide_agg_op(ctx, spec, inputs, cur);
   }
   return op;
 }
diff --git a/sail_b200/csrc/engine.hpp b/sail_b200/csrc/engine.hpp
--- a/sail_b200/csrc/engine.hpp
+++ b/sail_b200/csrc/engine.hpp
@@ -15,6 +15,7 @@
   uint64_t elapsed_compute_ns = 0, kernel_launches = 0;
   uint64_t build_input_rows = 0, build_input_batches = 0, build_time_ns = 0, join_time_ns = 0;
   uint64_t pipeline_launches = 0, pipeline_kernel_ns = 0, jit_launches = 0;
+  uint64_t host_syncs = 0;
   std::vector<std::pair<cudaEvent_t, cudaEvent_t>> pending;
 };
 
diff --git a/sail_b200/csrc/ops_more.cu b/sail_b200/csrc/ops_more.cu
--- a/sail_b200/csrc/ops_more.cu
+++ b/sail_b200/csrc/ops_more.cu
@@ -369,7 +369,7 @@
     const int64_t nblocks = std::min<int64_t>(1024, (n + 4095) / 4096);
     uint64_t total = 0;
     SG_CUDA(cudaMemcpyAsync(&total, static_cast<uint64_t*>(scratch->ptr) + nblocks, 8, cudaMemcpyDeviceToHost, ctx->stream));
-    SG_CUDA(cudaStreamSynchronize(ctx->stream));
+    stream_sync(ctx);
     if (total == 0) return;
     BufPtr ob = dev_alloc(ctx, (size_t)total * 8), op = dev_alloc(ctx, (size_t)total * 8);
     J.offsets = static_cast<const uint64_t*>(offs->ptr); J.out_build = static_cast<int64_t*>(ob->ptr); J.out_probe = static_cast<int64_t*>(op->ptr);
@@ -381,7 +381,7 @@
     out->rows = (int64_t)total;
     for (size_t i = 0; i < bs.size(); ++i) out->cols.push_back(gather_column(build->cols[i], bs[i], J.out_build, (int64_t)total, jt == "right"));
     for (size_t i = 0; i < ps.size(); ++i) out->cols.push_back(gather_column(b->cols[i], ps[i], J.out_probe, (int64_t)total, false));
-    SG_CUDA(cudaStreamSynchronize(ctx->stream));
+    stream_sync(ctx);
     ready.push_back(post_filter(out));
   }
 
@@ -667,20 +667,20 @@
     if (c.validity) {
       uint8_t byte = 0;
       SG_CUDA(cudaMemcpyAsync(&byte, static_cast<const uint8_t*>(c.validity->ptr) + (row >> 3), 1, cudaMemcpyDeviceToHost, ctx->stream));
-      SG_CUDA(cudaStreamSynchronize(ctx->stream));
+      stream_sync(ctx);
       if (!((byte >> (row & 7)) & 1)) { e->lit_null = true; e->nullable = true; return e; }
     }
     if (t.id == TypeId::Bool) {
       uint8_t byte = 0;
       SG_CUDA(cudaMemcpyAsync(&byte, static_cast<const uint8_t*>(c.data->ptr) + (row >> 3), 1, cudaMemcpyDeviceToHost, ctx->stream));
-      SG_CUDA(cudaStreamSynchronize(ctx->stream));
+      stream_sync(ctx);
       e->lit_i = (byte >> (row & 7)) & 1;
       return e;
     }
     const int w = t.is_string() ? 16 : t.arrow_width();
     uint8_t raw[16] = {0};
     SG_CUDA(cudaMemcpyAsync(raw, static_cast<const uint8_t*>(c.data->ptr) + row * w, (size_t)w, cudaMemcpyDeviceToHost, ctx->stream));
-    SG_CUDA(cudaStreamSynchronize(ctx->stream));
+    stream_sync(ctx);
     if (t.is_string()) {
       uint32_t len; memcpy(&len, raw, 4);
       e->lit_s.resize(len);
@@ -688,7 +688,7 @@
       else {
         uint64_t ptr; memcpy(&ptr, raw + 8, 8);
         SG_CUDA(cudaMemcpyAsync(&e->lit_s[0], reinterpret_cast<const void*>(ptr), len, cudaMemcpyDeviceToHost, ctx->stream));
-        SG_CUDA(cudaStreamSynchronize(ctx->stream));
+        stream_sync(ctx);
       }
     } else if (t.id == TypeId::Float64) { memcpy(&e->lit_f, raw, 8); }
     else if (t.id == TypeId::Float32) { float f; memcpy(&f, raw, 4); e->lit_f = f; }
@@ -816,13 +816,10 @@
 
   struct Encoded { BufPtr keys, bits; int key_bytes = 0; };
 
-  Encoded encode_keys(const BatchPtr& all, const Schema& sch, const std::vector<Key>& ks) {
-    const int64_t n = all->rows;
+  SortEncodeParams describe_keys(const BatchPtr& all, const Schema& sch, const std::vector<Key>& ks) {
     SortEncodeParams E; memset(&E, 0, sizeof(E));
-    E.n = n; E.n_keys = (int)ks.size();
-    int off = 0;
-    BufPtr maxlen = dev_alloc_zero(ctx, 8 * 8);
-    std::vector<int> str_keys;
+    E.n = all->rows; E.n_keys = (int)ks.size();
+    SG_CHECK(ks.size() <= sizeof(E.cols) / sizeof(E.cols[0]), SAILGPU_ERR_UNSUPPORTED, "more than 8 sort keys");
     for (size_t k = 0; k < ks.size(); ++k) {
       SG_CHECK(ks[k].e->kind == Expr::Col, SAILGPU_ERR_UNSUPPORTED, "sort keys must be column references");
       const DevColumn& c = all->cols[(size_t)ks[k].e->col];
@@ -831,16 +828,27 @@
       s.data = static_cast<const uint8_t*>(c.data->ptr);
       s.validity_bits = c.validity ? static_cast<const uint8_t*>(c.validity->ptr) : nullptr;
       s.asc = ks[k].asc; s.nulls_first = ks[k].nulls_first;
-      if (t.is_string()) { s.kind = SORT_VIEW; s.width = 16; SG_CUDA(launch_max_view_len(c.data->ptr, n, static_cast<unsigned int*>(maxlen->ptr) + k, ctx->stream)); str_keys.push_back((int)k); }
+      if (t.is_string()) { s.kind = SORT_VIEW; s.width = 16; }
       else if (t.id == TypeId::Bool) { s.kind = SORT_BOOL; s.width = 1; s.enc_bytes = 1; }
       else if (t.is_float()) { SG_CHECK(t.id == TypeId::Float64, SAILGPU_ERR_UNSUPPORTED, "Float32 sort keys"); s.kind = SORT_F64; s.width = 8; s.enc_bytes = 8; }
       else if (t.is_unsigned_int()) { s.kind = SORT_UINT; s.width = t.arrow_width(); s.enc_bytes = s.width; }
       else { s.kind = SORT_INT; s.width = t.arrow_width(); s.enc_bytes = s.width; }
     }
+    return E;
+  }
+
+  Encoded encode_keys(const BatchPtr& all, const Schema& sch, const std::vector<Key>& ks) {
+    const int64_t n = all->rows;
+    SortEncodeParams E = describe_keys(all, sch, ks);
+    int off = 0;
+    BufPtr maxlen = dev_alloc_zero(ctx, 8 * 8);
+    std::vector<int> str_keys;
+    for (size_t k = 0; k < ks.size(); ++k)
+      if (E.cols[k].kind == SORT_VIEW) { SG_CUDA(launch_max_view_len(E.cols[k].data, n, static_cast<unsigned int*>(maxlen->ptr) + k, ctx->stream)); str_keys.push_back((int)k); }
     if (!str_keys.empty()) {
       unsigned int lens[8] = {0};
       SG_CUDA(cudaMemcpyAsync(lens, maxlen->ptr, sizeof(lens), cudaMemcpyDeviceToHost, ctx->stream));
-      SG_CUDA(cudaStreamSynchronize(ctx->stream));
+      stream_sync(ctx);
       for (int k : str_keys) {
         SG_CHECK(lens[k] <= 256, SAILGPU_ERR_UNSUPPORTED, "sort key strings longer than 256 bytes are not supported yet");
         E.cols[k].str_len = (int)lens[k]; E.cols[k].enc_bytes = (int)lens[k] + 4;
@@ -872,6 +880,15 @@
     const int64_t n = all->rows;
     if (n == 0) return all;
     SG_CHECK(n < (1ll << 32), SAILGPU_ERR_UNSUPPORTED, "sort of more than 2^32 rows in one partition");
+    const int64_t take = limit >= 0 ? std::min<int64_t>(limit, n) : n;
+    if (n <= SMALL_SORT_ROWS) {
+      const SortEncodeParams E = describe_keys(all, sch, ks);
+      BufPtr order = dev_alloc(ctx, (size_t)n * 4), idx = dev_alloc(ctx, (size_t)take * 8);
+      SG_CUDA(launch_small_sort_cols(E, static_cast<uint32_t*>(order->ptr), ctx->stream));
+      SG_CUDA(launch_widen_u32(static_cast<const uint32_t*>(order->ptr), static_cast<int64_t*>(idx->ptr), take, ctx->stream));
+      m.kernel_launches += 2;
+      return take_rows(all, sch, static_cast<const int64_t*>(idx->ptr), take);
+    }
     Encoded enc = encode_keys(all, sch, ks);
     const int64_t n_chunks = (n + 2047) / 2048;
     BufPtr ia = dev_alloc(ctx, (size_t)n * 4), ib = dev_alloc(ctx, (size_t)n * 4), ka = dev_alloc(ctx, (size_t)n * 8), kbuf = dev_alloc(ctx, (size_t)n * 8),
@@ -883,12 +900,9 @@
     int sort_launches = 0;
     SG_CUDA(radix_sort_indices(static_cast<const uint8_t*>(enc.keys->ptr), enc.key_bytes, n, S, static_cast<const uint32_t*>(enc.bits->ptr), ctx->stream, &sort_launches));
     m.kernel_launches += (uint64_t)(sort_launches + 1);
-    const int64_t take = limit >= 0 ? std::min<int64_t>(limit, n) : n;
     BufPtr idx = dev_alloc(ctx, (size_t)take * 8);
     SG_CUDA(launch_widen_u32(static_cast<const uint32_t*>(ia->ptr), static_cast<int64_t*>(idx->ptr), take, ctx->stream));
-    BatchPtr out = take_rows(all, sch, static_cast<const int64_t*>(idx->ptr), take);
-    SG_CUDA(cudaStreamSynchronize(ctx->stream));
-    return out;
+    return take_rows(all, sch, static_cast<const int64_t*>(idx->ptr), take);
   }
 
   static constexpr int64_t TOPK_MIN_ROWS = 1 << 18, TOPK_MAX_K = 1 << 16;
@@ -908,7 +922,7 @@
       SG_CUDA(cudaMemsetAsync(hist->ptr, 0, 2048 * 4, ctx->stream));
       SG_CUDA(launch_topk_hist(kp, enc.key_bytes, n, used, prefix, db, static_cast<uint32_t*>(hist->ptr), ctx->stream));
       SG_CUDA(cudaMemcpyAsync(h.data(), hist->ptr, 2048 * 4, cudaMemcpyDeviceToHost, ctx->stream));
-      SG_CUDA(cudaStreamSynchronize(ctx->stream));
+      stream_sync(ctx);
       m.kernel_launches += 1;
       int64_t run = below;
       int bin = 0;
@@ -997,7 +1011,7 @@
           BufPtr idx = dev_alloc(ctx, (size_t)fetch * 8);
           SG_CUDA(launch_iota(static_cast<int64_t*>(idx->ptr), fetch, ctx->stream));
           r = take_rows(r, sch, static_cast<const int64_t*>(idx->ptr), fetch);
-          SG_CUDA(cudaStreamSynchronize(ctx->stream));
+          stream_sync(ctx);
         }
     if (runs.size() == 1) return runs[0];
     std::vector<int64_t> off(runs.size() + 1, 0);
@@ -1012,7 +1026,7 @@
     m.kernel_launches += 1;
     const int64_t take = fetch >= 0 ? std::min<int64_t>(fetch, n) : n;
     BatchPtr out = take_rows(all, sch, static_cast<const int64_t*>(perm->ptr), take);
-    SG_CUDA(cudaStreamSynchronize(ctx->stream));
+    stream_sync(ctx);
     return out;
   }
 };
@@ -1135,7 +1149,7 @@
                                static_cast<const uint8_t*>(hk->ptr), static_cast<unsigned long long*>(coll->ptr), ctx->stream));
     unsigned long long n_coll = 0;
     SG_CUDA(cudaMemcpyAsync(&n_coll, coll->ptr, 8, cudaMemcpyDeviceToHost, ctx->stream));
-    SG_CUDA(cudaStreamSynchronize(ctx->stream));
+    stream_sync(ctx);
     if (n_coll != 0 || getenv("SAILGPU_WIDEAGG_FULL_SORT") != nullptr) {
       int more = 0;
       SG_CUDA(radix_sort_indices(static_cast<const uint8_t*>(enc.keys->ptr), enc.key_bytes, n, S, static_cast<const uint32_t*>(enc.bits->ptr), ctx->stream, &more));
@@ -1145,7 +1159,7 @@
     SG_CUDA(launch_exclusive_scan_u32(static_cast<const uint32_t*>(heads->ptr), n, static_cast<uint64_t*>(before->ptr), static_cast<uint64_t*>(scr2->ptr), ctx->stream));
     uint64_t n_groups = 0;
     SG_CUDA(cudaMemcpyAsync(&n_groups, static_cast<uint64_t*>(scr2->ptr) + std::min<int64_t>(1024, (n + 4095) / 4096), 8, cudaMemcpyDeviceToHost, ctx->stream));
-    SG_CUDA(cudaStreamSynchronize(ctx->stream));
+    stream_sync(ctx);
     DevColumn gid; gid.type = T(TypeId::Int64); gid.length = n; gid.data = dev_alloc(ctx, (size_t)n * 8);
     BufPtr rep = dev_alloc(ctx, (size_t)n_groups * 8);
     SG_CUDA(launch_assign_groups(S.idx_a, static_cast<const uint32_t*>(heads->ptr), static_cast<const uint64_t*>(before->ptr), n,
@@ -1183,7 +1197,7 @@
     }
     for (size_t i = 1; i < agg->cols.size(); ++i) out->cols.push_back(agg->cols[i]);
     m.kernel_launches += (uint64_t)n_keys + 1;
-    SG_CUDA(cudaStreamSynchronize(ctx->stream));
+    stream_sync(ctx);
     return out;
   }
 };
@@ -1228,7 +1242,7 @@
       ready[(size_t)p].push_back(pb);
     }
     next_idx = (next_idx + n) % n_parts;
-    SG_CUDA(cudaStreamSynchronize(ctx->stream));
+    stream_sync(ctx);
   }
 
   void push(int input, const BatchPtr& b) override {
@@ -1276,7 +1290,7 @@
     run.launch(P, cp, &aux, m);
     std::vector<int64_t> cnt((size_t)n_parts), off((size_t)n_parts);
     SG_CUDA(cudaMemcpyAsync(cnt.data(), counts->ptr, (size_t)n_parts * 8, cudaMemcpyDeviceToHost, ctx->stream));
-    SG_CUDA(cudaStreamSynchronize(ctx->stream));
+    stream_sync(ctx);
     int64_t run_off = 0;
     for (int p = 0; p < n_parts; ++p) { off[(size_t)p] = run_off; run_off += cnt[(size_t)p]; }
     SG_CUDA(cudaMemcpyAsync(offsets->ptr, off.data(), (size_t)n_parts * 8, cudaMemcpyHostToDevice, ctx->stream));
@@ -1328,7 +1342,7 @@
       }
       ready[(size_t)p].push_back(pb);
     }
-    SG_CUDA(cudaStreamSynchronize(ctx->stream));
+    stream_sync(ctx);
   }
 };
 
@@ -1392,7 +1406,7 @@
       auto b = std::make_shared<DevBatch>();
       b->rows = k;
       for (size_t c = 0; c < sch.size(); ++c) b->cols.push_back(helper.gather_column(result->cols[c], sch[c], static_cast<const int64_t*>(idx->ptr), k, false));
-      SG_CUDA(cudaStreamSynchronize(ctx->stream));
+      stream_sync(ctx);
       run_batches.push_back(b);
     }
     if (run_batches.empty()) run_batches.push_back(result);
@@ -1612,7 +1626,7 @@
   NCCL_CALL(g_nccl.AllGather(dmine->ptr, dall->ptr, mine.size(), NCCL_INT64, ctx->nccl_comm, ctx->stream));
   std::vector<int64_t> all(mine.size() * (size_t)W);
   SG_CUDA(cudaMemcpyAsync(all.data(), dall->ptr, all.size() * 8, cudaMemcpyDeviceToHost, ctx->stream));
-  SG_CUDA(cudaStreamSynchronize(ctx->stream));
+  stream_sync(ctx);
   auto cnt = [&](int src, int dst, size_t field) { return all[((size_t)src * W + dst) * rec + field]; };
   if (abort_above_rows >= 0) {
     int64_t mx = 0;
diff --git a/sail_b200/csrc/parquet.cu b/sail_b200/csrc/parquet.cu
--- a/sail_b200/csrc/parquet.cu
+++ b/sail_b200/csrc/parquet.cu
@@ -376,7 +376,7 @@
     expand_runs_kernel<<<(int)std::min<int64_t>((n + 255) / 256, grid_cap(8)), 256, 0, ctx->stream>>>(dbase, static_cast<const Run*>(druns->ptr), static_cast<const int64_t*>(dstarts->ptr),
                                                                                                 (int)runs.size(), n, static_cast<uint32_t*>(out->ptr));
     SG_CUDA(cudaGetLastError());
-    SG_CUDA(cudaStreamSynchronize(ctx->stream));
+    stream_sync(ctx);
     return out;
   };
   DecodeParams D; memset(&D, 0, sizeof(D));
@@ -412,7 +412,7 @@
     ddict = dev_alloc(ctx, (size_t)std::max<int64_t>(dict_count, 1) * out_width);
     if (dict_count) decode_values_kernel<<<(int)std::min<int64_t>((dict_count + 255) / 256, grid_cap(4)), 256, 0, ctx->stream>>>(Q, static_cast<uint8_t*>(ddict->ptr));
     SG_CUDA(cudaGetLastError());
-    SG_CUDA(cudaStreamSynchronize(ctx->stream));
+    stream_sync(ctx);
     didx = expand(index_runs, dense_done);
     D.dict_idx = static_cast<const uint32_t*>(didx->ptr); D.dict_vals = static_cast<const uint8_t*>(ddict->ptr); D.dict_size = (uint32_t)dict_count;
   }
@@ -438,7 +438,7 @@
   }
   uint32_t e = 0;
   SG_CUDA(cudaMemcpyAsync(&e, err->ptr, 4, cudaMemcpyDeviceToHost, ctx->stream));
-  SG_CUDA(cudaStreamSynchronize(ctx->stream));
+  stream_sync(ctx);
   SG_CHECK(e == 0, SAILGPU_ERR_INVALID, "parquet: dictionary index out of range in column '" + f.name + "'");
   return col;
 }
diff --git a/sail_b200/csrc/relational.cu b/sail_b200/csrc/relational.cu
--- a/sail_b200/csrc/relational.cu
+++ b/sail_b200/csrc/relational.cu
@@ -266,6 +266,64 @@
   idx_out[rank] = (uint32_t)i;
 }
 
+__device__ int cmp_sort_key(const SortKeyCol& c, int64_t a, int64_t b) {
+  const bool na = c.validity_bits && !((c.validity_bits[a >> 3] >> (a & 7)) & 1);
+  const bool nb = c.validity_bits && !((c.validity_bits[b >> 3] >> (b & 7)) & 1);
+  if (na || nb) return na == nb ? 0 : ((na == (c.nulls_first != 0)) ? -1 : 1);
+  int r = 0;
+  switch (c.kind) {
+    case SORT_INT:
+    case SORT_UINT: {
+      const uint8_t* pa = c.data + a * c.width;
+      const uint8_t* pb = c.data + b * c.width;
+      for (int i = 0; i < c.width && r == 0; ++i) {
+        const uint8_t f = (i == 0 && c.kind == SORT_INT) ? 0x80 : 0x00;
+        r = (int)(pa[c.width - 1 - i] ^ f) - (int)(pb[c.width - 1 - i] ^ f);
+      }
+      break;
+    }
+    case SORT_F64: {
+      uint64_t x = *reinterpret_cast<const uint64_t*>(c.data + a * 8), y = *reinterpret_cast<const uint64_t*>(c.data + b * 8);
+      x = (x >> 63) ? ~x : (x | 0x8000000000000000ull);
+      y = (y >> 63) ? ~y : (y | 0x8000000000000000ull);
+      r = x < y ? -1 : (x > y ? 1 : 0);
+      break;
+    }
+    case SORT_BOOL:
+      r = (int)((c.data[a >> 3] >> (a & 7)) & 1) - (int)((c.data[b >> 3] >> (b & 7)) & 1);
+      break;
+    default: {
+      const uint8_t* va = c.data + a * 16;
+      const uint8_t* vb = c.data + b * 16;
+      const ulonglong2 x = *reinterpret_cast<const ulonglong2*>(va), y = *reinterpret_cast<const ulonglong2*>(vb);
+      const uint32_t la = (uint32_t)x.x, lb = (uint32_t)y.x;
+      const uint8_t* sa = view_ptr(x, va);
+      const uint8_t* sb = view_ptr(y, vb);
+      const uint32_t m = la > lb ? la : lb;
+      for (uint32_t i = 0; i < m && r == 0; ++i) r = (int)(i < la ? sa[i] : 0) - (int)(i < lb ? sb[i] : 0);
+      if (r == 0) r = la < lb ? -1 : (la > lb ? 1 : 0);
+    }
+  }
+  return c.asc ? r : -r;
+}
+__global__ void small_sort_cols_kernel(const SortEncodeParams P, uint32_t* __restrict__ idx_out) {
+  const int i = threadIdx.x;
+  if (i >= P.n) return;
+  int rank = 0;
+  for (int j = 0; j < (int)P.n; ++j) {
+    int c = 0;
+    for (int k = 0; k < P.n_keys && c == 0; ++k) c = cmp_sort_key(P.cols[k], j, i);
+    rank += (c < 0 || (c == 0 && j < i)) ? 1 : 0;
+  }
+  idx_out[rank] = (uint32_t)i;
+}
+cudaError_t launch_small_sort_cols(const SortEncodeParams& P, uint32_t* idx_out, cudaStream_t s) {
+  if (P.n == 0) return cudaSuccess;
+  if (P.n > SMALL_SORT_ROWS) return cudaErrorInvalidValue;
+  small_sort_cols_kernel<<<1, SMALL_SORT_ROWS, 0, s>>>(P, idx_out);
+  return cudaGetLastError();
+}
+
 cudaError_t radix_sort_indices(const uint8_t* keys, int key_bytes, int64_t n, const RadixScratch& S, const uint32_t* bits, cudaStream_t s, int* launches) {
   int nl = 0;
   if (launches) *launches = 0;
diff --git a/sail_b200/csrc/relational.hpp b/sail_b200/csrc/relational.hpp
--- a/sail_b200/csrc/relational.hpp
+++ b/sail_b200/csrc/relational.hpp
@@ -63,6 +63,8 @@
 cudaError_t launch_gather_bits(const uint8_t* bits, uint8_t* out, const int64_t* idx, int64_t n, int dflt, cudaStream_t s);
 cudaError_t launch_max_view_len(const void* views, int64_t n, unsigned int* out, cudaStream_t s);
 cudaError_t launch_sort_encode(const SortEncodeParams& P, cudaStream_t s);
+constexpr int SMALL_SORT_ROWS = 1024;
+cudaError_t launch_small_sort_cols(const SortEncodeParams& P, uint32_t* idx_out, cudaStream_t s);
 cudaError_t radix_sort_indices(const uint8_t* keys, int key_bytes, int64_t n, const RadixScratch& S, const uint32_t* bits, cudaStream_t s, int* launches);
 cudaError_t launch_topk_hist(const uint8_t* keys, int key_bytes, int64_t n, int used, uint64_t prefix, int digit_bits, uint32_t* hist , cudaStream_t s);
 cudaError_t launch_topk_compact(const uint8_t* keys, int key_bytes, int64_t n, int used, uint64_t threshold, int64_t* out, unsigned long long* counter, cudaStream_t s);
diff --git a/sail_b200/csrc/runner.hpp b/sail_b200/csrc/runner.hpp
--- a/sail_b200/csrc/runner.hpp
+++ b/sail_b200/csrc/runner.hpp
@@ -120,7 +120,7 @@
       }
       if (!cp->literals.empty()) {
         SG_CUDA(cudaMemcpyAsync(dp.literals->ptr, blob.data(), blob.size(), cudaMemcpyHostToDevice, ctx->stream));
-        SG_CUDA(cudaStreamSynchronize(ctx->stream));
+        stream_sync(ctx);
       }
       for (auto& fx : cp->literal_fixups) cp->prog[(size_t)fx.first].imm1 = dp.literal_ptrs[(size_t)fx.second];
       it = programs.emplace(cp.get(), std::move(dp)).first;
@@ -298,7 +298,7 @@
         c.null_count = -1;
       }
     }
-    if (!bool_tmp.empty() || !valid_tmp.empty()) SG_CUDA(cudaStreamSynchronize(ctx->stream));
+    if (!bool_tmp.empty() || !valid_tmp.empty()) stream_sync(ctx);
   } else {
     check_device_error(ctx, run.scal.error());
   }
```

Result: faster. 25.84 billion (median of 6 runs) (+3.3%).
